# MishaLaskin/vqvae

Measured on AMD Instinct MI355X. Metric: images/sec VQ-VAE forward (32x32x3, K=512, D=64), higher is better.
Workload: dtype f32 (fp32 in/out/accumulate; conv products from two fp16 terms per operand, <= 2^-21 rel per product); 1 GPU; BASELINE config 3: full HIP path (Encoder+VQ+Decoder), 32x32x3, K=512, D=64; per_gpu_batch=4096, global_batch=4096, K=512, D=64, parallelism=batch-sharded replicas x1, no collective

## Files before the change

### vqvae_amd/csrc/common.h

```cpp
#pragma once

#include <hip/hip_runtime.h>
#include <stddef.h>
#include <stdint.h>

#include "../../include/vqvae_hip.h"

namespace vqvae {

typedef float f32x4 __attribute__((ext_vector_type(4)));
typedef float f32x16 __attribute__((ext_vector_type(16)));

__device__ __forceinline__ float sqsum8_f16(unsigned vx, unsigned vy, unsigned vz, unsigned vw, float s) {
    asm("v_dot2c_f32_f16 %0, %1, %1\n\tv_dot2c_f32_f16 %0, %2, %2\n\tv_dot2c_f32_f16 %0, %3, %3\n\tv_dot2c_f32_f16 %0, %4, %4"
        : "+v"(s) : "v"(vx), "v"(vy), "v"(vz), "v"(vw));
    return s;
}

constexpr int kWave = 64;
constexpr int kLdsBytes = 160 * 1024;

inline int num_cus() {
    static int n[64] = {0};
    int dev = 0;
    if (hipGetDevice(&dev) != hipSuccess || dev < 0 || dev >= 64) return 256;
    if (n[dev] == 0) {
        hipDeviceProp_t p;
        int c = 0;
        if (hipGetDeviceProperties(&p, dev) == hipSuccess) c = p.multiProcessorCount;
        n[dev] = c > 0 ? c : 256;
    }
    return n[dev];
}

void prof_begin(int id, hipStream_t st);
void prof_end(int id, hipStream_t st);
bool prof_dispatch(int id, hipEvent_t *start, hipEvent_t *stop);

inline size_t align_up(size_t x, size_t a) { return (x + a - 1) / a * a; }

inline unsigned grid_of(long long total, long long cap = 65536) {
    long long g = (total + 255) / 256;
    if (g > cap) g = cap;
    if (g < 1) g = 1;
    return (unsigned)g;
}

__device__ __forceinline__ void block_sum_f64(double *red, int tid, double v) {
    red[tid] = v;
    __syncthreads();
    for (int o = 128; o > 0; o >>= 1) {
        if (tid < o) red[tid] += red[tid + o];
        __syncthreads();
    }
}

struct VqPlan {
    int KC;
    int nchunks;
    int K_pad;
    size_t off_flags, off_ee, off_img, off_partials, off_img16, off_neh, off_imgh, off_seeds, off_imgf, off_chunk, total;
    size_t lds_bytes;
    int K32;
    size_t filter_lds_bytes;
};
constexpr int kVqCandCap = 8;
constexpr int kVqTilesPerWave = 2;
constexpr int kVqTicketBytes = 4096;
constexpr int kVqMaxGrid = 1024;
constexpr int kVqSlabRows = 1 << 18;
constexpr int kVqGroupSlabs = 16;

bool vq_track_ok(int K, int D);
bool vq_chunk_ok(int K, int D);
size_t vq_chunk_scratch_bytes(int D);

inline size_t vq_filter_lds_bytes(int K, int D) {
    const size_t K32 = ((size_t)K + 31) / 32 * 32;
    return K32 * D * 2 + K32 * 4 + (size_t)K * 4 + kVqTilesPerWave * (8 * 32 * 2 * kVqCandCap * 2 + 8 * 96 * 4) + 256 + 8;
}

enum class VqRoute { Track, TrackNchw, Chunk, Filter, Exact, AnyD, GenericVector, Unsupported };
VqRoute vq_route(int K, int D, int HW, int flags);

inline VqPlan vq_plan(int K, int D) {
    VqPlan p;
    const long budget = kLdsBytes - 256 - (long)K * 4;
    long kc = budget / ((long)D * 4 + 4);
    kc = kc / 32 * 32;
    const long kneed = ((long)K + 31) / 32 * 32;
    if (kc > kneed) kc = kneed;
    if (kc < 32) kc = 32;
    p.KC = (int)kc;
    p.nchunks = (K + p.KC - 1) / p.KC;
    p.K_pad = p.nchunks * p.KC;
    p.lds_bytes = (size_t)p.KC * D * 4 + (size_t)p.KC * 4 + (size_t)K * 4 + 256;
    p.off_flags = 0;
    p.off_ee = 256 + kVqTicketBytes;
    p.off_img = align_up(p.off_ee + (size_t)p.K_pad * 4, 256);
    p.off_partials = align_up(p.off_img + (size_t)p.K_pad * D * 4, 256);
    p.K32 = (K + 31) / 32 * 32;
    p.off_img16 = align_up(p.off_partials + sizeof(double) * kVqMaxGrid, 256);
    p.off_neh = align_up(p.off_img16 + (size_t)p.K32 * D * 2, 256);
    p.off_imgh = align_up(p.off_neh + (size_t)p.K32 * 4, 256);
    p.off_seeds = align_up(p.off_imgh + (size_t)(p.K32 + 512) * D * 2, 256);
    p.off_imgf = align_up(p.off_seeds + (size_t)p.K32 * 4 + 4096, 256);
    p.off_chunk = align_up(p.off_imgf + (size_t)(p.K32 + 512) * D * 2, 256);
    p.total = p.off_chunk + (vq_route(K, D, 0, VQVAE_VQ_ROWMAJOR) == VqRoute::Chunk ? vq_chunk_scratch_bytes(D) : 0);
    p.filter_lds_bytes = vq_filter_lds_bytes(K, D);
    return p;
}

int launch_vq_filter_d64(const float *z, const float *cb, long long N, int HW, int K, bool rowmajor,
                         float *zq, long long *idx, int *hist, char *ws, hipStream_t st, int *grid_out);

bool vq_track_nchw_ok(int K, int D, int HW);
inline int vq_form_of_flags(int flags) {
    const bool a = flags & VQVAE_VQ_UNITS64_8WAVES, b = flags & VQVAE_VQ_UNITS32_16WAVES;
    if (flags & VQVAE_VQ_UNITS32_8WAVES) return 32;
    return a && b ? 12 : (b ? 16 : (a ? 8 : 0));
}
struct VqTrackForm { int waves, unit_rows, grid, pool_pct; long long nunits; };
bool vq_track_form(long long N, int K, int HW, bool nchw, int form, int cus, VqTrackForm &f);
int launch_vq_track_d64(const float *z, const float *cb, long long N, int K, float *zq, long long *idx, int *hist,
                        char *ws, hipStream_t st, int *grid_out, int HW = 0, bool nchw = false, int form = 0);
void launch_vq_prepare16(const float *cb, int K, int D, char *ws, hipStream_t st);
int launch_vq_chunked(const float *z, const float *cb, long long N, int K, int D, float *zq, long long *idx, int *hist,
                      char *ws, hipStream_t st, int *grid_out, int *zq_amax = nullptr, int hw = 1);

int conv_forward_impl(int kind, const float *x, const float *packed, const float *bias, int64_t B, int H, int W, int Cin,
                      int Cout, int flags, float *y, hipStream_t stream, const int *in_amax, int *out_amax,
                      const float *ep_add = nullptr, const float *ep_mask = nullptr);
bool conv_reads_amax(int kind, int H, int W, int Cin, int Cout, int flags);
int res_layer_forward_impl(const float *x, const float *packed_w1, const float *packed_w2, int64_t B, int H, int W, int C,
                           int Rh, int flags, float *y, hipStream_t stream, const int *in_amax, int *out_amax,
                           float *hidden = nullptr, float *hid_scratch = nullptr);
bool res_layer_fused_ok(int C, int Rh);
bool res_pair_supported(int H, int W, int C, int Rh, int flags);
struct VqFuse {
    const uint4 *imgf; const float *seeds; const float *ee; const int *flags; const float *cb;
    int K, K32;
    float *zq; long long *idx; int *hist; double *partials;
};
struct ResPairPost { const float *packed; const float *bias; int Cout; float *out; int *zero = nullptr; int zero_n = 0;
                     const VqFuse *vq = nullptr; bool debug_ze = false; };
bool res_pair_post_supported(int C, int Cout);
int res_pair_forward_impl(const float *x, const float *packed_w1, const float *packed_w2, int64_t B, int H, int W, int C,
                          int Rh, int flags, float *y, hipStream_t stream, const int *in_amax, int *out_amax,
                          const ResPairPost *post = nullptr);
bool conv_res_pair_supported(int kind, int H, int W, int Cin, int C, int Rh);
int conv_res_pair_forward_impl(int kind, const float *x, const float *packed_front, const float *bias_front, int Cin,
                               const float *packed_w1, const float *packed_w2, int64_t B, int H, int W, int C, int Rh, int flags,
                               float *y, hipStream_t stream, const int *in_amax, int *out_amax, const ResPairPost *post = nullptr,
                               const int64_t *gather_idx = nullptr, int gather_K = 0);
int convt_out_forward_impl(const float *x, const float *packed, const float *bias, int64_t B, int H, int W, int Cin, int Cout,
                           int flags, float *y_nchw, hipStream_t stream, const int *in_amax);
void weight_spread_impl(const float *w, int Cout, int Cin, int taps, bool transposed, float *out, hipStream_t st);
void act_absmax_impl(const float *x, int64_t B, long long elems_per_image, int *amax, hipStream_t st);
constexpr int kVqGenericMaxD = 256;
constexpr int kRowSqnormMaxD = 1024;
bool vq_generic_ok(int K, int D);
size_t vq_generic_workspace_bytes(int K, int D);
int launch_vq_generic(const float *z, const float *cb, long long N, int HW, int K, int D, float beta, bool rowmajor, float *zq,
                      long long *idx, int *hist, float *loss, float *ppl, char *ws, hipStream_t st, bool hist_zeroed,
                      bool vector_units = false, bool prepared = false);
bool vq_fuse_ok(int K, int D, int flags);
int vq_prepare_impl(const float *codebook, int K, int D, int flags, void *workspace, size_t workspace_bytes, hipStream_t st);
VqFuse vq_fuse_args(const float *codebook, int K, void *workspace, float *z_q, int64_t *idx, int32_t *hist);
int vq_finalize_impl(const double *partials, int grid, int32_t *hist, int K, int64_t n_rows, int D, float beta, float *loss,
                     float *perplexity, hipStream_t st);
int vq_forward_impl(const float *z_e, const float *codebook, int64_t B, int D, int H, int W, int K, float beta, int flags,
                    float *z_q, int64_t *idx, int32_t *hist, float *loss, float *perplexity, void *workspace,
                    size_t workspace_bytes, vqvae_stream_t stream, bool hist_zeroed, int *zq_amax = nullptr,
                    bool *zq_amax_done = nullptr);
bool enc_front_supported(int H, int W, int Cin, int C1, int C2);
int enc_front_forward_impl(const float *x_nchw, const float *packed_in, const float *bias_in, const float *packed2,
                           const float *bias2, int64_t B, int H, int W, int Cin, int C1, int C2, float *y, hipStream_t st,
                           int *out_amax, int *zero_buf = nullptr, int zero_n = 0);
bool dec_tail_supported(int h4, int w4, int C, int C1, int Cout);
int dec_tail_forward_impl(const float *x, const float *packed2, const float *bias2, const float *packed4, const float *bias4,
                          int64_t B, int h4, int w4, int C, int C1, int Cout, float *y_nchw, hipStream_t st, const int *in_amax);
int conv_in_forward_impl(const float *x_nchw, const float *packed, const float *bias, int64_t B, int H, int W, int Cin,
                         int Cout, int flags, float *y, hipStream_t stream, int *out_amax, const float *ep_mask = nullptr);

}
```

### vqvae_amd/csrc/conv_fused.hip

```cpp
#include "conv_host.h"

namespace vqvae {
#ifndef CRP_NW
#define CRP_NW 4
#endif
#ifndef CRP_MINW
#define CRP_MINW 2
#endif
template <int NT3, bool VQ = false, bool GATHER = false, bool ZEOUT = false>
__global__ __launch_bounds__(CRP_NW * 64, CRP_MINW) void conv_res_pair8_h2_kernel(const float *__restrict__ in, FrontConv fc,
                                                                   const u32x4 *__restrict__ w1img, const u32x4 *__restrict__ w2img,
                                                                   float *__restrict__ out, int B, int flags,
                                                                   const int *__restrict__ hdr1, const int *__restrict__ hdr2,
                                                                   const int *__restrict__ in_amax, int *__restrict__ out_amax,
                                                                   const u32x4 *__restrict__ w3img, const int *__restrict__ hdr3,
                                                                   const float *__restrict__ bias3, float *__restrict__ out3,
                                                                   int *__restrict__ zero_buf, int zero_n, VqFuse vq) {
    static_assert(NT3 == 0 || NT3 == 1 || NT3 == 2 || NT3 == 4, "the 1x1 post conv streams through NT3 weight stages of 16 KiB");
    static_assert(!VQ || (NT3 == 2 && CRP_NW == 4), "the fused quantizer takes the 64-channel z_e of four images per workgroup");
    constexpr int NT2 = 4, C = 128, MT = 2, PX = 64, HP = PX + 1, PLANE = HP * 2;
    constexpr int TILE4 = 2 * 2 * PLANE;
    constexpr int RBUF = 4 * HP;
    __shared__ u32x4 As_all[CRP_NW * TILE4];
    constexpr int WBUF = 18 * 64;
    const int nvq = VQ ? (vq.K32 >> 7) : 0;
    const int NSTAGE = 18 + NT3 + nvq;
    __shared__ u32x4 Wb_all[2 * WBUF];
    __shared__ __attribute__((aligned(16))) unsigned char vq_tab_all[VQ ? CRP_NW * 1040 : 16];
    __shared__ int vq_hist_s[VQ ? 1024 : 1];
    __shared__ __attribute__((aligned(16))) float dw_s[288 + 32 * (NT3 > 0 ? NT3 : 1)];
    for (int i = threadIdx.x; i < 288 + 32 * NT3; i += CRP_NW * 64)
        dw_s[i] = i < 128 ? h2_dw(fc.hdr)[i] : (i < 160 ? h2_dw(hdr1)[i - 128] : (i < 288 ? h2_dw(hdr2)[i - 160] : h2_dw(hdr3)[i - 288]));
    __shared__ double vq_red_s[VQ ? CRP_NW : 1];
    if constexpr (VQ) {
        for (int i = threadIdx.x; i < vq.K; i += CRP_NW * 64) vq_hist_s[i] = 0;
    }
    const int tid = threadIdx.x, lane = tid & 63, wave = tid >> 6;
    const int l31 = lane & 31, h = lane >> 5;
    u32x4 *As = As_all + wave * TILE4;
    float *Hs = reinterpret_cast<float *>(As);
    const bool relu_out = flags & kFlagReluOut;
    constexpr int cpt = C >> 5;

    const long long img = (long long)blockIdx.x * CRP_NW + wave;
    const bool img_ok = img < B;
    if (zero_buf && blockIdx.x == 0)
        for (int i = tid; i < zero_n; i += CRP_NW * 64) zero_buf[i] = 0;

    int spx[MT];
    unsigned tapok[MT], tapok0[MT];
#pragma unroll
    for (int mt = 0; mt < MT; ++mt) {
        spx[mt] = 32 * mt + l31;
        const int y = spx[mt] >> 3, x = spx[mt] & 7;
        unsigned m = 0, m0 = 0;
#pragma unroll
        for (int t = 0; t < 9; ++t) {
            const int yy = y + t / 3 - 1, xx = x + t % 3 - 1;
            if (yy >= 0 && yy < 8 && xx >= 0 && xx < 8) m |= 1u << t;
            const int y0 = y + (int)((fc.dym >> (4 * t)) & 15) - 8, x0 = x + (int)((fc.dxm >> (4 * t)) & 15) - 8;
            if (y0 >= 0 && y0 < 8 && x0 >= 0 && x0 < 8) m0 |= 1u << t;
        }
        tapok[mt] = m;
        tapok0[mt] = m0;
    }

    f32x16 Y[MT][NT2];
    const int wave_u = __builtin_amdgcn_readfirstlane(wave);
    const unsigned dma_lane = (unsigned)lane * 16u;
    auto dma = [&](const u32x4 *src_uniform, u32x4 *dst_piece) {
        const unsigned lds = __builtin_amdgcn_readfirstlane((unsigned)(unsigned long long)(__attribute__((address_space(3))) char *)(char *)dst_piece);
        asm volatile("s_mov_b32 m0, %2\n\ts_nop 0\n\tglobal_load_lds_dwordx4 %0, %1" ::"v"(dma_lane), "s"(src_uniform), "s"(lds) : "memory");
    };
    auto dma_slice = [&](int sl, int buf) {
        const u32x4 *base = w1img + (size_t)(sl >> 1) * 256 + (sl & 1) * 64;
        for (int p = wave_u; p < 18; p += CRP_NW)
            dma(base + (size_t)(p >> 1) * cpt * 256 + (p & 1) * 128, Wb_all + buf * WBUF + p * 64);
    };
    auto dma_linear = [&](const u32x4 *src, int buf) {
#pragma unroll
        for (int j = 0; j < 16 / CRP_NW; ++j) dma(src + (wave_u * (16 / CRP_NW) + j) * 64, Wb_all + buf * WBUF + (wave_u * (16 / CRP_NW) + j) * 64);
    };
    auto dma_stage = [&](int k, int buf) {
        if (VQ && k >= 18 + NT3) {
            const int j = k - (18 + NT3);
            dma_linear(reinterpret_cast<const u32x4 *>(vq.imgf) + (size_t)j * 1024, buf);
            if (wave_u == 0) dma(reinterpret_cast<const u32x4 *>(vq.seeds) + (size_t)j * 32, Wb_all + buf * WBUF + 16 * 64);
        }
        else if (k >= 18) dma_linear(w3img + (size_t)(k - 18) * 1024, buf);
        else if (k % 9 == 8) dma_linear(w2img, buf);
        else dma_slice(k % 9, buf);
    };
    auto dma_wait_sync = [&]() {
        asm volatile("s_waitcnt vmcnt(0)" ::: "memory");
        __syncthreads();
    };
    float ymax = 0.0f;
    int wstage = 0;
    {
        const int cpt0 = fc.Cin >> 5;
        const float *src = in + ((size_t)(img_ok ? img : 0) * PX + lane) * fc.Cin;
        bool gbad = false;
        if constexpr (GATHER) {
            const long long k = vq.idx[(size_t)(img_ok ? img : 0) * PX + lane];
            gbad = k < 0 || k >= vq.K;
            src = in + (size_t)(gbad ? 0 : k) * fc.Cin;
        }
        const bool gany = GATHER && __builtin_amdgcn_ballot_w64(gbad) != 0;
        f32x4 raw[8];
        auto load_raw0 = [&](int cc) {
#pragma unroll
            for (int j = 0; j < 8; ++j) raw[j] = *reinterpret_cast<const f32x4 *>(src + 32 * cc + 4 * j);
            if (gany) {
                const float qn = __builtin_nanf("");
#pragma unroll
                for (int j = 0; j < 8; ++j) if (gbad) raw[j] = f32x4{qn, qn, qn, qn};
            }
        };
        float m = 0.0f;
        const int given = (in_amax && img_ok) ? in_amax[img] : -1;
        if (given >= 0) m = __int_as_float(given);
        else for (int cc = 0; cc < cpt0; ++cc) {
            load_raw0(cc);
#pragma unroll
            for (int j = 0; j < 8; ++j)
                m = fmaxf(m, fmaxf(fmaxf(__builtin_fabsf(raw[j].x), __builtin_fabsf(raw[j].y)), fmaxf(__builtin_fabsf(raw[j].z), __builtin_fabsf(raw[j].w))));
        }
        const int kx = wave_scale_exp(img_ok ? m : 0.0f);
        const float xs = __builtin_ldexpf(1.0f, kx), d0 = __builtin_ldexpf(1.0f, -kx);
#pragma unroll
        for (int mt = 0; mt < MT; ++mt)
#pragma unroll
            for (int nt = 0; nt < NT2; ++nt)
#pragma unroll
                for (int r = 0; r < 16; ++r) Y[mt][nt][r] = 0.0f;
        if (lane < 8) As[(lane >> 1) * PLANE + (lane & 1) * HP + PX] = u32x4{0, 0, 0, 0};
        auto dma_front = [&](int cc, int tap, int buf) {
            const u32x4 *base = fc.wimg + (size_t)(tap * cpt0 + cc) * (NT2 * 256);
#pragma unroll
            for (int j = 0; j < 16 / CRP_NW; ++j) {
                const int p = wave_u * (16 / CRP_NW) + j;
                dma(base + (p >> 2) * 256 + ((p >> 1) & 1) * 64 + (p & 1) * 128, Wb_all + buf * WBUF + p * 64);
            }
        };
        load_raw0(0);
        dma_front(0, 0, 0);
        for (int cc = 0; cc < cpt0; ++cc) {
            __builtin_amdgcn_wave_barrier();
            u32x4 *dst = As + lane;
#pragma unroll
            for (int t = 0; t < 2; ++t)
#pragma unroll
                for (int hh = 0; hh < 2; ++hh) {
                    u32x4 t1, t2;
                    split8_h(raw[4 * hh + 2 * t], raw[4 * hh + 2 * t + 1], xs, t1, t2);
                    dst[(t * 2 + 0) * PLANE + hh * HP] = t1;
                    dst[(t * 2 + 1) * PLANE + hh * HP] = t2;
                }
            lds_order_wave();
#pragma unroll 1
            for (int tap = 0; tap < 9; ++tap, ++wstage) {
                const int shift = ((int)((fc.dym >> (4 * tap)) & 15) - 8) * 8 + ((int)((fc.dxm >> (4 * tap)) & 15) - 8);
                u32x4 X[2][MT][2];
#pragma unroll
                for (int t = 0; t < 2; ++t)
#pragma unroll
                    for (int mt = 0; mt < MT; ++mt) {
                        const int p = ((tapok0[mt] >> tap) & 1u) ? spx[mt] + shift : PX;
                        const u32x4 *ap = As + (t * 2) * PLANE + h * HP + p;
                        X[t][mt][0] = ap[0];
                        X[t][mt][1] = ap[PLANE];
                    }
                if (tap == 1 && cc + 1 < cpt0) {
                    asm volatile("s_waitcnt vmcnt(8)" ::: "memory");
                    __syncthreads();
                } else dma_wait_sync();
                if (tap + 1 < 9) dma_front(cc, tap + 1, (wstage + 1) & 1);
                else if (cc + 1 < cpt0) dma_front(cc + 1, 0, (wstage + 1) & 1);
                else dma_stage(0, (wstage + 1) & 1);
                if (tap == 0 && cc + 1 < cpt0) load_raw0(cc + 1);
                const u32x4 *wt = Wb_all + (wstage & 1) * WBUF + lane;
                u32x4 Wc0 = wt[0], Wc1 = wt[64];
#pragma unroll
                for (int g = 0; g < 8; ++g) {
                    const int t = g >> 2, nt = g & 3;
                    u32x4 Wn0 = Wc0, Wn1 = Wc1;
                    if (g + 1 < 8) {
                        const u32x4 *bp = wt + (((g + 1) & 3) * 4 + ((g + 1) >> 2) * 2) * 64;
                        Wn0 = bp[0];
                        Wn1 = bp[64];
                    }
                    __builtin_amdgcn_sched_barrier(0);
                    prod3x2t(X[t][0][0], X[t][0][1], X[t][1][0], X[t][1][1], Wc0, Wc1, Y[0][nt], Y[1][nt]);
                    __builtin_amdgcn_sched_barrier(0);
                    Wc0 = Wn0;
                    Wc1 = Wn1;
                }
            }
        }
#pragma unroll
        for (int nt = 0; nt < NT2; ++nt)
#pragma unroll
            for (int g = 0; g < 4; ++g) {
                f32x4 bv = {0.0f, 0.0f, 0.0f, 0.0f};
                if (fc.bias) bv = *reinterpret_cast<const f32x4 *>(fc.bias + nt * 32 + 8 * g + 4 * h);
                const f32x4 dv = h2_dw4(dw_s, nt * 32, g, h, d0);
#pragma unroll
                for (int mt = 0; mt < MT; ++mt)
#pragma unroll
                    for (int q = 0; q < 4; q += 2)
                        SCALE2_BIAS_RELU2(Y[mt][nt][4 * g + q], Y[mt][nt][4 * g + q + 1], dv[q], dv[q + 1], bv[q], bv[q + 1], ymax);
            }
    }
    lds_order_wave();

    auto stage_sync = [&](int k) -> const u32x4 * {
        dma_wait_sync();
        if (k + 1 < NSTAGE) dma_stage(k + 1, (wstage + k + 1) & 1);
        return Wb_all + ((wstage + k) & 1) * WBUF + lane;
    };
    f32x16 acc1[MT];
    auto taps = [&](const u32x4 *wb, const u32x4 *pl) {
        u32x4 Xc[MT][2], Wc[2];
        auto ld = [&](int tap, u32x4(&X)[MT][2], u32x4(&W)[2]) {
            const int shift = (tap / 3 - 1) * 8 + (tap % 3 - 1);
#pragma unroll
            for (int mt = 0; mt < MT; ++mt) {
                const int p = ((tapok[mt] >> tap) & 1u) ? spx[mt] + shift : PX;
                X[mt][0] = pl[p];
                X[mt][1] = pl[p + HP * 2];
            }
            W[0] = wb[tap * 128];
            W[1] = wb[tap * 128 + 64];
        };
        ld(0, Xc, Wc);
#pragma unroll
        for (int tap = 0; tap < 9; ++tap) {
            u32x4 Xn[MT][2], Wn[2];
            if (tap + 1 < 9) ld(tap + 1, Xn, Wn);
            __builtin_amdgcn_sched_barrier(0);
            prod3x2t(Xc[0][0], Xc[0][1], Xc[1][0], Xc[1][1], Wc[0], Wc[1], acc1[0], acc1[1]);
            __builtin_amdgcn_sched_barrier(0);
            if (tap + 1 < 9) {
#pragma unroll
                for (int mt = 0; mt < MT; ++mt) { Xc[mt][0] = Xn[mt][0]; Xc[mt][1] = Xn[mt][1]; }
                Wc[0] = Wn[0]; Wc[1] = Wn[1];
            }
        }
    };
    auto put_planes = [&](int buf, const u32x4(&T1)[MT][2], const u32x4(&T2)[MT][2], int t) {
        u32x4 *pb = As + buf * RBUF + h * HP + l31;
#pragma unroll
        for (int mt = 0; mt < MT; ++mt) {
            pb[32 * mt] = T1[mt][t];
            pb[32 * mt + 2 * HP] = T2[mt][t];
        }
    };
    auto layer = [&](auto LT, bool relu_after) __attribute__((always_inline)) {
        constexpr int LI = decltype(LT)::value;
        const int kx = wave_scale_exp(img_ok ? ymax : 0.0f);
        const float xscale = __builtin_ldexpf(1.0f, kx), d1 = __builtin_ldexpf(1.0f, -kx);
#pragma unroll
        for (int mt = 0; mt < MT; ++mt)
#pragma unroll
            for (int r = 0; r < 16; ++r) acc1[mt][r] = 0.0f;
        u32x4 T1[MT][2], T2[MT][2];
#pragma unroll
        for (int mt = 0; mt < MT; ++mt) acc_to_ksteps(Y[mt][0], xscale, T1[mt], T2[mt]);
        __builtin_amdgcn_wave_barrier();
        put_planes(0, T1, T2, 0);
#pragma unroll
        for (int c = 0; c < NT2; ++c) {
            __builtin_amdgcn_wave_barrier();
            put_planes(1, T1, T2, 1);
            lds_order_wave();
            taps(stage_sync(9 * LI + 2 * c), As + h * HP);
            if (c + 1 < NT2) {
#pragma unroll
                for (int mt = 0; mt < MT; ++mt) acc_to_ksteps(Y[mt][c + 1], xscale, T1[mt], T2[mt]);
                __builtin_amdgcn_wave_barrier();
                put_planes(0, T1, T2, 0);
            }
            lds_order_wave();
            taps(stage_sync(9 * LI + 2 * c + 1), As + RBUF + h * HP);
        }
        float m = 0.0f;
#pragma unroll
        for (int g = 0; g < 4; ++g) {
            const f32x4 dv = h2_dw4(dw_s + 128, 0, g, h, d1);
#pragma unroll
            for (int mt = 0; mt < MT; ++mt)
#pragma unroll
                for (int q = 0; q < 4; q += 2)
                    SCALE2_BIAS_RELU2(acc1[mt][4 * g + q], acc1[mt][4 * g + q + 1], dv[q], dv[q + 1], 0.0f, 0.0f, m);
        }
        const int kh = wave_scale_exp(m);
        const float hscale = __builtin_ldexpf(1.0f, kh), d2 = __builtin_ldexpf(1.0f, -kh);
        u32x4 H1[MT][2], Hb[MT][2];
#pragma unroll
        for (int mt = 0; mt < MT; ++mt) acc_to_ksteps(acc1[mt], hscale, H1[mt], Hb[mt]);
        const u32x4 *wb = stage_sync(9 * LI + 8);
        float nmax = 0.0f;
#pragma unroll
        for (int nt = 0; nt < NT2; ++nt) {
            u32x4 Wc[2][2];
#pragma unroll
            for (int t = 0; t < 2; ++t) { Wc[t][0] = wb[nt * 256 + t * 64]; Wc[t][1] = wb[nt * 256 + t * 64 + 128]; }
            f32x16 acc2[MT];
#pragma unroll
            for (int mt = 0; mt < MT; ++mt)
#pragma unroll
                for (int r = 0; r < 16; ++r) acc2[mt][r] = 0.0f;
#pragma unroll
            for (int t = 0; t < 2; ++t)
                prod3x2t(H1[0][t], Hb[0][t], H1[1][t], Hb[1][t], Wc[t][0], Wc[t][1], acc2[0], acc2[1]);
            if (relu_after) {
#pragma unroll
                for (int g = 0; g < 4; ++g) {
                    const f32x4 dv = h2_dw4(dw_s + 160, nt * 32, g, h, d2);
#pragma unroll
                    for (int mt = 0; mt < MT; ++mt)
#pragma unroll
                        for (int q = 0; q < 4; q += 2) {
                            const int r = 4 * g + q;
                            const float y0 = relu1(__builtin_fmaf(acc2[mt][r], dv[q], Y[mt][nt][r]));
                            const float y1 = relu1(__builtin_fmaf(acc2[mt][r + 1], dv[q + 1], Y[mt][nt][r + 1]));
                            Y[mt][nt][r] = y0;
                            Y[mt][nt][r + 1] = y1;
                            vmax3(nmax, y0, y1);
                        }
                }
            } else {
#pragma unroll
                for (int g = 0; g < 4; ++g) {
                    const f32x4 dv = h2_dw4(dw_s + 160, nt * 32, g, h, d2);
#pragma unroll
                    for (int mt = 0; mt < MT; ++mt)
#pragma unroll
                        for (int q = 0; q < 4; q += 2) {
                            const int r = 4 * g + q;
                            const float y0 = __builtin_fmaf(acc2[mt][r], dv[q], Y[mt][nt][r]), y1 = __builtin_fmaf(acc2[mt][r + 1], dv[q + 1], Y[mt][nt][r + 1]);
                            Y[mt][nt][r] = y0;
                            Y[mt][nt][r + 1] = y1;
                            vmax3_abs(nmax, y0, y1);
                        }
                }
            }
        }
        ymax = nmax;
    };
    layer(std::integral_constant<int, 0>{}, true);
    layer(std::integral_constant<int, 1>{}, relu_out);
    if (out_amax && img_ok) publish_amax_exclusive(out_amax, img, ymax, lane);

    auto store_tile = [&](const float(&v)[16], float *dst, int ld) {
        __builtin_amdgcn_wave_barrier();
#pragma unroll
        for (int g = 0; g < 4; ++g)
            *reinterpret_cast<f32x4 *>(Hs + l31 * 36 + 8 * g + 4 * h) = f32x4{v[4 * g], v[4 * g + 1], v[4 * g + 2], v[4 * g + 3]};
        lds_order_wave();
#pragma unroll
        for (int k = 0; k < 4; ++k) {
            const int p = (lane >> 3) + 8 * k;
            *reinterpret_cast<f32x4 *>(dst + (size_t)p * ld + 4 * (lane & 7)) = *reinterpret_cast<const f32x4 *>(Hs + p * 36 + 4 * (lane & 7));
        }
    };
    const long long wbase = img * PX;
    if constexpr (NT3 > 0) {
        const int kx3 = wave_scale_exp(img_ok ? ymax : 0.0f);
        const float xs3 = __builtin_ldexpf(1.0f, kx3), d3 = __builtin_ldexpf(1.0f, -kx3);
        f32x16 acc3[MT][NT3];
#pragma unroll
        for (int mt = 0; mt < MT; ++mt)
#pragma unroll
            for (int n3 = 0; n3 < NT3; ++n3)
#pragma unroll
                for (int r = 0; r < 16; ++r) acc3[mt][n3][r] = 0.0f;
        const u32x4 *wb = nullptr;
#pragma unroll
        for (int c = 0; c < NT2; ++c) {
            u32x4 T1[MT][2], T2[MT][2];
#pragma unroll
            for (int mt = 0; mt < MT; ++mt) acc_to_ksteps(Y[mt][c], xs3, T1[mt], T2[mt]);
            constexpr int CPS = 4 / NT3;
            if (c % CPS == 0) wb = stage_sync(18 + c / CPS);
#pragma unroll
            for (int t = 0; t < 2; ++t)
#pragma unroll
                for (int n3 = 0; n3 < NT3; ++n3) {
                    const u32x4 *bp = wb + ((c % CPS) * NT3 + n3) * 256 + t * 64;
                    prod3x2t(T1[0][t], T2[0][t], T1[1][t], T2[1][t], bp[0], bp[128], acc3[0][n3], acc3[1][n3]);
                }
        }
        if constexpr (VQ) {
#pragma unroll
            for (int mt = 0; mt < MT; ++mt)
#pragma unroll
                for (int n3 = 0; n3 < NT3; ++n3)
#pragma unroll
                    for (int g = 0; g < 4; ++g) {
                        f32x4 bv = {0.0f, 0.0f, 0.0f, 0.0f};
                        if (bias3) bv = *reinterpret_cast<const f32x4 *>(bias3 + n3 * 32 + 8 * g + 4 * h);
                        const f32x4 dv = h2_dw4(dw_s + 288, n3 * 32, g, h, d3);
#pragma unroll
                        for (int q = 0; q < 4; ++q) acc3[mt][n3][4 * g + q] = acc3[mt][n3][4 * g + q] * dv[q] + bv[q];
                    }
            u32x4 zb[MT][4];
            float zn2[MT];
#pragma unroll
            for (int mt = 0; mt < MT; ++mt) {
                float sq = 0.0f;
#pragma unroll
                for (int n3 = 0; n3 < NT3; ++n3)
#pragma unroll
                    for (int t = 0; t < 2; ++t) {
                        float P[4], Q[4];
#pragma unroll
                        for (int q = 0; q < 4; ++q) {
                            P[q] = acc3[mt][n3][4 * t + q];
                            Q[q] = acc3[mt][n3][8 + 4 * t + q];
                            swap_halves(P[q], Q[q]);
                        }
                        u32x4 v;
                        v.x = __builtin_bit_cast(unsigned, __builtin_convertvector((f32x2v{P[0], P[1]}), f16x2));
                        v.y = __builtin_bit_cast(unsigned, __builtin_convertvector((f32x2v{P[2], P[3]}), f16x2));
                        v.z = __builtin_bit_cast(unsigned, __builtin_convertvector((f32x2v{Q[0], Q[1]}), f16x2));
                        v.w = __builtin_bit_cast(unsigned, __builtin_convertvector((f32x2v{Q[2], Q[3]}), f16x2));
                        zb[mt][2 * n3 + t] = v;
                        sq = sqsum8_f16(v.x, v.y, v.z, v.w, sq);
                    }
                const auto sw = __builtin_amdgcn_permlane32_swap(__float_as_uint(sq), __float_as_uint(sq), false, false);
                zn2[mt] = sq + __uint_as_float(h ? sw[0] : sw[1]);
            }
            const float inf = __builtin_inff();
            const float pinf = inf, ninf = -inf;
            unsigned keymask = trk::kKeyMask;
            asm volatile("" : "+v"(keymask));
            trk::Lane L[MT];
#pragma unroll
            for (int mt = 0; mt < MT; ++mt) trk::init(L[mt], ninf);
            auto sweep_stage = [&](const u32x4 *wb, const float *sd, int j, auto &&use) {
#pragma unroll
                for (int ctl = 0; ctl < 4; ++ctl) {
                    f32x16 seed;
#pragma unroll
                    for (int g = 0; g < 4; ++g) {
                        const f32x4 e4 = *reinterpret_cast<const f32x4 *>(sd + ctl * 32 + h * 16 + 4 * g);
                        seed[4 * g] = e4.x; seed[4 * g + 1] = e4.y; seed[4 * g + 2] = e4.z; seed[4 * g + 3] = e4.w;
                    }
                    u32x4 a[4];
#pragma unroll
                    for (int ks = 0; ks < 4; ++ks) a[ks] = wb[ctl * 256 + ks * 64];
                    use(4 * j + ctl, a, seed);
                }
            };
            for (int j = 0; j < nvq; ++j) {
                const u32x4 *wb = stage_sync(18 + NT3 + j);
                const float *sd = reinterpret_cast<const float *>(wb - lane + 16 * 64);
                sweep_stage(wb, sd, j, [&](int ct, const u32x4(&a)[4], const f32x16 &seed) {
                    f32x16 acc[MT];
#pragma unroll
                    for (int mt = 0; mt < MT; ++mt) {
                        acc[mt] = __builtin_amdgcn_mfma_f32_32x32x16_f16(__builtin_bit_cast(f16x8, a[0]), __builtin_bit_cast(f16x8, zb[mt][0]), seed, 0, 0, 0);
#pragma unroll
                        for (int ks = 1; ks < 4; ++ks)
                            acc[mt] = __builtin_amdgcn_mfma_f32_32x32x16_f16(__builtin_bit_cast(f16x8, a[ks]), __builtin_bit_cast(f16x8, zb[mt][ks]), acc[mt], 0, 0, 0);
                    }
                    unsigned cell0 = (unsigned)(2 * ct), cell1 = cell0 + 1u;
                    asm volatile("" : "+s"(cell0), "+s"(cell1));
#pragma unroll
                    for (int mt = 0; mt < MT; ++mt) trk::tile(L[mt], acc[mt], cell0, cell1, keymask, ninf, pinf);
                });
            }
            vqu::Tables tb = vqu::tables(vq_tab_all + wave_u * 1040);
            const vqu::BoundP bound = vqu::load_boundp(vq.flags);
            vqu::RowsSp<MT> R;
            vqu::classify_sp<MT>(L, zn2, bound, vq.K, lane, img_ok ? PX : 0, ninf, tb.task_s, R);
            vqu::Flagged FL = vqu::exact_begin_sp<MT>(R, lane, tb);
            int ntasks = FL.ndirect;
            const bool rescan_me = FL.hmask && FL.ndirect <= 64;
            int nres = 0;
            if (__syncthreads_or(rescan_me ? 1 : 0)) {
                dma_stage(18 + NT3, 0);
                for (int j = 0; j < nvq; ++j) {
                    dma_wait_sync();
                    if (j + 1 < nvq) dma_stage(18 + NT3 + j + 1, (j + 1) & 1);
                    if (rescan_me && FL.ndirect + nres <= 64) {
                        const u32x4 *wb = Wb_all + (j & 1) * WBUF + lane;
                        const float *sd = reinterpret_cast<const float *>(Wb_all + (j & 1) * WBUF + 16 * 64);
#pragma unroll
                        for (int mt = 0; mt < MT; ++mt)
                            if ((unsigned)(FL.hmask >> (32 * mt))) {
                                const float thr_t = (((unsigned)(FL.hmask >> (32 * mt)) >> l31) & 1u) ? R.thr[mt] : inf;
                                sweep_stage(wb, sd, j, [&](int ct, const u32x4(&a)[4], const f32x16 &seed) {
                                    f32x16 acc = __builtin_amdgcn_mfma_f32_32x32x16_f16(__builtin_bit_cast(f16x8, a[0]), __builtin_bit_cast(f16x8, zb[mt][0]), seed, 0, 0, 0);
#pragma unroll
                                    for (int ks = 1; ks < 4; ++ks)
                                        acc = __builtin_amdgcn_mfma_f32_32x32x16_f16(__builtin_bit_cast(f16x8, a[ks]), __builtin_bit_cast(f16x8, zb[mt][ks]), acc, 0, 0, 0);
                                    vqu::rescan_tile(acc, thr_t, ct, mt, lane, vq.K, FL.ndirect, ninf, tb, nres);
                                });
                            }
                    }
                }
                if (rescan_me) {
                    lds_order_wave();
                    ntasks = FL.ndirect + nres;
                }
            }
            __syncthreads();
            unsigned char *zlo = reinterpret_cast<unsigned char *>(As);
            unsigned char *zhi = reinterpret_cast<unsigned char *>(Wb_all) + (size_t)wave_u * 9216;
            auto zchunk = [&](int row, int c16) -> f32x4 * {
                unsigned char *b = row < 32 ? zlo + row * 256 : zhi + (row - 32) * 256;
                return reinterpret_cast<f32x4 *>(b + (((unsigned)c16 ^ ((unsigned)row & 15u)) << 4));
            };
            __builtin_amdgcn_wave_barrier();
#pragma unroll
            for (int mt = 0; mt < MT; ++mt)
#pragma unroll
                for (int n3 = 0; n3 < NT3; ++n3)
#pragma unroll
                    for (int g = 0; g < 4; ++g)
                        *zchunk(32 * mt + l31, 8 * n3 + 2 * g + h) = f32x4{acc3[mt][n3][4 * g], acc3[mt][n3][4 * g + 1], acc3[mt][n3][4 * g + 2], acc3[mt][n3][4 * g + 3]};
            lds_order_wave();
            if constexpr (ZEOUT) {
                if (img_ok)
#pragma unroll
                    for (int c16 = 0; c16 < 16; ++c16)
                        *reinterpret_cast<f32x4 *>(out3 + ((size_t)img * PX + lane) * 64 + 4 * c16) = *zchunk(lane, c16);
            }
            vqu::exact_end_sp<MT>(R, FL, ntasks, lane, tb, vq.cb, vq.ee, vq.K,
                           [&](int rr, int jc) { return *zchunk(rr, jc); },
                           [&](int rr, int c) { return reinterpret_cast<const float *>(zchunk(rr, c >> 2))[c & 3]; });
            const int j16 = lane & 15, g4 = lane >> 4;
            const float sacc = vqu::epilogue_sp<false, MT>(R, lane, vq.cb, vq.K, [&](int t, int i) { return *zchunk(32 * t + 4 * i + g4, j16); },
                                             (img_ok && vq.zq) ? vq.zq + (size_t)img * PX * 64 : nullptr, img_ok ? PX : 0,
                                             vq.idx + (size_t)(img_ok ? img : 0) * PX, vq_hist_s);
            double dacc = img_ok ? (double)sacc : 0.0;
#pragma unroll
            for (int o = 32; o > 0; o >>= 1) dacc += __shfl_xor(dacc, o);
            if (lane == 0) vq_red_s[wave_u] = dacc;
            __syncthreads();
            if (tid == 0) {
                double sum = 0.0;
                for (int w = 0; w < CRP_NW; ++w) sum += vq_red_s[w];
                vq.partials[blockIdx.x] = sum;
            }
            for (int k = tid; k < vq.K; k += CRP_NW * 64) {
                const int c = vq_hist_s[k];
                if (c) atomicAdd(&vq.hist[k], c);
            }
        } else
        if (img_ok) {
#pragma unroll
            for (int mt = 0; mt < MT; ++mt)
#pragma unroll
                for (int n3 = 0; n3 < NT3; ++n3) {
                    float v[16];
#pragma unroll
                    for (int g = 0; g < 4; ++g) {
                        f32x4 bv = {0.0f, 0.0f, 0.0f, 0.0f};
                        if (bias3) bv = *reinterpret_cast<const f32x4 *>(bias3 + n3 * 32 + 8 * g + 4 * h);
                        const f32x4 dv = h2_dw4(dw_s + 288, n3 * 32, g, h, d3);
#pragma unroll
                        for (int q = 0; q < 4; ++q) v[4 * g + q] = acc3[mt][n3][4 * g + q] * dv[q] + bv[q];
                    }
                    store_tile(v, out3 + (wbase + mt * 32) * (32 * NT3) + n3 * 32, 32 * NT3);
                }
        }
    } else if (img_ok) {
#pragma unroll
        for (int mt = 0; mt < MT; ++mt)
#pragma unroll
            for (int nt = 0; nt < NT2; ++nt) {
                float v[16];
#pragma unroll
                for (int r = 0; r < 16; ++r) v[r] = Y[mt][nt][r];
                store_tile(v, out + (wbase + mt * 32) * C + nt * 32, C);
            }
    }
}

#ifndef EF_MINW
#define EF_MINW 2
#endif
template <int CIN>
__global__ __launch_bounds__(256, EF_MINW) void enc_front8_h2_kernel(const float *__restrict__ x, const u32x4 *__restrict__ w0img,
                                                               const int *__restrict__ hdr0, const float *__restrict__ bias0,
                                                               const u32x4 *__restrict__ w2img, const int *__restrict__ hdr2,
                                                               const float *__restrict__ bias2, float *__restrict__ out, int B,
                                                               int *__restrict__ out_amax, int *__restrict__ zero_buf, int zero_n) {
    constexpr int NT = 4, MT = 2, PX = 64, HP = PX + 1, PLANE = HP * 2, C0 = 64, C = 128;
    if (zero_buf && blockIdx.x == 0)
        for (int i = threadIdx.x; i < zero_n; i += 256) zero_buf[i] = 0;
    constexpr int TILE4 = 2 * 2 * PLANE;
    constexpr int WBUF = 16 * 64, NSTAGE = 32;
    __shared__ u32x4 As_all[4 * TILE4];
    __shared__ u32x4 Wb_all[2 * WBUF];
    __shared__ u32x4 W0s[2 * CIN * 2 * 64];
    __shared__ __attribute__((aligned(16))) float dw_s[64 + 128];
    const int tid = threadIdx.x, lane = tid & 63, wave = tid >> 6;
    const int l31 = lane & 31, h = lane >> 5;
    u32x4 *As = As_all + wave * TILE4;
    float *Hs = reinterpret_cast<float *>(As);
    const int wave_u = __builtin_amdgcn_readfirstlane(wave);
    const long long img = (long long)blockIdx.x * 4 + wave;
    const bool img_ok = img < B;

    const unsigned dma_lane = (unsigned)lane * 16u;
    auto dma = [&](const u32x4 *src_uniform, u32x4 *dst_piece) {
        const unsigned lds = __builtin_amdgcn_readfirstlane((unsigned)(unsigned long long)(__attribute__((address_space(3))) char *)(char *)dst_piece);
        asm volatile("s_mov_b32 m0, %2\n\ts_nop 0\n\tglobal_load_lds_dwordx4 %0, %1" ::"v"(dma_lane), "s"(src_uniform), "s"(lds) : "memory");
    };
    auto dma_stage = [&](int k, int buf) {
        const u32x4 *src = w2img + (size_t)k * 1024;
#pragma unroll
        for (int j = 0; j < 4; ++j) dma(src + (wave_u * 4 + j) * 64, Wb_all + buf * WBUF + (wave_u * 4 + j) * 64);
    };
    auto dma_wait_sync = [&]() {
        asm volatile("s_waitcnt vmcnt(0)" ::: "memory");
        __syncthreads();
    };
    dma_stage(0, 0);
    for (int i = tid; i < 2 * CIN * 2 * 64; i += 256) W0s[i] = w0img[i];
    if (tid < C0 + C) dw_s[tid] = tid < C0 ? h2_dw(hdr0)[tid] : h2_dw(hdr2)[tid - C0];
    if (lane < 8) As[(lane >> 1) * PLANE + (lane & 1) * HP + PX] = u32x4{0, 0, 0, 0};

    int spx[MT];
    unsigned tapok[MT];
#pragma unroll
    for (int mt = 0; mt < MT; ++mt) {
        spx[mt] = 32 * mt + l31;
        const int y = spx[mt] >> 3, xx0 = spx[mt] & 7;
        unsigned m = 0;
        for (int q = 0; q < 16; ++q) {
            const int yy = y + ((q >> 1) & 1) - (q >> 3), xx = xx0 + (q & 1) - ((q >> 2) & 1);
            if (yy >= 0 && yy < 8 && xx >= 0 && xx < 8) m |= 1u << q;
        }
        tapok[mt] = m;
    }

    const float *ximg = x + (size_t)(img_ok ? img : 0) * (CIN * 1024);
    float xm = 0.0f;
#pragma unroll
    for (int j = 0; j < CIN * 4; ++j) {
        const f32x4 v = *reinterpret_cast<const f32x4 *>(ximg + 4 * lane + 256 * j);
        xm = fmaxf(xm, fmaxf(fmaxf(__builtin_fabsf(v.x), __builtin_fabsf(v.y)), fmaxf(__builtin_fabsf(v.z), __builtin_fabsf(v.w))));
    }
#pragma unroll
    for (int o = 32; o > 0; o >>= 1) xm = fmaxf(xm, __shfl_xor(xm, o));
    const int kx0 = wave_scale_exp(img_ok ? xm : 0.0f);
    const float xs0 = __builtin_ldexpf(1.0f, kx0), d0 = __builtin_ldexpf(1.0f, -kx0);
    float bm = bias0 ? __builtin_fabsf(bias0[lane]) : 0.0f;
    const float bound = (__int_as_float(hdr0[1]) * xm + bm) * 1.0001f;
    const int k1 = wave_scale_exp(img_ok ? bound : 0.0f);
    const float xs1 = __builtin_ldexpf(1.0f, k1), d2 = __builtin_ldexpf(1.0f, -k1);

    f32x16 Y[MT][NT];
#pragma unroll
    for (int mt = 0; mt < MT; ++mt)
#pragma unroll
        for (int nt = 0; nt < NT; ++nt)
#pragma unroll
            for (int r = 0; r < 16; ++r) Y[mt][nt][r] = 0.0f;
    const long long img_u = (long long)blockIdx.x * 4 + wave_u;
    const auto xrs = __builtin_amdgcn_make_buffer_rsrc(const_cast<float *>(x + (size_t)(img_u < B ? img_u : 0) * (CIN * 1024)), 0,
                                                       (unsigned)(CIN * 4096), 0x00020000);
    __syncthreads();

    auto taps = [&](int cc) {
        const int sub = cc >> 1;
#pragma unroll 1
        for (int tap = 0; tap < 4; ++tap) {
            const int k = cc * 4 + tap;
            const int shift = ((tap >> 1) - (sub >> 1)) * 8 + ((tap & 1) - (sub & 1)), okbit = sub * 4 + tap;
            u32x4 X[2][MT][2];
#pragma unroll
            for (int t = 0; t < 2; ++t)
#pragma unroll
                for (int mt = 0; mt < MT; ++mt) {
                    const int p = ((tapok[mt] >> okbit) & 1u) ? spx[mt] + shift : PX;
                    const u32x4 *ap = As + (t * 2) * PLANE + h * HP + p;
                    X[t][mt][0] = ap[0];
                    X[t][mt][1] = ap[PLANE];
                }
            dma_wait_sync();
            if (k + 1 < NSTAGE) dma_stage(k + 1, (k + 1) & 1);
            const u32x4 *wt = Wb_all + (k & 1) * WBUF + lane;
            u32x4 Wc0 = wt[0], Wc1 = wt[128];
#pragma unroll
            for (int g = 0; g < 8; ++g) {
                const int t = g >> 2, nt = g & 3;
                u32x4 Wn0 = Wc0, Wn1 = Wc1;
                if (g + 1 < 8) {
                    const u32x4 *bp = wt + ((g + 1) & 3) * 256 + ((g + 1) >> 2) * 64;
                    Wn0 = bp[0];
                    Wn1 = bp[128];
                }
                __builtin_amdgcn_sched_barrier(0);
                prod3x2t(X[t][0][0], X[t][0][1], X[t][1][0], X[t][1][1], Wc0, Wc1, Y[0][nt], Y[1][nt]);
                __builtin_amdgcn_sched_barrier(0);
                Wc0 = Wn0;
                Wc1 = Wn1;
            }
        }
    };
    auto put_planes = [&](const u32x4(&T1)[MT][2], const u32x4(&T2)[MT][2]) {
        __builtin_amdgcn_wave_barrier();
#pragma unroll
        for (int t = 0; t < 2; ++t)
#pragma unroll
            for (int mt = 0; mt < MT; ++mt) {
                As[(t * 2 + 0) * PLANE + h * HP + 32 * mt + l31] = T1[mt][t];
                As[(t * 2 + 1) * PLANE + h * HP + 32 * mt + l31] = T2[mt][t];
            }
        lds_order_wave();
    };
    auto first_layer = [&](int sl, const u32x4(&XB)[MT][CIN][2], u32x4(&T1)[MT][2], u32x4(&T2)[MT][2]) {
        f32x16 acc0[MT];
#pragma unroll
        for (int mt = 0; mt < MT; ++mt)
#pragma unroll
            for (int r = 0; r < 16; ++r) acc0[mt][r] = 0.0f;
        const u32x4 *wp = W0s + (sl * CIN) * 128 + lane;
#pragma unroll
        for (int ci = 0; ci < CIN; ++ci)
            prod3x2t(XB[0][ci][0], XB[0][ci][1], XB[1][ci][0], XB[1][ci][1], wp[ci * 128], wp[ci * 128 + 64], acc0[0], acc0[1]);
#pragma unroll
        for (int g = 0; g < 4; ++g) {
            f32x4 bv = {0.0f, 0.0f, 0.0f, 0.0f};
            if (bias0) bv = *reinterpret_cast<const f32x4 *>(bias0 + sl * 32 + 8 * g + 4 * h);
            const f32x4 dv = h2_dw4(dw_s, sl * 32, g, h, d0);
#pragma unroll
            for (int mt = 0; mt < MT; ++mt)
#pragma unroll
                for (int q = 0; q < 4; q += 2) {
                    float unused = 0.0f;
                    SCALE2_BIAS_RELU2(acc0[mt][4 * g + q], acc0[mt][4 * g + q + 1], dv[q], dv[q + 1], bv[q], bv[q + 1], unused);
                }
        }
#pragma unroll
        for (int mt = 0; mt < MT; ++mt) acc_to_ksteps(acc0[mt], xs1, T1[mt], T2[mt]);
    };

#pragma unroll 1
    for (int s = 0; s < 4; ++s) {
        const int sy = s >> 1, sx = s & 1;
        u32x4 XB[MT][CIN][2];
#pragma unroll
        for (int mt = 0; mt < MT; ++mt) {
            const int by = spx[mt] >> 3, bx = spx[mt] & 7;
            const int col0 = 4 * bx + 2 * sx - 1;
            const int adj = col0 < 0 ? 1 : (col0 + 3 > 31 ? -1 : 0);
            f32x4 pv[CIN][2];
#pragma unroll
            for (int ci = 0; ci < CIN; ++ci)
#pragma unroll
                for (int rr = 0; rr < 2; ++rr) {
                    const int row = 4 * by + 2 * sy - 1 + 2 * h + rr;
                    const unsigned off = (row >= 0 && row < 32) ? (unsigned)(((ci * 32 + row) * 32 + col0 + adj) * 4) : kOobOffset;
                    pv[ci][rr] = __builtin_bit_cast(f32x4, __builtin_amdgcn_raw_buffer_load_b128(xrs, off, 0, 0));
                }
#pragma unroll
            for (int ci = 0; ci < CIN; ++ci) {
#pragma unroll
                for (int rr = 0; rr < 2; ++rr) {
                    const f32x4 v = pv[ci][rr];
                    f32x4 o;
                    o.x = adj > 0 ? 0.0f : (adj < 0 ? v.y : v.x);
                    o.y = adj > 0 ? v.x : (adj < 0 ? v.z : v.y);
                    o.z = adj > 0 ? v.y : (adj < 0 ? v.w : v.z);
                    o.w = adj > 0 ? v.z : (adj < 0 ? 0.0f : v.w);
                    pv[ci][rr] = o;
                }
                split8_h(pv[ci][0], pv[ci][1], xs0, XB[mt][ci][0], XB[mt][ci][1]);
            }
        }
        u32x4 T1[MT][2], T2[MT][2], U1[MT][2], U2[MT][2];
        first_layer(0, XB, T1, T2);
        put_planes(T1, T2);
        first_layer(1, XB, U1, U2);
        taps(2 * s);
        put_planes(U1, U2);
        taps(2 * s + 1);
    }

    float ymax = 0.0f;
    const long long wbase = img * PX;
#pragma unroll
    for (int mt = 0; mt < MT; ++mt)
#pragma unroll
        for (int nt = 0; nt < NT; ++nt) {
            float v[16];
#pragma unroll
            for (int g = 0; g < 4; ++g) {
                f32x4 bv = {0.0f, 0.0f, 0.0f, 0.0f};
                if (bias2) bv = *reinterpret_cast<const f32x4 *>(bias2 + nt * 32 + 8 * g + 4 * h);
                const f32x4 dv = h2_dw4(dw_s + C0, nt * 32, g, h, d2);
#pragma unroll
                for (int q = 0; q < 4; q += 2) {
                    v[4 * g + q] = Y[mt][nt][4 * g + q];
                    v[4 * g + q + 1] = Y[mt][nt][4 * g + q + 1];
                    SCALE2_BIAS_RELU2(v[4 * g + q], v[4 * g + q + 1], dv[q], dv[q + 1], bv[q], bv[q + 1], ymax);
                }
            }
            if (img_ok) {
                float *dst = out + (wbase + mt * 32) * C + nt * 32;
                __builtin_amdgcn_wave_barrier();
#pragma unroll
                for (int g = 0; g < 4; ++g)
                    *reinterpret_cast<f32x4 *>(Hs + l31 * 36 + 8 * g + 4 * h) = f32x4{v[4 * g], v[4 * g + 1], v[4 * g + 2], v[4 * g + 3]};
                lds_order_wave();
#pragma unroll
                for (int k = 0; k < 4; ++k) {
                    const int p = (lane >> 3) + 8 * k;
                    *reinterpret_cast<f32x4 *>(dst + (size_t)p * C + 4 * (lane & 7)) = *reinterpret_cast<const f32x4 *>(Hs + p * 36 + 4 * (lane & 7));
                }
            }
        }
    if (out_amax && img_ok) publish_amax_exclusive(out_amax, img, ymax, lane);
    (void)C0;
}

struct TailGeom {
    unsigned long long dym[4], dxm[4];
};

#ifndef DT_MINW
#define DT_MINW 2
#endif
__global__ __launch_bounds__(256, DT_MINW) void dec_tail8_h2_kernel(const float *__restrict__ in, const u32x4 *__restrict__ w2img,
                                                              const int *__restrict__ hdr2, const float *__restrict__ bias2,
                                                              TailGeom tg, const u32x4 *__restrict__ w4img,
                                                              const int *__restrict__ hdr4, const float *__restrict__ bias4,
                                                              float *__restrict__ out, int B, const int *__restrict__ in_amax) {
    constexpr int NT = 2, MT = 2, PX = 64, HP = PX + 1, PLANE = HP * 2, CIN = 128, CPT = CIN / 32, CO = 3;
    constexpr int TILE4 = 2 * 2 * PLANE;
    constexpr int WBUF = 16 * 64, NSTAGE = 34;
    __shared__ u32x4 As_all[4 * TILE4];
    __shared__ u32x4 Wb_all[2 * WBUF];
    __shared__ __attribute__((aligned(16))) float dw_s[64];
    if (threadIdx.x < 64) dw_s[threadIdx.x] = h2_dw(hdr2)[threadIdx.x];
    const int tid = threadIdx.x, lane = tid & 63, wave = tid >> 6;
    const int l31 = lane & 31, h = lane >> 5;
    u32x4 *As = As_all + wave * TILE4;
    const int wave_u = __builtin_amdgcn_readfirstlane(wave);
    const long long img = (long long)blockIdx.x * 4 + wave;
    const bool img_ok = img < B;

    const unsigned dma_lane = (unsigned)lane * 16u;
    auto dma = [&](const u32x4 *src_uniform, u32x4 *dst_piece) {
        const unsigned lds = __builtin_amdgcn_readfirstlane((unsigned)(unsigned long long)(__attribute__((address_space(3))) char *)(char *)dst_piece);
        asm volatile("s_mov_b32 m0, %2\n\ts_nop 0\n\tglobal_load_lds_dwordx4 %0, %1" ::"v"(dma_lane), "s"(src_uniform), "s"(lds) : "memory");
    };
    auto dma_stage = [&](int k, int buf) {
        const int py = k / 17, i = k - 17 * py;
#pragma unroll
        for (int j = 0; j < 4; ++j) {
            const int p = wave_u * 4 + j, half = p >> 3;
            const int ty = (i >> 1) & 1, kind = i & 1, tap = ty * 2 + (half ? 1 - kind : kind);
            const u32x4 *src = i == 16 ? w4img + p * 64
                                       : w2img + (size_t)((2 * py + half) * 16 + tap * CPT + (i >> 2)) * 512 + (p & 7) * 64;
            dma(src, Wb_all + buf * WBUF + p * 64);
        }
    };
    auto dma_wait_sync = [&]() {
        asm volatile("s_waitcnt vmcnt(0)" ::: "memory");
        __syncthreads();
    };
    dma_stage(0, 0);
    if (lane < 8) As[(lane >> 1) * PLANE + (lane & 1) * HP + PX] = u32x4{0, 0, 0, 0};

    const long long img_u = (long long)blockIdx.x * 4 + wave_u;
    const auto ors = __builtin_amdgcn_make_buffer_rsrc(out + (size_t)(img_u < B ? img_u : 0) * (CO * 1024), 0, img_u < B ? (unsigned)(CO * 4096) : 0u, 0x00020000);
    int spx[MT];
#pragma unroll
    for (int mt = 0; mt < MT; ++mt) spx[mt] = 32 * mt + l31;
    const float *src = in + ((size_t)(img_ok ? img : 0) * PX + lane) * CIN;
    f32x4 raw[8];
    auto load_raw = [&](int cc) {
#pragma unroll
        for (int j = 0; j < 8; ++j) raw[j] = *reinterpret_cast<const f32x4 *>(src + 32 * cc + 4 * j);
    };
    float m = 0.0f;
    const int given = (in_amax && img_ok) ? in_amax[img] : -1;
    if (given >= 0) m = __int_as_float(given);
    else for (int cc = 0; cc < CPT; ++cc) {
        load_raw(cc);
#pragma unroll
        for (int j = 0; j < 8; ++j)
            m = fmaxf(m, fmaxf(fmaxf(__builtin_fabsf(raw[j].x), __builtin_fabsf(raw[j].y)), fmaxf(__builtin_fabsf(raw[j].z), __builtin_fabsf(raw[j].w))));
    }
    const int kx = wave_scale_exp(img_ok ? m : 0.0f);
    const float xs = __builtin_ldexpf(1.0f, kx), d1 = __builtin_ldexpf(1.0f, -kx);
    load_raw(0);

#pragma unroll 1
    for (int py = 0; py < 2; ++py) {
        unsigned long long dym[2], dxm[2];
        unsigned tapok[2][MT];
#pragma unroll
        for (int px = 0; px < 2; ++px) {
            dym[px] = tg.dym[2 * py + px];
            dxm[px] = tg.dxm[2 * py + px];
#pragma unroll
            for (int mt = 0; mt < MT; ++mt) {
                const int y = spx[mt] >> 3, x = spx[mt] & 7;
                unsigned mk = 0;
#pragma unroll
                for (int t = 0; t < 4; ++t) {
                    const int yy = y + (int)((dym[px] >> (4 * t)) & 15) - 8, xx = x + (int)((dxm[px] >> (4 * t)) & 15) - 8;
                    if (yy >= 0 && yy < 8 && xx >= 0 && xx < 8) mk |= 1u << t;
                }
                tapok[px][mt] = mk;
            }
        }
        f32x16 acc[2][MT][NT];
#pragma unroll
        for (int px = 0; px < 2; ++px)
#pragma unroll
            for (int mt = 0; mt < MT; ++mt)
#pragma unroll
                for (int nt = 0; nt < NT; ++nt)
#pragma unroll
                    for (int r = 0; r < 16; ++r) acc[px][mt][nt][r] = 0.0f;
#pragma unroll 1
        for (int cc = 0; cc < CPT; ++cc) {
            __builtin_amdgcn_wave_barrier();
            u32x4 *dst = As + lane;
#pragma unroll
            for (int t = 0; t < 2; ++t)
#pragma unroll
                for (int hh = 0; hh < 2; ++hh) {
                    u32x4 t1, t2;
                    split8_h(raw[4 * hh + 2 * t], raw[4 * hh + 2 * t + 1], xs, t1, t2);
                    dst[(t * 2 + 0) * PLANE + hh * HP] = t1;
                    dst[(t * 2 + 1) * PLANE + hh * HP] = t2;
                }
            lds_order_wave();
#pragma unroll 1
            for (int i = 0; i < 4; ++i) {
                const int k = py * 17 + cc * 4 + i;
                const int ty = i >> 1, kind = i & 1;
                const int tapA = ty * 2 + kind, tapB = ty * 2 + 1 - kind;
                u32x4 X[2][MT][2];
                auto ldX = [&](int t, int px, int tap) {
                    const int shift = ((int)((dym[px] >> (4 * tap)) & 15) - 8) * 8 + ((int)((dxm[px] >> (4 * tap)) & 15) - 8);
#pragma unroll
                    for (int mt = 0; mt < MT; ++mt) {
                        const int p = ((tapok[px][mt] >> tap) & 1u) ? spx[mt] + shift : PX;
                        const u32x4 *ap = As + (t * 2) * PLANE + h * HP + p;
                        X[t][mt][0] = ap[0];
                        X[t][mt][1] = ap[PLANE];
                    }
                };
                ldX(0, 0, tapA);
                ldX(1, 0, tapA);
                if (i == 1) {
                    asm volatile("s_waitcnt vmcnt(8)" ::: "memory");
                    __syncthreads();
                } else dma_wait_sync();
                dma_stage(k + 1, (k + 1) & 1);
                if (i == 0) load_raw(cc + 1 < CPT ? cc + 1 : 0);
                const u32x4 *wt = Wb_all + (k & 1) * WBUF + lane;
                u32x4 Wc0 = wt[0], Wc1 = wt[128];
#pragma unroll
                for (int g = 0; g < 8; ++g) {
                    const int px = g >> 2, t = (g >> 1) & 1, nt = g & 1;
                    u32x4 Wn0 = Wc0, Wn1 = Wc1;
                    if (g + 1 < 8) {
                        const int g1 = g + 1;
                        const u32x4 *bp = wt + (g1 >> 2) * 512 + (g1 & 1) * 256 + ((g1 >> 1) & 1) * 64;
                        Wn0 = bp[0];
                        Wn1 = bp[128];
                    }
                    if (g == 2) ldX(0, 1, tapB);
                    if (g == 4) ldX(1, 1, tapB);
                    __builtin_amdgcn_sched_barrier(0);
                    prod3x2t(X[t][0][0], X[t][0][1], X[t][1][0], X[t][1][1], Wc0, Wc1, acc[px][0][nt], acc[px][1][nt]);
                    __builtin_amdgcn_sched_barrier(0);
                    Wc0 = Wn0;
                    Wc1 = Wn1;
                }
            }
        }
        f32x16 T[2][2][MT];
        float d4[2];
        const u32x4 *wt4 = nullptr;
#pragma unroll
        for (int px = 0; px < 2; ++px) {
            float um = 0.0f;
#pragma unroll
            for (int nt = 0; nt < NT; ++nt)
#pragma unroll
                for (int g = 0; g < 4; ++g) {
                    f32x4 bv = {0.0f, 0.0f, 0.0f, 0.0f};
                    if (bias2) bv = *reinterpret_cast<const f32x4 *>(bias2 + nt * 32 + 8 * g + 4 * h);
                    const f32x4 dv = h2_dw4(dw_s, nt * 32, g, h, d1);
#pragma unroll
                    for (int mt = 0; mt < MT; ++mt)
#pragma unroll
                        for (int q = 0; q < 4; q += 2)
                            SCALE2_BIAS_RELU2(acc[px][mt][nt][4 * g + q], acc[px][mt][nt][4 * g + q + 1], dv[q], dv[q + 1], bv[q], bv[q + 1], um);
                }
            const int ku = wave_scale_exp(img_ok ? um : 0.0f);
            const float us = __builtin_ldexpf(1.0f, ku);
            d4[px] = __builtin_ldexpf(1.0f, -ku);
            u32x4 U1[MT][NT][2], U2[MT][NT][2];
#pragma unroll
            for (int mt = 0; mt < MT; ++mt)
#pragma unroll
                for (int nt = 0; nt < NT; ++nt) acc_to_ksteps(acc[px][mt][nt], us, U1[mt][nt], U2[mt][nt]);
#pragma unroll
            for (int m2 = 0; m2 < 2; ++m2)
#pragma unroll
                for (int mt = 0; mt < MT; ++mt)
#pragma unroll
                    for (int r = 0; r < 16; ++r) T[px][m2][mt][r] = 0.0f;
            if (px == 0) {
                const int k = py * 17 + 16;
                dma_wait_sync();
                if (k + 1 < NSTAGE) dma_stage(k + 1, (k + 1) & 1);
                wt4 = Wb_all + (k & 1) * WBUF + lane;
            }
#pragma unroll
            for (int kk = 0; kk < 4; ++kk)
#pragma unroll
                for (int m2 = 0; m2 < 2; ++m2) {
                    const u32x4 *bp = wt4 + (m2 * 4 + kk) * 128;
                    prod3x2t(U1[0][kk >> 1][kk & 1], U2[0][kk >> 1][kk & 1], U1[1][kk >> 1][kk & 1], U2[1][kk >> 1][kk & 1], bp[0], bp[64],
                             T[px][m2][0], T[px][m2][1]);
                }
        }
        const bool xl = (lane & 7) != 0, xr = (lane & 7) != 7;
        unsigned roff[MT][2];
        bool only1[MT][2];
#pragma unroll
        for (int mt = 0; mt < MT; ++mt)
#pragma unroll
            for (int g = 0; g < 2; ++g) {
                const int row = 4 * (spx[mt] >> 3) + 2 * py - 1 + h + 2 * g;
                roff[mt][g] = (row >= 0 && row < 32) ? (unsigned)((row * 32 + 4 * (lane & 7)) * 4) : kOobOffset;
                only1[mt][g] = row == 31;
            }
        f32x4 ov[2][MT][2];
        auto ov_load = [&](int co, f32x4(&o)[MT][2]) {
#pragma unroll
            for (int mt = 0; mt < MT; ++mt)
#pragma unroll
                for (int g = 0; g < 2; ++g)
                    o[mt][g] = __builtin_bit_cast(f32x4, __builtin_amdgcn_raw_buffer_load_b128(ors, roff[mt][g], (unsigned)co * 4096u, 0));
        };
        if (py > 0) ov_load(0, ov[0]);
#pragma unroll
        for (int co = 0; co < CO; ++co) {
            if (py > 0 && co + 1 < CO) ov_load(co + 1, ov[(co + 1) & 1]);
            const float bv = bias4 ? bias4[co] : 0.0f;
            const float w4d = h2_dw(hdr4)[co];
            const float d40 = d4[0] * w4d, d41 = d4[1] * w4d;
#pragma unroll
            for (int mt = 0; mt < MT; ++mt)
#pragma unroll
                for (int g = 0; g < 2; ++g) {
                    const f32x16 &T0 = T[0][co >> 1][mt], &T1 = T[1][co >> 1][mt];
                    const int r0 = 8 * (co & 1) + 4 * g;
                    const float a0 = T0[r0] * d40, b0 = T1[r0] * d41, b1 = T1[r0 + 1] * d41, b2 = T1[r0 + 2] * d41, b3 = T1[r0 + 3] * d41;
                    float lb3 = __builtin_bit_cast(float, __builtin_amdgcn_update_dpp(0, __builtin_bit_cast(int, b3), 0x111, 0xf, 0xf, true));
                    float ra0 = __builtin_bit_cast(float, __builtin_amdgcn_update_dpp(0, __builtin_bit_cast(int, a0), 0x101, 0xf, 0xf, true));
                    lb3 = xl ? lb3 : 0.0f;
                    ra0 = xr ? ra0 : 0.0f;
                    f32x4 e;
                    e.x = __builtin_fmaf(T0[r0 + 1], d40, lb3);
                    e.y = __builtin_fmaf(T0[r0 + 2], d40, b0);
                    e.z = __builtin_fmaf(T0[r0 + 3], d40, b1);
                    e.w = ra0 + b2;
                    f32x4 base = {bv, bv, bv, bv};
                    if (py > 0 && !only1[mt][g]) base = ov[co & 1][mt][g];
                    const f32x4 v = base + e;
                    __builtin_amdgcn_raw_buffer_store_b128(__builtin_bit_cast(u32x4, v), ors, roff[mt][g] == kOobOffset ? kOobOffset : roff[mt][g] + (unsigned)co * 4096u, 0, 0);
                }
        }
        __builtin_amdgcn_wave_barrier();
        if (lane < 8) As[(lane >> 1) * PLANE + (lane & 1) * HP + PX] = u32x4{0, 0, 0, 0};
    }
}

}

using namespace vqvae;

bool vqvae::conv_res_pair_supported(int kind, int H, int W, int Cin, int C, int Rh) {
    return (kind == VQVAE_CONV_3x3_S1 || kind == VQVAE_CONVT_3x3_S1) && H == 8 && W == 8 && C == 128 && Cin >= 32 && Cin % 32 == 0 &&
           Cin <= 256 && Rh >= 1 && Rh <= 32;
}

int vqvae::conv_res_pair_forward_impl(int kind, const float *x, const float *packed_front, const float *bias_front, int Cin,
                                      const float *packed_w1, const float *packed_w2, int64_t B, int H, int W, int C, int Rh,
                                      int flags, float *y, hipStream_t st, const int *in_amax, int *out_amax,
                                      const ResPairPost *post, const int64_t *gather_idx, int gather_K) {
    if (gather_idx && (post || gather_K < 1)) return VQVAE_ERR_UNSUPPORTED;
    if (!x || !packed_front || !packed_w1 || !packed_w2 || (!y && !post)) return VQVAE_ERR_NULL;
    if (B < 1 || !conv_res_pair_supported(kind, H, W, Cin, C, Rh)) return VQVAE_ERR_UNSUPPORTED;
    if ((reinterpret_cast<uintptr_t>(x) | reinterpret_cast<uintptr_t>(y) | reinterpret_cast<uintptr_t>(post ? post->out : nullptr)) & 15)
        return VQVAE_ERR_UNSUPPORTED;
    ConvGeom g;
    if (make_geom(kind, B, H, W, Cin, C, 0, g) != VQVAE_OK || g.nphase != 1 || g.ntaps != 9) return VQVAE_ERR_UNSUPPORTED;
    const char *hf = reinterpret_cast<const char *>(packed_front) + packed_h2_offset(g, kind);
    FrontConv fc;
    fc.wimg = reinterpret_cast<const u32x4 *>(hf + h2_header_bytes(g.ntile));
    fc.hdr = reinterpret_cast<const int *>(hf);
    fc.bias = bias_front;
    fc.dym = g.dymask[0];
    fc.dxm = g.dxmask[0];
    fc.Cin = Cin;
    const int cpt = C / 32;
    const char *h1 = reinterpret_cast<const char *>(packed_w1) + (size_t)9 * cpt * (1024 * sizeof(float) + 3072 * sizeof(unsigned short));
    const char *h2 = reinterpret_cast<const char *>(packed_w2) + (size_t)cpt * (1024 * sizeof(float) + 3072 * sizeof(unsigned short));
    const u32x4 *w1h = reinterpret_cast<const u32x4 *>(h1 + h2_header_bytes(1)), *w2h = reinterpret_cast<const u32x4 *>(h2 + h2_header_bytes((C + 31) / 32));
    const int *hd1 = reinterpret_cast<const int *>(h1), *hd2 = reinterpret_cast<const int *>(h2);
    const unsigned gtc = (unsigned)((B + CRP_NW - 1) / CRP_NW);
    ConvGeom g3;
    if (post && (!post->packed || !post->out || !res_pair_post_supported(C, post->Cout) ||
                 make_geom(VQVAE_CONV_1x1, 1, 8, 8, C, post->Cout, 0, g3) != VQVAE_OK)) return VQVAE_ERR_UNSUPPORTED;
    if (post && post->vq && (post->Cout != 64 || CRP_NW != 4 || post->vq->K32 % 128 || post->vq->K32 > 1024 || !post->vq->partials))
        return VQVAE_ERR_UNSUPPORTED;
    prof_begin(VQVAE_PROF_RES_LAYER, st);
    if (post) {
        const char *h3 = reinterpret_cast<const char *>(post->packed) + packed_h2_offset(g3, VQVAE_CONV_1x1);
        const u32x4 *w3h = reinterpret_cast<const u32x4 *>(h3 + h2_header_bytes(g3.ntile));
        const int *hd3 = reinterpret_cast<const int *>(h3);
#define CRP_POST(NT3_)                                                                                                          \
    hipLaunchKernelGGL((conv_res_pair8_h2_kernel<NT3_>), dim3(gtc), dim3(CRP_NW * 64), 0, st, x, fc, w1h, w2h, y, (int)B, flags, hd1, hd2, \
                       in_amax, out_amax, w3h, hd3, post->bias, post->out, post->zero, post->zero_n, VqFuse{})
        if (post->vq && post->debug_ze) {
            hipLaunchKernelGGL((conv_res_pair8_h2_kernel<2, true, false, true>), dim3(gtc), dim3(CRP_NW * 64), 0, st, x, fc, w1h, w2h, y, (int)B, flags,
                               hd1, hd2, in_amax, out_amax, w3h, hd3, post->bias, post->out, post->zero, post->zero_n, *post->vq);
        } else if (post->vq) {
            hipLaunchKernelGGL((conv_res_pair8_h2_kernel<2, true>), dim3(gtc), dim3(CRP_NW * 64), 0, st, x, fc, w1h, w2h, y, (int)B, flags,
                               hd1, hd2, in_amax, out_amax, w3h, hd3, post->bias, post->out, post->zero, post->zero_n, *post->vq);
        } else
        switch (post->Cout / 32) {
            case 1: CRP_POST(1); break;
            case 2: CRP_POST(2); break;
            case 4: CRP_POST(4); break;
        }
#undef CRP_POST
    } else {
        if (gather_idx) {
            VqFuse gf{};
            gf.idx = reinterpret_cast<long long *>(const_cast<int64_t *>(gather_idx));
            gf.K = gather_K;
            hipLaunchKernelGGL((conv_res_pair8_h2_kernel<0, false, true>), dim3(gtc), dim3(CRP_NW * 64), 0, st, x, fc, w1h, w2h, y, (int)B, flags,
                               hd1, hd2, in_amax, out_amax, nullptr, nullptr, nullptr, nullptr, nullptr, 0, gf);
        } else
        hipLaunchKernelGGL((conv_res_pair8_h2_kernel<0>), dim3(gtc), dim3(CRP_NW * 64), 0, st, x, fc, w1h, w2h, y, (int)B, flags, hd1, hd2,
                           in_amax, out_amax, nullptr, nullptr, nullptr, nullptr, nullptr, 0, VqFuse{});
    }
    prof_end(VQVAE_PROF_RES_LAYER, st);
    return (int)hipGetLastError();
}

bool vqvae::enc_front_supported(int H, int W, int Cin, int C1, int C2) { return H == 32 && W == 32 && Cin == 3 && C1 == 64 && C2 == 128; }

int vqvae::enc_front_forward_impl(const float *x_nchw, const float *packed_in, const float *bias_in, const float *packed2,
                                  const float *bias2, int64_t B, int H, int W, int Cin, int C1, int C2, float *y, hipStream_t st,
                                  int *out_amax, int *zero_buf, int zero_n) {
    if (!x_nchw || !packed_in || !packed2 || !y) return VQVAE_ERR_NULL;
    if (B < 1 || !enc_front_supported(H, W, Cin, C1, C2)) return VQVAE_ERR_UNSUPPORTED;
    if ((reinterpret_cast<uintptr_t>(x_nchw) | reinterpret_cast<uintptr_t>(y)) & 15) return VQVAE_ERR_UNSUPPORTED;
    const int ntile0 = (C1 + 31) / 32;
    const char *h0 = reinterpret_cast<const char *>(packed_in) +
                     (size_t)ntile0 * ((size_t)((Cin * 8 + 3) / 4) * 256 + (size_t)Cin * 768) * sizeof(float);
    ConvGeom g;
    if (make_geom(VQVAE_CONV_4x4_S2, B, H / 2, W / 2, C1, C2, 0, g) != VQVAE_OK) return VQVAE_ERR_UNSUPPORTED;
    const char *h2 = reinterpret_cast<const char *>(packed2) + packed_h2_offset(g, VQVAE_CONV_4x4_S2);
    const u32x4 *w2s2d = reinterpret_cast<const u32x4 *>(h2 + h2_header_bytes(g.ntile) + packed_h2_bytes(g));
    prof_begin(VQVAE_PROF_CONV_IGEMM, st);
    hipLaunchKernelGGL((enc_front8_h2_kernel<3>), dim3((unsigned)((B + 3) / 4)), dim3(256), 0, st, x_nchw,
                       reinterpret_cast<const u32x4 *>(h0 + h2_header_bytes(ntile0)), reinterpret_cast<const int *>(h0), bias_in, w2s2d,
                       reinterpret_cast<const int *>(h2), bias2, y, (int)B, out_amax, zero_buf, zero_n);
    prof_end(VQVAE_PROF_CONV_IGEMM, st);
    return (int)hipGetLastError();
}

bool vqvae::dec_tail_supported(int h4, int w4, int C, int C1, int Cout) { return h4 == 8 && w4 == 8 && C == 128 && C1 == 64 && Cout == 3; }

int vqvae::dec_tail_forward_impl(const float *x, const float *packed2, const float *bias2, const float *packed4, const float *bias4,
                                 int64_t B, int h4, int w4, int C, int C1, int Cout, float *y_nchw, hipStream_t st, const int *in_amax) {
    if (!x || !packed2 || !packed4 || !y_nchw) return VQVAE_ERR_NULL;
    if (B < 1 || !dec_tail_supported(h4, w4, C, C1, Cout)) return VQVAE_ERR_UNSUPPORTED;
    if ((reinterpret_cast<uintptr_t>(x) | reinterpret_cast<uintptr_t>(y_nchw)) & 15) return VQVAE_ERR_UNSUPPORTED;
    ConvGeom g;
    if (make_geom(VQVAE_CONVT_4x4_S2, B, h4, w4, C, C1, 0, g) != VQVAE_OK) return VQVAE_ERR_UNSUPPORTED;
    const char *h2 = reinterpret_cast<const char *>(packed2) + packed_h2_offset(g, VQVAE_CONVT_4x4_S2);
    TailGeom tg;
    for (int ph = 0; ph < 4; ++ph) { tg.dym[ph] = g.dymask[ph]; tg.dxm[ph] = g.dxmask[ph]; }
    const int ntile4 = (16 * Cout + 31) / 32, cpt4 = (C1 + 31) / 32;
    const size_t cells = (size_t)cpt4 * ntile4;
    const char *h4p = reinterpret_cast<const char *>(packed4) + cells * (1024 * sizeof(float) + 3072 * sizeof(unsigned short));
    prof_begin(VQVAE_PROF_CONV_OUT, st);
    hipLaunchKernelGGL(dec_tail8_h2_kernel, dim3((unsigned)((B + 3) / 4)), dim3(256), 0, st, x,
                       reinterpret_cast<const u32x4 *>(h2 + h2_header_bytes(g.ntile)), reinterpret_cast<const int *>(h2), bias2, tg,
                       reinterpret_cast<const u32x4 *>(h4p + h2_header_bytes(1) + cells * 2048 * sizeof(unsigned short)),
                       reinterpret_cast<const int *>(h4p), bias4, y_nchw, (int)B, in_amax);
    prof_end(VQVAE_PROF_CONV_OUT, st);
    return (int)hipGetLastError();
}
```

### vqvae_amd/csrc/model.hip

```cpp
#include "common.h"
#include <map>
#include <mutex>
#include <utility>
#include <vector>

namespace vqvae {
namespace {

struct PartsRecord {
    int64_t B;
    int H, W, flags;
    const void *vqws;
    std::vector<std::pair<int64_t, int64_t>> claimed;
};
std::mutex g_parts_mu;
std::map<const void *, PartsRecord> g_parts;

constexpr int kVqFormFlags = VQVAE_VQ_UNITS64_8WAVES | VQVAE_VQ_UNITS32_16WAVES | VQVAE_VQ_UNITS32_8WAVES;

struct Carve {
    char *p;
    size_t left;
    bool ok = true;
    float *f32(size_t n) { return reinterpret_cast<float *>(raw(n * sizeof(float))); }
    void *raw(size_t bytes) {
        bytes = align_up(bytes, 256);
        if (bytes > left) { ok = false; return nullptr; }
        void *r = p;
        p += bytes;
        left -= bytes;
        return r;
    }
};

bool dims_ok(const VqvaeDims *d) {
    return d && d->h_dim >= 8 && d->h_dim % 8 == 0 && d->res_h_dim >= 1 && d->n_res_layers >= 0 && d->n_embeddings >= 1 &&
           d->embedding_dim >= 1 && (d->in_ch == 1 || d->in_ch == 3 || d->in_ch == 4);
}

size_t act_elems(const VqvaeDims *d, int64_t B, int H, int W) {
    const size_t half = (size_t)B * (H / 2) * (W / 2) * (d->h_dim / 2);
    const size_t quarter = (size_t)B * (H / 4) * (W / 4) * d->h_dim;
    return half > quarter ? half : quarter;
}

int res_stack(const float *w1, const float *w2, const float *x, int64_t B, int H, int W, int C, int Rh, int n_layers,
              bool first_relu_in, bool final_relu, float *y, float *tmp, hipStream_t st, const float **out, int *amax = nullptr,
              const ResPairPost *post = nullptr, bool *post_done = nullptr, int conv_flags = 0, float *hid_scratch = nullptr) {
    const float *cur = x;
    *out = x;
    const bool generic = !res_layer_fused_ok(C, Rh);
    if (generic && !hid_scratch) return VQVAE_ERR_UNSUPPORTED;
    if (generic) amax = nullptr;
    const bool pairs = !generic && n_layers >= 2 && res_pair_supported(H, W, C, Rh, conv_flags);
    const int nsteps = pairs ? n_layers / 2 + (n_layers & 1) : n_layers;
    int i = 0;
    for (int j = 0; j < nsteps; ++j) {
        const bool pair = pairs && i + 1 < n_layers;
        const int last = pair ? i + 1 : i;
        int flags = ((i == 0 && first_relu_in) ? VQVAE_CONV_RELU_IN : 0) | conv_flags;
        if (last < n_layers - 1 || final_relu) flags |= VQVAE_CONV_RELU_OUT;
        float *dst = ((nsteps - 1 - j) % 2 == 0) ? y : tmp;
        const int *ain = amax ? amax + (size_t)i * B : nullptr;
        int *aout = amax ? amax + (size_t)(last + 1) * B : nullptr;
#ifdef VQVAE_NO_PAIR_POST
        const bool with_post = false;
#else
        const bool with_post = pair && post && j == nsteps - 1 && res_pair_post_supported(C, post->Cout);
#endif
        const int rc = pair ? res_pair_forward_impl(cur, w1, w2, B, H, W, C, Rh, flags, dst, st, ain, aout, with_post ? post : nullptr)
                            : res_layer_forward_impl(cur, w1, w2, B, H, W, C, Rh, flags, dst, st, ain, aout, nullptr, hid_scratch);
        if (with_post && post_done) *post_done = true;
        if (rc != 0) return rc;
        cur = dst;
        i = last + 1;
    }
    *out = cur;
    return 0;
}

size_t res_hidden_bytes(const VqvaeDims *d, int64_t B, int H, int W) {
    if (d->n_res_layers < 1 || res_layer_fused_ok(d->h_dim, d->res_h_dim)) return 0;
    return align_up((size_t)B * (H / 4) * (W / 4) * d->res_h_dim * sizeof(float), 256);
}

size_t amax_bytes(const VqvaeDims *d, int64_t B) { return align_up((size_t)(4 + d->n_res_layers) * B * sizeof(int), 256); }

int conv_scheme(int flags) {
    const int sel = flags & (VQVAE_FWD_CONV_BF16_SPLIT | VQVAE_FWD_CONV_EXACT_FP32);
    if (sel == (VQVAE_FWD_CONV_BF16_SPLIT | VQVAE_FWD_CONV_EXACT_FP32)) return -1;
    return sel == VQVAE_FWD_CONV_BF16_SPLIT ? VQVAE_CONV_BF16_SPLIT : (sel == VQVAE_FWD_CONV_EXACT_FP32 ? VQVAE_CONV_EXACT_FP32 : 0);
}

struct FwdPlan {
    int cf;
    bool enc_front;
    bool enc_pair_post;
    bool dec_front;
    bool dec_tail;
    bool fused;
    bool vq_fuse;
    bool zq_amax;
};
FwdPlan fwd_plan(const VqvaeDims *d, int H, int W, int flags) {
    FwdPlan p{};
    p.cf = conv_scheme(flags);
    if (!dims_ok(d)) return p;
    const int h = d->h_dim, h4 = H / 4, w4 = W / 4;
    p.zq_amax = conv_reads_amax(VQVAE_CONVT_3x3_S1, h4, w4, d->embedding_dim, h, 0);
    if (p.cf != 0) return p;
#ifndef VQVAE_NO_ENC_FRONT_FUSION
    p.enc_front = enc_front_supported(H, W, d->in_ch, h / 2, h);
#endif
#ifndef VQVAE_NO_FRONT_FUSION
    p.enc_pair_post = d->n_res_layers == 2 && conv_res_pair_supported(VQVAE_CONV_3x3_S1, h4, w4, h, h, d->res_h_dim) &&
                      res_pair_post_supported(h, d->embedding_dim);
    p.dec_front = d->n_res_layers == 2 && conv_res_pair_supported(VQVAE_CONVT_3x3_S1, h4, w4, d->embedding_dim, h, d->res_h_dim);
#endif
#ifndef VQVAE_NO_DEC_TAIL_FUSION
    p.dec_tail = dec_tail_supported(h4, w4, h, h / 2, d->in_ch);
#endif
    p.fused = p.enc_front && p.enc_pair_post && p.dec_front && p.dec_tail;
    p.vq_fuse = p.fused && vq_fuse_ok(d->n_embeddings, d->embedding_dim, flags);
    return p;
}

__global__ __launch_bounds__(256) void decode_gather_kernel(const long long *__restrict__ idx, const float *__restrict__ codebook,
                                                            long long rows, int D, int K, float *__restrict__ z_q) {
    const long long total = rows * D;
    for (long long e = (long long)blockIdx.x * 256 + threadIdx.x; e < total; e += (long long)gridDim.x * 256) {
        const long long i = e / D;
        const int c = (int)(e - i * D);
        const long long k = idx[i];
        z_q[e] = (k >= 0 && k < K) ? codebook[(size_t)k * D + c] : __builtin_nanf("");
    }
}

}
}

using namespace vqvae;

extern "C" {

size_t vqvae_weights_packed_bytes(const VqvaeDims *d) {
    if (!dims_ok(d)) return 0;
    const int h = d->h_dim, D = d->embedding_dim, Rh = d->res_h_dim;
    size_t n = 0;
    const size_t parts[] = {
        vqvae_conv_in_packed_bytes(d->in_ch, h / 2), vqvae_conv_packed_bytes(VQVAE_CONV_4x4_S2, h / 2, h),
        vqvae_conv_packed_bytes(VQVAE_CONV_3x3_S1, h, h), vqvae_conv_packed_bytes(VQVAE_CONV_3x3_S1, h, Rh),
        vqvae_conv_packed_bytes(VQVAE_CONV_1x1, Rh, h), vqvae_conv_packed_bytes(VQVAE_CONV_1x1, h, D),
        vqvae_conv_packed_bytes(VQVAE_CONVT_3x3_S1, D, h), vqvae_conv_packed_bytes(VQVAE_CONV_3x3_S1, h, Rh),
        vqvae_conv_packed_bytes(VQVAE_CONV_1x1, Rh, h), vqvae_conv_packed_bytes(VQVAE_CONVT_4x4_S2, h, h / 2),
        vqvae_convt_out_packed_bytes(h / 2, d->in_ch)};
    for (size_t b : parts) {
        if (b == 0) return 0;
        n += align_up(b, 256);
    }
    return n;
}

int vqvae_weights_pack_f32(const VqvaeDims *d, const VqvaeRawWeights *raw, void *packed, size_t packed_bytes,
                           VqvaeWeights *out, vqvae_stream_t stream) {
    if (!d || !raw || !packed || !out) return VQVAE_ERR_NULL;
    const size_t need = vqvae_weights_packed_bytes(d);
    if (need == 0) return VQVAE_ERR_UNSUPPORTED;
    if (packed_bytes < need) return VQVAE_ERR_WORKSPACE;
    const float *req[] = {raw->enc0_w, raw->enc0_b, raw->enc2_w, raw->enc2_b, raw->enc4_w, raw->enc4_b, raw->enc_res_w1,
                          raw->enc_res_w2, raw->pre_w, raw->pre_b, raw->codebook, raw->dec0_w, raw->dec0_b, raw->dec_res_w1,
                          raw->dec_res_w2, raw->dec2_w, raw->dec2_b, raw->dec4_w, raw->dec4_b};
    for (const float *q : req)
        if (!q) return VQVAE_ERR_NULL;
    const int h = d->h_dim, D = d->embedding_dim, Rh = d->res_h_dim;
    Carve c{static_cast<char *>(packed), packed_bytes};
    int rc;
#define PACK_CONV(dst, kind, w, Cin, Cout)                                                          \
    do {                                                                                            \
        float *buf = static_cast<float *>(c.raw(vqvae_conv_packed_bytes(kind, Cin, Cout)));         \
        if (!c.ok) return VQVAE_ERR_WORKSPACE;                                                      \
        if ((rc = vqvae_conv_pack_f32(kind, w, Cin, Cout, buf, stream)) != 0) return rc;            \
        out->dst = buf;                                                                             \
    } while (0)
    {
        float *buf = static_cast<float *>(c.raw(vqvae_conv_in_packed_bytes(d->in_ch, h / 2)));
        if (!c.ok) return VQVAE_ERR_WORKSPACE;
        if ((rc = vqvae_conv_in_pack_f32(raw->enc0_w, d->in_ch, h / 2, buf, stream)) != 0) return rc;
        out->enc0 = buf;
    }
    PACK_CONV(enc2, VQVAE_CONV_4x4_S2, raw->enc2_w, h / 2, h);
    PACK_CONV(enc4, VQVAE_CONV_3x3_S1, raw->enc4_w, h, h);
    PACK_CONV(enc_res_w1, VQVAE_CONV_3x3_S1, raw->enc_res_w1, h, Rh);
    PACK_CONV(enc_res_w2, VQVAE_CONV_1x1, raw->enc_res_w2, Rh, h);
    PACK_CONV(pre, VQVAE_CONV_1x1, raw->pre_w, h, D);
    PACK_CONV(dec0, VQVAE_CONVT_3x3_S1, raw->dec0_w, D, h);
    PACK_CONV(dec_res_w1, VQVAE_CONV_3x3_S1, raw->dec_res_w1, h, Rh);
    PACK_CONV(dec_res_w2, VQVAE_CONV_1x1, raw->dec_res_w2, Rh, h);
    PACK_CONV(dec2, VQVAE_CONVT_4x4_S2, raw->dec2_w, h, h / 2);
#undef PACK_CONV
    {
        float *buf = static_cast<float *>(c.raw(vqvae_convt_out_packed_bytes(h / 2, d->in_ch)));
        if (!c.ok) return VQVAE_ERR_WORKSPACE;
        if ((rc = vqvae_convt_out_pack_f32(raw->dec4_w, h / 2, d->in_ch, buf, stream)) != 0) return rc;
        out->dec4 = buf;
    }
    out->dims = *d;
    out->enc0_b = raw->enc0_b; out->enc2_b = raw->enc2_b; out->enc4_b = raw->enc4_b; out->pre_b = raw->pre_b;
    out->dec0_b = raw->dec0_b; out->dec2_b = raw->dec2_b; out->dec4_b = raw->dec4_b;
    out->codebook = raw->codebook;
    return VQVAE_OK;
}

int vqvae_weights_range_check_f32(const VqvaeDims *d, const VqvaeRawWeights *raw, float *spread_log2_host, int *recommended_flags,
                                  void *scratch_device, size_t scratch_bytes, vqvae_stream_t stream) {
    if (!d || !raw || !recommended_flags || !scratch_device) return VQVAE_ERR_NULL;
    if (!dims_ok(d)) return VQVAE_ERR_UNSUPPORTED;
    if (scratch_bytes < 16 * sizeof(float)) return VQVAE_ERR_WORKSPACE;
    const int h = d->h_dim, D = d->embedding_dim, Rh = d->res_h_dim;
    struct Lay { const float *w; int Cout, Cin, taps; bool transposed; };
    const Lay lay[11] = {{raw->enc0_w, h / 2, d->in_ch, 16, false}, {raw->enc2_w, h, h / 2, 16, false}, {raw->enc4_w, h, h, 9, false},
                         {raw->enc_res_w1, Rh, h, 9, false},         {raw->enc_res_w2, h, Rh, 1, false},  {raw->pre_w, D, h, 1, false},
                         {raw->dec0_w, h, D, 9, true},               {raw->dec_res_w1, Rh, h, 9, false},  {raw->dec_res_w2, h, Rh, 1, false},
                         {raw->dec2_w, h / 2, h, 16, true},          {raw->dec4_w, d->in_ch, h / 2, 16, true}};
    hipStream_t st = static_cast<hipStream_t>(stream);
    float *out = static_cast<float *>(scratch_device);
    for (int i = 0; i < 11; ++i) {
        if (!lay[i].w) return VQVAE_ERR_NULL;
        if (d->n_res_layers == 0 && (i == 3 || i == 4 || i == 7 || i == 8)) { weight_spread_impl(nullptr, 0, 0, 0, false, out + i, st); continue; }
        if (lay[i].Cout > 1024 || lay[i].Cin > 1024) return VQVAE_ERR_UNSUPPORTED;
        weight_spread_impl(lay[i].w, lay[i].Cout, lay[i].Cin, lay[i].taps, lay[i].transposed, out + i, st);
    }
    float host[11];
    hipError_t e = hipMemcpyAsync(host, out, sizeof(host), hipMemcpyDeviceToHost, st);
    if (e == hipSuccess) e = hipStreamSynchronize(st);
    if (e != hipSuccess) return (int)e;
    float worst = 0.0f;
    for (int i = 1; i < 11; ++i) worst = host[i] > worst ? host[i] : worst;
    if (spread_log2_host) for (int i = 0; i < 11; ++i) spread_log2_host[i] = host[i];
    *recommended_flags = worst > VQVAE_RANGE_SPREAD_LIMIT_LOG2 ? VQVAE_FWD_CONV_BF16_SPLIT : 0;
    return VQVAE_OK;
}

size_t vqvae_workspace_ze_offset(const VqvaeDims *d, int64_t B, int H, int W) {
    if (vqvae_workspace_bytes(d, B, H, W) == 0) return 0;
    return 2 * align_up(act_elems(d, B, H, W) * sizeof(float), 256) + 2 * amax_bytes(d, B);
}

size_t vqvae_workspace_bytes(const VqvaeDims *d, int64_t B, int H, int W) {
    if (!dims_ok(d) || B < 1 || H < 4 || W < 4 || H % 4 || W % 4) return 0;
    const size_t vq = vqvae_vq_workspace_bytes(B * (int64_t)(H / 4) * (W / 4), d->n_embeddings, d->embedding_dim);
    if (vq == 0) return 0;
    const size_t act = align_up(act_elems(d, B, H, W) * sizeof(float), 256);
    const size_t lat = align_up((size_t)B * (H / 4) * (W / 4) * d->embedding_dim * sizeof(float), 256);
    const size_t rows = (size_t)B * (H / 4) * (W / 4);
    return 2 * act + 2 * amax_bytes(d, B) + 2 * lat + align_up(rows * sizeof(int64_t), 256) +
           align_up((size_t)d->n_embeddings * sizeof(int32_t), 256) + align_up(vq, 256) + 256 + res_hidden_bytes(d, B, H, W);
}

int vqvae_resstack_f32(const float *packed_w1, const float *packed_w2, const float *x, int64_t B, int H, int W, int C,
                       int Rh, int n_layers, int flags, float *y, float *tmp, vqvae_stream_t stream) {
    if (!packed_w1 || !packed_w2 || !x || !y) return VQVAE_ERR_NULL;
    if (n_layers > 1 && !tmp) return VQVAE_ERR_NULL;
    if (n_layers < 1) return VQVAE_ERR_SHAPE;
    const float *res = nullptr;
    return res_stack(packed_w1, packed_w2, x, B, H, W, C, Rh, n_layers, flags & VQVAE_CONV_RELU_IN, flags & VQVAE_CONV_RELU_OUT,
                     y, tmp, static_cast<hipStream_t>(stream), &res);
}

static int encoder_run(const VqvaeWeights *w, const float *x, int64_t B, int H, int W, float *z_e, void *workspace,
                       size_t workspace_bytes, hipStream_t st, const FwdPlan &p, int *am_given, int *zero_buf = nullptr, int zero_n = 0,
                       bool *zeroed = nullptr, const VqFuse *vq = nullptr, float *hid_given = nullptr, bool debug_ze = false) {
    if (!w || !x || !z_e || !workspace) return VQVAE_ERR_NULL;
    const VqvaeDims *d = &w->dims;
    if (!dims_ok(d) || B < 1 || H < 4 || W < 4 || H % 4 || W % 4) return VQVAE_ERR_SHAPE;
    Carve c{static_cast<char *>(workspace), workspace_bytes};
    const size_t act = act_elems(d, B, H, W);
    float *a = c.f32(act), *b = c.f32(act);
    if (!c.ok) return VQVAE_ERR_WORKSPACE;
    float *hid = hid_given;
    if (!hid && res_hidden_bytes(d, B, H, W)) {
        hid = static_cast<float *>(c.raw(res_hidden_bytes(d, B, H, W)));
        if (!c.ok) return VQVAE_ERR_WORKSPACE;
    }
    int *am = am_given;
    if (!am) {
        am = static_cast<int *>(c.raw(amax_bytes(d, B)));
        if (am && !p.fused && hipMemsetAsync(am, 0xFF, amax_bytes(d, B), st) != hipSuccess) am = nullptr;
    }
    int *am0 = am, *am1 = am ? am + B : nullptr, *am2 = am ? am + 2 * B : nullptr;
    const int h = d->h_dim, cf = p.cf;
    int rc;
    if (p.enc_front) {
        if ((rc = enc_front_forward_impl(x, w->enc0, w->enc0_b, w->enc2, w->enc2_b, B, H, W, d->in_ch, h / 2, h, b, st, am1,
                                         vq ? zero_buf : nullptr, vq ? zero_n : 0)) != 0) return rc;
    } else {
        if ((rc = conv_in_forward_impl(x, w->enc0, w->enc0_b, B, H, W, d->in_ch, h / 2, VQVAE_CONV_RELU_OUT | cf, a, st, am0)) != 0) return rc;
        if ((rc = conv_forward_impl(VQVAE_CONV_4x4_S2, a, w->enc2, w->enc2_b, B, H / 2, W / 2, h / 2, h, VQVAE_CONV_RELU_OUT | cf, b, st, am0, am1)) != 0) return rc;
    }
    if (p.enc_pair_post) {
        const ResPairPost post{w->pre, w->pre_b, d->embedding_dim, z_e, vq ? nullptr : zero_buf, vq ? 0 : zero_n, vq, vq && debug_ze};
        if (zeroed) *zeroed = zero_buf != nullptr;
        return conv_res_pair_forward_impl(VQVAE_CONV_3x3_S1, b, w->enc4, w->enc4_b, h, w->enc_res_w1, w->enc_res_w2, B, H / 4, W / 4, h,
                                          d->res_h_dim, VQVAE_CONV_RELU_OUT, nullptr, st, am1, nullptr, &post);
    }
    if ((rc = conv_forward_impl(VQVAE_CONV_3x3_S1, b, w->enc4, w->enc4_b, B, H / 4, W / 4, h, h, VQVAE_CONV_RELU_OUT | cf, a, st, am1, am2)) != 0) return rc;
    const float *t = a;
    const int *amt = am2;
    if (d->n_res_layers > 0) {
        float *y = (d->n_res_layers & 1) ? b : a, *tmp = (d->n_res_layers & 1) ? a : b;
        const ResPairPost post{w->pre, w->pre_b, d->embedding_dim, z_e};
        bool post_done = false;
        if ((rc = res_stack(w->enc_res_w1, w->enc_res_w2, a, B, H / 4, W / 4, h, d->res_h_dim, d->n_res_layers, false, true, y, tmp, st, &t, am2,
                            &post, &post_done, cf, hid)) != 0)
            return rc;
        if (post_done) return 0;
        if (am2) amt = am2 + (size_t)d->n_res_layers * B;
        if (!res_layer_fused_ok(h, d->res_h_dim)) amt = nullptr;
    }
    return conv_forward_impl(VQVAE_CONV_1x1, t, w->pre, w->pre_b, B, H / 4, W / 4, h, d->embedding_dim, cf, z_e, st, amt, nullptr);
}

int vqvae_encoder_ex_f32(const VqvaeWeights *w, const float *x, int64_t B, int H, int W, int flags, float *z_e, void *workspace,
                         size_t workspace_bytes, vqvae_stream_t stream) {
    const FwdPlan p = fwd_plan(w ? &w->dims : nullptr, H, W, flags);
    if (p.cf < 0 || (flags & ~(VQVAE_FWD_CONV_BF16_SPLIT | VQVAE_FWD_CONV_EXACT_FP32))) return VQVAE_ERR_UNSUPPORTED;
    return encoder_run(w, x, B, H, W, z_e, workspace, workspace_bytes, static_cast<hipStream_t>(stream), p, nullptr);
}

int vqvae_encoder_f32(const VqvaeWeights *w, const float *x, int64_t B, int H, int W, float *z_e, void *workspace,
                      size_t workspace_bytes, vqvae_stream_t stream) {
    return vqvae_encoder_ex_f32(w, x, B, H, W, 0, z_e, workspace, workspace_bytes, stream);
}

static int *zq_amax_slot(const VqvaeDims *d, int64_t B, int *am) { return am + (size_t)(2 + d->n_res_layers) * B; }
static int decoder_run(const VqvaeWeights *w, const float *z_q, int64_t B, int h4, int w4, float *x_hat, void *workspace,
                       size_t workspace_bytes, hipStream_t st, const FwdPlan &p, int *am_given, bool zq_amax_given = false,
                       float *hid_given = nullptr, const int64_t *gather_idx = nullptr) {
    if (!w || !z_q || !x_hat || !workspace) return VQVAE_ERR_NULL;
    const VqvaeDims *d = &w->dims;
    if (!dims_ok(d) || B < 1 || h4 < 1 || w4 < 1) return VQVAE_ERR_SHAPE;
    Carve c{static_cast<char *>(workspace), workspace_bytes};
    const size_t act = act_elems(d, B, 4 * h4, 4 * w4);
    float *a = c.f32(act), *b = c.f32(act);
    if (!c.ok) return VQVAE_ERR_WORKSPACE;
    float *hid = hid_given;
    if (!hid && res_hidden_bytes(d, B, 4 * h4, 4 * w4)) {
        hid = static_cast<float *>(c.raw(res_hidden_bytes(d, B, 4 * h4, 4 * w4)));
        if (!c.ok) return VQVAE_ERR_WORKSPACE;
    }
    int *am = am_given;
    if (!am) {
        am = static_cast<int *>(c.raw(amax_bytes(d, B)));
        if (am && !p.fused && hipMemsetAsync(am, 0xFF, amax_bytes(d, B), st) != hipSuccess) am = nullptr;
    }
    const int h = d->h_dim, cf = p.cf;
    int rc;
    if (gather_idx && !p.dec_front) return VQVAE_ERR_UNSUPPORTED;
    int *amz = nullptr;
    if (am && !gather_idx && p.zq_amax) {
        amz = zq_amax_slot(d, B, am);
        if (!zq_amax_given) act_absmax_impl(z_q, B, (long long)h4 * w4 * d->embedding_dim, amz, st);
    }
    const float *t = a;
    const int *amt = am;
    if (p.dec_front) {
        int *aout = am ? am + (size_t)2 * B : nullptr;
        if ((rc = conv_res_pair_forward_impl(VQVAE_CONVT_3x3_S1, z_q, w->dec0, w->dec0_b, d->embedding_dim, w->dec_res_w1, w->dec_res_w2, B, h4,
                                             w4, h, d->res_h_dim, VQVAE_CONV_RELU_OUT, a, st, amz, aout, nullptr, gather_idx,
                                             d->n_embeddings)) != 0) return rc;
        amt = aout;
    } else if ((rc = conv_forward_impl(VQVAE_CONVT_3x3_S1, z_q, w->dec0, w->dec0_b, B, h4, w4, d->embedding_dim, h, VQVAE_CONV_RELU_OUT | cf, a, st, amz, am)) != 0) return rc;
    if (!p.dec_front && d->n_res_layers > 0) {
        float *y = (d->n_res_layers & 1) ? b : a, *tmp = (d->n_res_layers & 1) ? a : b;
        if ((rc = res_stack(w->dec_res_w1, w->dec_res_w2, a, B, h4, w4, h, d->res_h_dim, d->n_res_layers, false, true, y, tmp, st, &t, am,
                            nullptr, nullptr, cf, hid)) != 0) return rc;
        if (am) amt = am + (size_t)d->n_res_layers * B;
        if (!res_layer_fused_ok(h, d->res_h_dim)) amt = nullptr;
    }
    if (p.dec_tail)
        return dec_tail_forward_impl(t, w->dec2, w->dec2_b, w->dec4, w->dec4_b, B, h4, w4, h, h / 2, d->in_ch, x_hat, st, amt);
    float *u = (t == a) ? b : a;
    int *am_u = am ? am + (size_t)(3 + d->n_res_layers) * B : nullptr;
    if ((rc = conv_forward_impl(VQVAE_CONVT_4x4_S2, t, w->dec2, w->dec2_b, B, h4, w4, h, h / 2, VQVAE_CONV_RELU_OUT | cf, u, st, amt, am_u)) != 0) return rc;
    return convt_out_forward_impl(u, w->dec4, w->dec4_b, B, 2 * h4, 2 * w4, h / 2, d->in_ch, cf, x_hat, st, am_u);
}

int vqvae_decoder_ex_f32(const VqvaeWeights *w, const float *z_q, int64_t B, int h4, int w4, int flags, float *x_hat, void *workspace,
                         size_t workspace_bytes, vqvae_stream_t stream) {
    const FwdPlan p = fwd_plan(w ? &w->dims : nullptr, 4 * h4, 4 * w4, flags);
    if (p.cf < 0 || (flags & ~(VQVAE_FWD_CONV_BF16_SPLIT | VQVAE_FWD_CONV_EXACT_FP32))) return VQVAE_ERR_UNSUPPORTED;
    return decoder_run(w, z_q, B, h4, w4, x_hat, workspace, workspace_bytes, static_cast<hipStream_t>(stream), p, nullptr);
}

int vqvae_decoder_f32(const VqvaeWeights *w, const float *z_q, int64_t B, int h4, int w4, float *x_hat, void *workspace,
                      size_t workspace_bytes, vqvae_stream_t stream) {
    return vqvae_decoder_ex_f32(w, z_q, B, h4, w4, 0, x_hat, workspace, workspace_bytes, stream);
}

}

namespace {
struct FwdWs {
    void *acts; size_t act, rows; int *am2; float *z_e, *z_q; int64_t *idx_ws; int32_t *hist; void *vqws; size_t vqws_bytes;
    float *hid;
};
int carve_forward(const VqvaeDims *d, int64_t B, int H, int W, void *workspace, size_t workspace_bytes, void *vq_workspace,
                  size_t vq_workspace_bytes, int &vq_flags, FwdWs &f, bool with_vq = true) {
    const size_t need = vqvae_workspace_bytes(d, B, H, W);
    if (need == 0) return VQVAE_ERR_UNSUPPORTED;
    if (workspace_bytes < need) return VQVAE_ERR_WORKSPACE;
    Carve c{static_cast<char *>(workspace), workspace_bytes};
    f.act = act_elems(d, B, H, W);
    f.rows = (size_t)B * (H / 4) * (W / 4);
    f.acts = c.raw(2 * align_up(f.act * sizeof(float), 256));
    f.am2 = static_cast<int *>(c.raw(2 * amax_bytes(d, B)));
    f.z_e = c.f32(f.rows * d->embedding_dim);
    f.z_q = c.f32(f.rows * d->embedding_dim);
    f.idx_ws = static_cast<int64_t *>(c.raw(f.rows * sizeof(int64_t)));
    f.hist = static_cast<int32_t *>(c.raw((size_t)d->n_embeddings * sizeof(int32_t)));
    const size_t vqb = vqvae_vq_workspace_bytes((int64_t)f.rows, d->n_embeddings, d->embedding_dim);
    f.vqws = vq_workspace;
    f.vqws_bytes = vq_workspace_bytes;
    if (!f.vqws && with_vq) {
        f.vqws = c.raw(vqb);
        f.vqws_bytes = vqb;
        vq_flags &= ~VQVAE_VQ_CODEBOOK_PREPARED;
    }
    f.hid = res_hidden_bytes(d, B, H, W) ? static_cast<float *>(c.raw(res_hidden_bytes(d, B, H, W))) : nullptr;
    return c.ok ? VQVAE_OK : VQVAE_ERR_WORKSPACE;
}
}

extern "C" {

int vqvae_forward_f32(const VqvaeWeights *w, const float *x, int64_t B, int H, int W, int vq_flags, float *x_hat,
                      float *loss, float *perplexity, int64_t *idx, void *workspace, size_t workspace_bytes,
                      void *vq_workspace, size_t vq_workspace_bytes, vqvae_stream_t stream) {
    if (!w || !x || !x_hat || !loss || !perplexity || !workspace) return VQVAE_ERR_NULL;
    const VqvaeDims *d = &w->dims;
    FwdWs f;
    {
        const int crc = carve_forward(d, B, H, W, workspace, workspace_bytes, vq_workspace, vq_workspace_bytes, vq_flags, f);
        if (crc != VQVAE_OK) return crc;
    }
    const size_t act = f.act, rows = f.rows;
    void *acts = f.acts;
    int *am2 = f.am2;
    float *z_e = f.z_e, *z_q = f.z_q;
    int64_t *idx_ws = f.idx_ws;
    int32_t *hist = f.hist;
    void *vqws = f.vqws;
    const size_t vqws_bytes = f.vqws_bytes;
    const size_t acts_bytes = 2 * align_up(act * sizeof(float), 256);
    hipStream_t st = static_cast<hipStream_t>(stream);
    const FwdPlan p = fwd_plan(d, H, W, vq_flags);
    if (p.cf < 0) return VQVAE_ERR_UNSUPPORTED;
    if (!p.fused && hipMemsetAsync(am2, 0xFF, 2 * amax_bytes(d, B), st) != hipSuccess) return VQVAE_ERR_WORKSPACE;
    int *am_dec = reinterpret_cast<int *>(reinterpret_cast<char *>(am2) + amax_bytes(d, B));
    int rc;
    bool hist_zeroed = false;
    if (p.vq_fuse && !(vq_flags & kVqFormFlags)) {
        if ((rc = vq_prepare_impl(w->codebook, d->n_embeddings, d->embedding_dim, vq_flags, vqws, vqws_bytes, st)) != 0) return rc;
        VqFuse vf = vq_fuse_args(w->codebook, d->n_embeddings, vqws, z_q, idx ? idx : idx_ws, hist);
        vf.partials = reinterpret_cast<double *>(z_e);
        const bool debug_ze = vq_flags & VQVAE_FWD_DEBUG_ZE;
        if (debug_ze && !idx) return VQVAE_ERR_NULL;
        if (debug_ze) vf.partials = reinterpret_cast<double *>(idx_ws);
        if ((rc = encoder_run(w, x, B, H, W, z_e, acts, acts_bytes, st, p, am2, hist, d->n_embeddings, &hist_zeroed, &vf, nullptr,
                              debug_ze)) != 0) return rc;
        if ((rc = vq_finalize_impl(vf.partials, (int)((B + 3) / 4), hist, d->n_embeddings, (int64_t)rows, d->embedding_dim, d->beta, loss,
                                   perplexity, st)) != 0) return rc;
        return decoder_run(w, z_q, B, H / 4, W / 4, x_hat, acts, acts_bytes, st, p, am_dec);
    }
    bool zq_amax_done = false;
    if ((rc = encoder_run(w, x, B, H, W, z_e, acts, acts_bytes, st, p, am2, p.fused ? hist : nullptr, d->n_embeddings, &hist_zeroed,
                          nullptr, f.hid)) != 0)
        return rc;
    if ((rc = vq_forward_impl(z_e, w->codebook, B, d->embedding_dim, H / 4, W / 4, d->n_embeddings, d->beta,
                              (vq_flags & (VQVAE_VQ_CODEBOOK_PREPARED | VQVAE_VQ_EXACT_SWEEP | VQVAE_VQ_BF16_FILTER |
                                           VQVAE_VQ_REMOVED_FLAGS | kVqFormFlags)) | VQVAE_VQ_ROWMAJOR,
                              z_q, idx ? idx : idx_ws, hist, loss, perplexity, vqws, vqws_bytes, stream, hist_zeroed,
                              p.zq_amax ? zq_amax_slot(d, B, am_dec) : nullptr, &zq_amax_done)) != 0) return rc;
    return decoder_run(w, z_q, B, H / 4, W / 4, x_hat, acts, acts_bytes, st, p, am_dec, zq_amax_done, f.hid);
}


int vqvae_encode_f32(const VqvaeWeights *w, const float *x, int64_t B, int H, int W, int vq_flags, int64_t *idx, void *workspace,
                     size_t workspace_bytes, void *vq_workspace, size_t vq_workspace_bytes, vqvae_stream_t stream) {
    if (!w || !x || !idx || !workspace) return VQVAE_ERR_NULL;
    const VqvaeDims *d = &w->dims;
    FwdWs f;
    {
        const int crc = carve_forward(d, B, H, W, workspace, workspace_bytes, vq_workspace, vq_workspace_bytes, vq_flags, f);
        if (crc != VQVAE_OK) return crc;
    }
    hipStream_t st = static_cast<hipStream_t>(stream);
    const FwdPlan p = fwd_plan(d, H, W, vq_flags);
    if (p.cf < 0) return VQVAE_ERR_UNSUPPORTED;
    const size_t acts_bytes = 2 * align_up(f.act * sizeof(float), 256);
    if (!p.fused && hipMemsetAsync(f.am2, 0xFF, 2 * amax_bytes(d, B), st) != hipSuccess) return VQVAE_ERR_WORKSPACE;
    int rc;
    bool hist_zeroed = false;
    if (p.vq_fuse && !(vq_flags & kVqFormFlags)) {
        if ((rc = vq_prepare_impl(w->codebook, d->n_embeddings, d->embedding_dim, vq_flags, f.vqws, f.vqws_bytes, st)) != 0) return rc;
        VqFuse vf = vq_fuse_args(w->codebook, d->n_embeddings, f.vqws, nullptr, idx, f.hist);
        vf.partials = reinterpret_cast<double *>(f.z_e);
        return encoder_run(w, x, B, H, W, f.z_e, f.acts, acts_bytes, st, p, f.am2, f.hist, d->n_embeddings, &hist_zeroed, &vf);
    }
    if ((rc = encoder_run(w, x, B, H, W, f.z_e, f.acts, acts_bytes, st, p, f.am2, p.fused ? f.hist : nullptr, d->n_embeddings, &hist_zeroed,
                          nullptr, f.hid)) != 0) return rc;
    float *scal = reinterpret_cast<float *>(f.idx_ws);
    return vq_forward_impl(f.z_e, w->codebook, B, d->embedding_dim, H / 4, W / 4, d->n_embeddings, d->beta,
                           (vq_flags & (VQVAE_VQ_CODEBOOK_PREPARED | VQVAE_VQ_EXACT_SWEEP | VQVAE_VQ_BF16_FILTER | VQVAE_VQ_REMOVED_FLAGS |
                                        kVqFormFlags)) | VQVAE_VQ_ROWMAJOR,
                           f.z_q, idx, f.hist, scal, scal + 1, f.vqws, f.vqws_bytes, stream, hist_zeroed, nullptr, nullptr);
}

int vqvae_decode_f32(const VqvaeWeights *w, const int64_t *idx, int64_t B, int h4, int w4, int flags, float *x_hat, void *workspace,
                     size_t workspace_bytes, vqvae_stream_t stream) {
    if (!w || !idx || !x_hat || !workspace) return VQVAE_ERR_NULL;
    const VqvaeDims *d = &w->dims;
    const FwdPlan p = fwd_plan(d, 4 * h4, 4 * w4, flags);
    if (p.cf < 0 || (flags & ~(VQVAE_FWD_CONV_BF16_SPLIT | VQVAE_FWD_CONV_EXACT_FP32))) return VQVAE_ERR_UNSUPPORTED;
    if (!dims_ok(d) || B < 1 || h4 < 1 || w4 < 1) return VQVAE_ERR_SHAPE;
    FwdWs f;
    int vq_flags = VQVAE_VQ_CODEBOOK_PREPARED;
    {
        const int crc = carve_forward(d, B, 4 * h4, 4 * w4, workspace, workspace_bytes, workspace, 0, vq_flags, f, false);
        if (crc != VQVAE_OK) return crc;
    }
    hipStream_t st = static_cast<hipStream_t>(stream);
    const size_t acts_bytes = 2 * align_up(f.act * sizeof(float), 256);
    int *am_dec = reinterpret_cast<int *>(reinterpret_cast<char *>(f.am2) + amax_bytes(d, B));
    if (!p.fused && hipMemsetAsync(am_dec, 0xFF, amax_bytes(d, B), st) != hipSuccess) return VQVAE_ERR_WORKSPACE;
    if (p.dec_front)
        return decoder_run(w, w->codebook, B, h4, w4, x_hat, f.acts, acts_bytes, st, p, am_dec, false, f.hid, idx);
    {
        const long long total = (long long)f.rows * d->embedding_dim;
        const long long blocks = (total + 255) / 256;
        hipLaunchKernelGGL(decode_gather_kernel, dim3((unsigned)(blocks < 65536 ? blocks : 65536)), dim3(256), 0, st,
                           reinterpret_cast<const long long *>(idx), w->codebook, (long long)f.rows, d->embedding_dim, d->n_embeddings,
                           f.z_q);
        const int lrc = (int)hipGetLastError();
        if (lrc != 0) return lrc;
    }
    return decoder_run(w, f.z_q, B, h4, w4, x_hat, f.acts, acts_bytes, st, p, am_dec, false, f.hid);
}

int vqvae_forward_begin_f32(const VqvaeWeights *w, int64_t B, int H, int W, int vq_flags, void *workspace, size_t workspace_bytes,
                            void *vq_workspace, size_t vq_workspace_bytes, vqvae_stream_t stream) {
    if (!w || !workspace) return VQVAE_ERR_NULL;
    const VqvaeDims *d = &w->dims;
    FwdWs f;
    int rc = carve_forward(d, B, H, W, workspace, workspace_bytes, vq_workspace, vq_workspace_bytes, vq_flags, f);
    if (rc != VQVAE_OK) return rc;
    if (!fwd_plan(d, H, W, vq_flags).vq_fuse) return VQVAE_ERR_UNSUPPORTED;
    hipStream_t st = static_cast<hipStream_t>(stream);
    if ((rc = vq_prepare_impl(w->codebook, d->n_embeddings, d->embedding_dim, vq_flags, f.vqws, f.vqws_bytes, st)) != 0) return rc;
    if (hipMemsetAsync(f.hist, 0, (size_t)d->n_embeddings * sizeof(int32_t), st) != hipSuccess) return VQVAE_ERR_WORKSPACE;
    {
        std::lock_guard<std::mutex> lk(g_parts_mu);
        g_parts[workspace] = PartsRecord{B, H, W, vq_flags, vq_workspace, {}};
    }
    return VQVAE_OK;
}

int vqvae_forward_part_f32(const VqvaeWeights *w, const float *x, int64_t B, int64_t b0, int64_t Bc, int H, int W, int vq_flags,
                           float *x_hat, int64_t *idx, void *workspace, size_t workspace_bytes, void *vq_workspace,
                           size_t vq_workspace_bytes, vqvae_stream_t stream) {
    if (!w || !x || !x_hat || !workspace) return VQVAE_ERR_NULL;
    const VqvaeDims *d = &w->dims;
    if (B < 1 || b0 < 0 || Bc < 1 || b0 + Bc > B || b0 % 64 || (b0 + Bc < B && Bc % 64)) return VQVAE_ERR_SHAPE;
    FwdWs f;
    int rc = carve_forward(d, B, H, W, workspace, workspace_bytes, vq_workspace, vq_workspace_bytes, vq_flags, f);
    if (rc != VQVAE_OK) return rc;
    const FwdPlan p = fwd_plan(d, H, W, vq_flags);
    if (!p.vq_fuse) return VQVAE_ERR_UNSUPPORTED;
    {
        std::lock_guard<std::mutex> lk(g_parts_mu);
        auto it = g_parts.find(workspace);
        if (it == g_parts.end()) return VQVAE_ERR_SHAPE;
        PartsRecord &r = it->second;
        if (r.B != B || r.H != H || r.W != W || r.flags != vq_flags || r.vqws != vq_workspace) return VQVAE_ERR_SHAPE;
        for (const auto &c : r.claimed)
            if (b0 < c.second && c.first < b0 + Bc) return VQVAE_ERR_SHAPE;
        r.claimed.emplace_back(b0, b0 + Bc);
    }
    hipStream_t st = static_cast<hipStream_t>(stream);
    const size_t per_img = f.act / (size_t)B, lat = (size_t)(H / 4) * (W / 4);
    char *acts_p = static_cast<char *>(f.acts) + 2 * (size_t)b0 * per_img * sizeof(float);
    const size_t acts_p_bytes = 2 * align_up((size_t)Bc * per_img * sizeof(float), 256);
    const size_t am_ints = (size_t)(4 + d->n_res_layers);
    int *am_p = f.am2 + 2 * am_ints * (size_t)b0;
    int *am_dec_p = reinterpret_cast<int *>(reinterpret_cast<char *>(am_p) + amax_bytes(d, Bc));
    float *z_q_p = f.z_q + (size_t)b0 * lat * d->embedding_dim;
    int64_t *idx_p = (idx ? idx : f.idx_ws) + (size_t)b0 * lat;
    VqFuse vf = vq_fuse_args(w->codebook, d->n_embeddings, f.vqws, z_q_p, idx_p, f.hist);
    vf.partials = reinterpret_cast<double *>(f.z_e) + b0 / 4;
    const float *x_p = x + (size_t)b0 * d->in_ch * H * W;
    rc = encoder_run(w, x_p, Bc, H, W, f.z_e, acts_p, acts_p_bytes, st, p, am_p, nullptr, 0, nullptr, &vf);
    if (rc == 0) rc = decoder_run(w, z_q_p, Bc, H / 4, W / 4, x_hat + (size_t)b0 * d->in_ch * H * W, acts_p, acts_p_bytes, st, p, am_dec_p);
    if (rc != 0) {
        std::lock_guard<std::mutex> lk(g_parts_mu);
        auto it = g_parts.find(workspace);
        if (it != g_parts.end()) {
            auto &cl = it->second.claimed;
            for (size_t i = 0; i < cl.size(); ++i)
                if (cl[i].first == b0 && cl[i].second == b0 + Bc) { cl.erase(cl.begin() + (long)i); break; }
        }
    }
    return rc;
}

int vqvae_forward_abort_f32(void *workspace) {
    std::lock_guard<std::mutex> lk(g_parts_mu);
    g_parts.erase(workspace);
    return VQVAE_OK;
}

int vqvae_forward_end_f32(const VqvaeWeights *w, int64_t B, int H, int W, float *loss, float *perplexity, void *workspace,
                          size_t workspace_bytes, vqvae_stream_t stream) {
    if (!w || !loss || !perplexity || !workspace) return VQVAE_ERR_NULL;
    const VqvaeDims *d = &w->dims;
    FwdWs f;
    int flags = 0;
    int rc = carve_forward(d, B, H, W, workspace, workspace_bytes, nullptr, 0, flags, f, false);
    if (rc != VQVAE_OK) return rc;
    {
        std::lock_guard<std::mutex> lk(g_parts_mu);
        auto it = g_parts.find(workspace);
        if (it == g_parts.end() || it->second.B != B || it->second.H != H || it->second.W != W) return VQVAE_ERR_SHAPE;
        int64_t covered = 0;
        for (const auto &c : it->second.claimed) covered += c.second - c.first;
        if (covered != B) return VQVAE_ERR_SHAPE;
        g_parts.erase(it);
    }
    return vq_finalize_impl(reinterpret_cast<const double *>(f.z_e), (int)((B + 3) / 4), f.hist, d->n_embeddings, (int64_t)f.rows,
                            d->embedding_dim, d->beta, loss, perplexity, static_cast<hipStream_t>(stream));
}

}
```

### vqvae_amd/csrc/vq_exact.hip

```cpp
#include "common.h"
#include "vq_device.h"

namespace vqvae {

template <int D>
__global__ __launch_bounds__(64) void vq_prepare_kernel(const float *__restrict__ cb, int K, int KC,
                                                        int K_pad, float *__restrict__ ee,
                                                        float *__restrict__ img,
                                                        int *__restrict__ flags, int K32,
                                                        unsigned short *__restrict__ img16,
                                                        float *__restrict__ neh) {
    const int k = blockIdx.x * 64 + threadIdx.x;
    if (k >= K_pad && k >= K32) return;
    if (k >= K_pad) {
        for (int c = 0; c < D; ++c) img16[(((c % (D / 2)) / 8 * 2 + c / (D / 2)) * (size_t)K32 + k) * 8 + (c & 7)] = 0;
        neh[k] = -__builtin_inff();
        return;
    }
    const int ch = k / KC, kl = k - ch * KC;
    float *dst = img + (size_t)ch * KC * D;
    float e[D];
    if (k < K) {
#pragma unroll
        for (int c = 0; c < D; c += 4) {
            const f32x4 v = *reinterpret_cast<const f32x4 *>(cb + (size_t)k * D + c);
            e[c] = v.x; e[c + 1] = v.y; e[c + 2] = v.z; e[c + 3] = v.w;
        }
    } else {
#pragma unroll
        for (int c = 0; c < D; ++c) e[c] = 0.0f;
    }
#pragma unroll
    for (int c = 0; c < D; ++c) {
        const int j = c >> 3, i = (c & 7) >> 1, h = c & 1;
        dst[((size_t)(j * 2 + h) * KC + kl) * 4 + i] = e[c];
    }
    float n2 = __builtin_inff();
    if (k < K) {
        float sq[D];
#pragma unroll
        for (int c = 0; c < D; ++c) sq[c] = e[c] * e[c];
        n2 = aten_sqsum_full<D>(sq);
        if (!(n2 < 1.0e38f)) atomicOr(flags, 1);
        atomicMax(flags + 1, __float_as_int(n2));
        float am = 0.0f;
#pragma unroll
        for (int c = 0; c < D; ++c) am = fmaxf(am, __builtin_fabsf(e[c]));
        atomicMax(flags + 2, __float_as_int(am));
    }
    ee[k] = n2;
    if (k < K32) {
#pragma unroll
        for (int c = 0; c < D; ++c) {
            const unsigned u = __float_as_uint(e[c]);
            const unsigned r = (u + 0x7FFFu + ((u >> 16) & 1u)) >> 16;
            const unsigned short bf = (e[c] != e[c]) ? 0x7FC0 : (unsigned short)r;
            img16[(((c % (D / 2)) / 8 * 2 + c / (D / 2)) * (size_t)K32 + k) * 8 + (c & 7)] = bf;
        }
        neh[k] = k < K ? -0.5f * n2 : -__builtin_inff();
    }
}

template <int D, int RT, bool DO_MFMA, bool DO_ARG>
__device__ __forceinline__ void vq_tile_step(const float *__restrict__ ap, size_t jstride,
                                             const float (&zr)[RT][D / 2], f32x16 (&accM)[RT],
                                             const float *__restrict__ ee_t, int code0,
                                             const f32x16 (&accA)[RT], const float (&zz)[RT],
                                             float (&bd)[RT], int (&bk)[RT]) {
    constexpr int NJ = D / 8;
    if (DO_MFMA) {
#pragma unroll
        for (int t = 0; t < RT; ++t)
#pragma unroll
            for (int r = 0; r < 16; ++r) accM[t][r] = 0.0f;
    }
    f32x4 e4 = {0.0f, 0.0f, 0.0f, 0.0f};
#pragma unroll
    for (int j = 0; j < NJ; ++j) {
        if (DO_MFMA) {
            const f32x4 a = *reinterpret_cast<const f32x4 *>(ap + (size_t)j * jstride);
#pragma unroll
            for (int i = 0; i < 4; ++i)
#pragma unroll
                for (int t = 0; t < RT; ++t)
                    accM[t] = __builtin_amdgcn_mfma_f32_32x32x2f32(a[i], zr[t][4 * j + i], accM[t], 0, 0, 0);
        }
        if (DO_ARG) {
            const int r0 = (16 * j) / NJ, r1 = (16 * (j + 1)) / NJ;
#pragma unroll
            for (int r = r0; r < r1; ++r) {
                if ((r & 3) == 0) e4 = *reinterpret_cast<const f32x4 *>(ee_t + 8 * (r >> 2));
                const int code = code0 + 8 * (r >> 2) + (r & 3);
#pragma unroll
                for (int t = 0; t < RT; ++t) {
                    const float tt = zz[t] + e4[r & 3];
                    const float d = __builtin_fmaf(-2.0f, accA[t][r], tt);
                    const bool lt = d < bd[t];
                    bd[t] = lt ? d : bd[t];
                    bk[t] = lt ? code : bk[t];
                }
            }
        }
    }
}

template <int D, int RT, bool ROWMAJOR>
__global__ __launch_bounds__(512, 2) void vq_exact_kernel(
    const float *__restrict__ z, const float *__restrict__ cb, const float *__restrict__ img,
    const float *__restrict__ ee_g, const int *__restrict__ flags, long long N, int HW, int K,
    int KC, int nchunks, long long nblocks, float *__restrict__ zq, long long *__restrict__ idx,
    int *__restrict__ hist, double *__restrict__ partials) {
    constexpr int S = D / 2;
    constexpr int ROWS_WG = 8 * 32 * RT;
    extern __shared__ __attribute__((aligned(16))) float smem[];
    float *Es = smem;
    float *ee_s = Es + (size_t)KC * D;
    int *hist_s = reinterpret_cast<int *>(ee_s + KC);
    double *red = reinterpret_cast<double *>(hist_s + ((K + 1) & ~1));

    const int tid = threadIdx.x;
    const int lane = tid & 63, wave = tid >> 6;
    const int l31 = lane & 31, h = lane >> 5;
    const int wave_u = __builtin_amdgcn_readfirstlane(wave);
    const int cb_bad = flags[0];
    for (int k = tid; k < K; k += 512) hist_s[k] = 0;

    auto stage = [&](int ch) {
        const f32x4 *src = reinterpret_cast<const f32x4 *>(img + (size_t)ch * KC * D);
        f32x4 *dst = reinterpret_cast<f32x4 *>(Es);
        const int n4 = KC * D / 4;
        for (int i = tid; i < n4; i += 512) dst[i] = src[i];
        for (int i = tid; i < KC; i += 512) ee_s[i] = ee_g[ch * KC + i];
    };
    if (nchunks == 1) stage(0);
    __syncthreads();

    double dacc = 0.0;

    for (long long rb = blockIdx.x; rb < nblocks; rb += gridDim.x) {
        float zr[RT][S];
        float zz[RT];
        long long row[RT];
        size_t zbase[RT];
        size_t img0[RT];
        unsigned voff[RT];
        bool valid[RT];
#pragma unroll
        for (int t = 0; t < RT; ++t) {
            row[t] = rb * ROWS_WG + wave * (32 * RT) + t * 32 + l31;
            valid[t] = row[t] < N;
            const long long rc = valid[t] ? row[t] : N - 1;
            if (ROWMAJOR) {
                zbase[t] = (size_t)rc * D;
#pragma unroll
                for (int q = 0; q < D / 4; ++q) {
                    const f32x4 v = *reinterpret_cast<const f32x4 *>(z + zbase[t] + 4 * q);
                    zr[t][2 * q] = h ? v.y : v.x;
                    zr[t][2 * q + 1] = h ? v.w : v.z;
                }
            } else {
                const long long r0 = rb * ROWS_WG + wave_u * (32 * RT) + t * 32;
                const long long b0 = (r0 < N ? r0 : N - 1) / HW;
                const long long b = rc / HW;
                const int hw = (int)(rc - b * HW);
                zbase[t] = (size_t)b * D * HW + hw;
                img0[t] = (size_t)b0 * D * HW;
                voff[t] = (unsigned)((((b - b0) * D + h) * HW + hw) * 4);
                const auto rs = make_rsrc(z + img0[t]);
#pragma unroll
                for (int s = 0; s < S; ++s)
                    zr[t][s] = __builtin_bit_cast(
                        float, __builtin_amdgcn_raw_buffer_load_b32(rs, voff[t], (unsigned)(2 * s) * HW * 4u, 0));
            }
        }
#pragma unroll
        for (int t = 0; t < RT; ++t) {
            constexpr int NV = D / 8, NI = NV / 4;
            float A[4];
#pragma unroll
            for (int u = 0; u < 4; ++u) {
                float P[4] = {0.0f, 0.0f, 0.0f, 0.0f};
#pragma unroll
                for (int i = 0; i < NI; ++i)
#pragma unroll
                    for (int q = 0; q < 4; ++q) {
                        const float x = zr[t][4 * (4 * i + q) + u];
                        P[q] = P[q] + x * x;
                    }
#pragma unroll
                for (int v = NI * 4; v < NV; ++v) {
                    const float x = zr[t][4 * v + u];
                    P[0] = P[0] + x * x;
                }
                A[u] = ((P[0] + P[1]) + P[2]) + P[3];
            }
            float fin = 0.0f;
#pragma unroll
            for (int u = 0; u < 4; ++u) {
                const float other = __shfl_xor(A[u], 32);
                const float ev = h ? other : A[u];
                const float od = h ? A[u] : other;
                fin = fin + ev;
                fin = fin + od;
            }
            zz[t] = fin;
        }

        float bd[RT];
        int bk[RT];
#pragma unroll
        for (int t = 0; t < RT; ++t) { bd[t] = __builtin_inff(); bk[t] = 0; }

        for (int ch = 0; ch < nchunks; ++ch) {
            if (nchunks > 1) {
                __syncthreads();
                stage(ch);
                __syncthreads();
            }
            const int ncode = min(KC, K - ch * KC);
            const int ntile = (ncode + 31) >> 5;
            const size_t jstride = (size_t)2 * KC * 4;
            const float *ap0 = Es + ((size_t)h * KC + l31) * 4;
            const float *ee0 = ee_s + 4 * h;
            const int cbase = ch * KC + 4 * h;
            f32x16 accA[RT], accB[RT];
            vq_tile_step<D, RT, true, false>(ap0, jstride, zr, accA, ee0, cbase, accB, zz, bd, bk);
            int ct = 1;
            for (; ct + 1 < ntile; ct += 2) {
                vq_tile_step<D, RT, true, true>(ap0 + ct * 128, jstride, zr, accB, ee0 + (ct - 1) * 32,
                                                cbase + (ct - 1) * 32, accA, zz, bd, bk);
                vq_tile_step<D, RT, true, true>(ap0 + (ct + 1) * 128, jstride, zr, accA, ee0 + ct * 32,
                                                cbase + ct * 32, accB, zz, bd, bk);
            }
            if (ct < ntile) {
                vq_tile_step<D, RT, true, true>(ap0 + ct * 128, jstride, zr, accB, ee0 + (ct - 1) * 32,
                                                cbase + (ct - 1) * 32, accA, zz, bd, bk);
                vq_tile_step<D, RT, false, true>(ap0, jstride, zr, accA, ee0 + ct * 32, cbase + ct * 32, accB, zz,
                                                 bd, bk);
            } else {
                vq_tile_step<D, RT, false, true>(ap0, jstride, zr, accB, ee0 + (ct - 1) * 32,
                                                 cbase + (ct - 1) * 32, accA, zz, bd, bk);
            }
        }

#pragma unroll
        for (int t = 0; t < RT; ++t) {
            const float pd = __shfl_xor(bd[t], 32);
            const int pk = __shfl_xor(bk[t], 32);
            const bool take = (pd < bd[t]) || (pd == bd[t] && pk < bk[t]);
            int k = take ? pk : bk[t];

            const bool bad = valid[t] && (cb_bad || !(zz[t] < 1.0e38f));
            if (__any(bad)) {
                int ks = 0;
                if (bad && h == 0)
                    ks = vq_slow_argmin<D, ROWMAJOR>(z, zbase[t], ROWMAJOR ? 1 : (size_t)HW, cb, ee_g,
                                                     K, zz[t]);
                ks = __shfl(ks, l31);
                if (bad) k = ks;
            }

            float sq = 0.0f;
            const float *e = cb + (size_t)k * D;
#pragma unroll
            for (int s = 0; s < S; ++s) {
                const float ev = e[2 * s + h];
                const float diff = ev - zr[t][s];
                sq = sq + diff * diff;
                zr[t][s] = zr[t][s] + diff;
            }
            if (valid[t]) {
                dacc += (double)sq;
                if (zq) {
                    if (ROWMAJOR) {
#pragma unroll
                        for (int q = 0; q < D / 4; ++q) {
                            const float o0 = __shfl_xor(zr[t][2 * q], 32);
                            const float o1 = __shfl_xor(zr[t][2 * q + 1], 32);
                            if ((q & 1) == h) {
                                f32x4 v;
                                v.x = h ? o0 : zr[t][2 * q];
                                v.y = h ? zr[t][2 * q] : o0;
                                v.z = h ? o1 : zr[t][2 * q + 1];
                                v.w = h ? zr[t][2 * q + 1] : o1;
                                *reinterpret_cast<f32x4 *>(zq + zbase[t] + 4 * q) = v;
                            }
                        }
                    }
                }
                if (h == 0) {
                    idx[row[t]] = k;
                    atomicAdd(&hist_s[k], 1);
                }
            }
            if (!ROWMAJOR && zq && valid[t]) {
                const auto rs = make_rsrc(zq + img0[t]);
#pragma unroll
                for (int s = 0; s < S; ++s)
                    __builtin_amdgcn_raw_buffer_store_b32(__builtin_bit_cast(unsigned, zr[t][s]), rs,
                                                          voff[t], (unsigned)(2 * s) * HW * 4u, 0);
            }
        }
    }

#pragma unroll
    for (int o = 32; o > 0; o >>= 1) dacc += __shfl_xor(dacc, o);
    __syncthreads();
    if (lane == 0) red[wave] = dacc;
    __syncthreads();
    if (tid == 0) {
        double s = 0.0;
        for (int w = 0; w < 8; ++w) s += red[w];
        partials[blockIdx.x] = s;
    }
    for (int k = tid; k < K; k += 512) {
        const int c = hist_s[k];
        if (c) atomicAdd(&hist[k], c);
    }
}

__global__ __launch_bounds__(256) void vq_finalize_kernel(const double *__restrict__ partials, int nparts,
                                                          const int *__restrict__ hist, int K,
                                                          long long N, int D, float beta,
                                                          float *__restrict__ loss,
                                                          float *__restrict__ perplexity) {
    __shared__ double red[256];
    const int tid = threadIdx.x;
    double s = 0.0;
    const float fn = (float)N;
    for (int k = tid; k < K; k += 256) {
        const float p = (float)hist[k] / fn;
        const float lg = (float)log((double)(p + 1e-10f));
        s += (double)(p * lg);
    }
    red[tid] = s;
    __syncthreads();
    for (int o = 128; o > 0; o >>= 1) {
        if (tid < o) red[tid] += red[tid + o];
        __syncthreads();
    }
    const double ent = red[0];
    __syncthreads();
    double q = 0.0;
    for (int i = tid; i < nparts; i += 256) q += partials[i];
    red[tid] = q;
    __syncthreads();
    for (int o = 128; o > 0; o >>= 1) {
        if (tid < o) red[tid] += red[tid + o];
        __syncthreads();
    }
    if (tid == 0) {
        *perplexity = (float)exp(-(double)(float)ent);
        const float m = (float)(red[0] / ((double)N * (double)D));
        const float bm = beta * m;
        *loss = m + bm;
    }
}

__global__ __launch_bounds__(256) void vq_onehot_kernel(const long long *__restrict__ idx, long long N,
                                                        int K, float *__restrict__ onehot) {
    const long long total = N * (long long)K;
    for (long long i = (long long)blockIdx.x * 256 + threadIdx.x; i < total;
         i += (long long)gridDim.x * 256) {
        const long long n = i / K;
        const int k = (int)(i - n * K);
        onehot[i] = idx[n] == k ? 1.0f : 0.0f;
    }
}

__global__ __launch_bounds__(256) void vq_decode_indices_kernel(const long long *__restrict__ idx,
                                                                const float *__restrict__ cb,
                                                                long long total, int D, int HW, int K,
                                                                float *__restrict__ zq) {
    for (long long i = (long long)blockIdx.x * 256 + threadIdx.x; i < total;
         i += (long long)gridDim.x * 256) {
        const int hw = (int)(i % HW);
        const long long bc = i / HW;
        const int c = (int)(bc % D);
        const long long b = bc / D;
        const long long k = idx[b * HW + hw];
        zq[i] = (k >= 0 && k < K) ? cb[(size_t)k * D + c] : __builtin_nanf("");
    }
}

template <int D>
static int launch_vq_prepare(const float *cb, int K, char *ws, hipStream_t st) {
    const VqPlan p = vq_plan(K, D);
    int *wflags = reinterpret_cast<int *>(ws + p.off_flags);
    hipError_t e;
    if ((e = hipMemsetAsync(wflags, 0, 256 + kVqTicketBytes, st)) != hipSuccess) return (int)e;
    const int kmax = p.K_pad > p.K32 ? p.K_pad : p.K32;
    hipLaunchKernelGGL(vq_prepare_kernel<D>, dim3((kmax + 63) / 64), dim3(64), 0, st, cb, K, p.KC, p.K_pad,
                       reinterpret_cast<float *>(ws + p.off_ee), reinterpret_cast<float *>(ws + p.off_img), wflags, p.K32,
                       reinterpret_cast<unsigned short *>(ws + p.off_img16), reinterpret_cast<float *>(ws + p.off_neh));
    const VqRoute r = vq_route(K, D, 0, VQVAE_VQ_ROWMAJOR);
    if (r == VqRoute::Track || r == VqRoute::Chunk) launch_vq_prepare16(cb, K, D, ws, st);
    return (int)hipGetLastError();
}

template <int D>
static int launch_vq(VqRoute route, const float *z, const float *cb, long long N, int HW, int K, float beta,
                     int flags, float *zq, long long *idx, int *hist, float *loss, float *ppl,
                     char *ws, hipStream_t st, bool hist_zeroed, int *zq_amax, bool *zq_amax_done) {
    const VqPlan p = vq_plan(K, D);
    int *wflags = reinterpret_cast<int *>(ws + p.off_flags);
    float *ee = reinterpret_cast<float *>(ws + p.off_ee);
    float *img = reinterpret_cast<float *>(ws + p.off_img);
    double *partials = reinterpret_cast<double *>(ws + p.off_partials);

    hipError_t e;
    if (!hist_zeroed && (e = hipMemsetAsync(hist, 0, sizeof(int) * (size_t)K, st)) != hipSuccess) return (int)e;
    if (!(flags & VQVAE_VQ_CODEBOOK_PREPARED)) {
        const int rc = launch_vq_prepare<D>(cb, K, ws, st);
        if (rc != 0) return rc;
    }
    const bool rowmajor = flags & VQVAE_VQ_ROWMAJOR;
    const bool timed = route != VqRoute::Track && route != VqRoute::TrackNchw;
    if (timed) prof_begin(VQVAE_PROF_VQ_MAIN, st);
    int fgrid = 0, rc = 0;
    switch (route) {
        case VqRoute::Track:
        case VqRoute::TrackNchw:
            rc = launch_vq_track_d64(z, cb, N, K, zq, idx, hist, ws, st, &fgrid, HW, route == VqRoute::TrackNchw, vq_form_of_flags(flags));
            break;
        case VqRoute::Chunk:
            rc = launch_vq_chunked(z, cb, N, K, D, zq, idx, hist, ws, st, &fgrid, zq_amax, HW);
            if (zq_amax_done) *zq_amax_done = zq_amax != nullptr && zq != nullptr;
            break;
        case VqRoute::Filter:
            rc = launch_vq_filter_d64(z, cb, N, HW, K, rowmajor, zq, idx, hist, ws, st, &fgrid);
            break;
        default: {
            const int cus = num_cus();
            int rt = (D <= 64 && (N + 511) / 512 >= 2LL * cus) ? 2 : 1;
            const long long rows_wg = 256LL * rt;
            const long long nblocks = (N + rows_wg - 1) / rows_wg;
            long long grid = nblocks < cus ? nblocks : cus;
            if (grid > kVqMaxGrid) grid = kVqMaxGrid;
            fgrid = (int)grid;
#define VQ_LAUNCH(RT_, RM_)                                                                        \
    do {                                                                                           \
        auto kfn = vq_exact_kernel<D, RT_, RM_>;                                                   \
                           \
            (void)hipFuncSetAttribute(reinterpret_cast<const void *>(kfn),                             \
                                hipFuncAttributeMaxDynamicSharedMemorySize, kLdsBytes);            \
        hipLaunchKernelGGL(kfn, dim3((unsigned)grid), dim3(512), p.lds_bytes, st, z, cb, img, ee,  \
                           wflags, N, HW, K, p.KC, p.nchunks, nblocks, zq, idx, hist, partials);   \
    } while (0)
            if (rt == 2) {
                if constexpr (D <= 64) {
                    if (rowmajor) VQ_LAUNCH(2, true); else VQ_LAUNCH(2, false);
                }
            } else {
                if (rowmajor) VQ_LAUNCH(1, true); else VQ_LAUNCH(1, false);
            }
#undef VQ_LAUNCH
        }
    }
    if (timed) prof_end(VQVAE_PROF_VQ_MAIN, st);
    if (rc != 0) return rc;
    hipLaunchKernelGGL(vq_finalize_kernel, dim3(1), dim3(256), 0, st, partials, fgrid, hist, K, N, D, beta, loss, ppl);
    return (int)hipGetLastError();
}

static bool vq_mfma_dim(int D) { return D == 32 || D == 64 || D == 128 || D == 256; }

VqRoute vq_route(int K, int D, int HW, int flags) {
    if (K < 1 || K > 16384 || (flags & VQVAE_VQ_REMOVED_FLAGS)) return VqRoute::Unsupported;
    if (!vq_mfma_dim(D)) return !vq_generic_ok(K, D) ? VqRoute::Unsupported
                                                      : ((flags & VQVAE_VQ_BF16_FILTER) ? VqRoute::GenericVector : VqRoute::AnyD);
    const bool rowmajor = flags & VQVAE_VQ_ROWMAJOR;
    const bool screen = !(flags & (VQVAE_VQ_EXACT_SWEEP | VQVAE_VQ_BF16_FILTER));
    if (screen && rowmajor && vq_track_ok(K, D)) return VqRoute::Track;
    if (screen && !rowmajor && vq_track_nchw_ok(K, D, HW)) return VqRoute::TrackNchw;
    if (screen && rowmajor && vq_chunk_ok(K, D)) return VqRoute::Chunk;
    if (D == 64 && !(flags & VQVAE_VQ_EXACT_SWEEP) && vq_filter_lds_bytes(K, D) <= (size_t)kLdsBytes) return VqRoute::Filter;
    return VqRoute::Exact;
}

}

using namespace vqvae;

extern "C" {

const char *vqvae_vq_kernel_name(int K, int D, int flags) {
    static const char *const names[] = {"vq_track_kernel_d64", "vq_track_kernel_d64", "vq_stream_sweep_kernel", "vq_filter_kernel_d64",
                                        "vq_exact_kernel", "vq_anyd_kernel", "vq_generic_kernel", "unsupported"};
    return names[(int)vq_route(K, D, 64, flags)];
}

int vqvae_vq_launch_form(int64_t n_rows, int K, int D, int HW, int flags, int *waves, int *unit_rows, int *pool_pct) {
    if (n_rows < 1 || K < 1 || HW < 1) return VQVAE_ERR_SHAPE;
    const VqRoute r = vq_route(K, D, HW, flags);
    VqTrackForm f;
    if ((r != VqRoute::Track && r != VqRoute::TrackNchw) ||
        !vq_track_form(n_rows, K, HW, r == VqRoute::TrackNchw, vq_form_of_flags(flags), num_cus(), f))
        return VQVAE_ERR_UNSUPPORTED;
    if (waves) *waves = f.waves;
    if (unit_rows) *unit_rows = f.unit_rows;
    if (pool_pct) *pool_pct = f.pool_pct;
    return VQVAE_OK;
}

int vqvae_vq_screen_sweeps(int K, int D, int flags) {
    const VqRoute r = vq_route(K, D, 64, flags);
    return (r == VqRoute::Track || r == VqRoute::TrackNchw || r == VqRoute::Chunk) ? 1 : (r == VqRoute::Filter ? 2 : 0);
}

size_t vqvae_vq_workspace_bytes(int64_t n_rows, int K, int D) {
    (void)n_rows;
    const VqRoute r = vq_route(K, D, 0, VQVAE_VQ_ROWMAJOR);
    return r == VqRoute::Unsupported ? 0 : (r == VqRoute::AnyD ? vq_generic_workspace_bytes(K, D) : vq_plan(K, D).total);
}

int vqvae_vq_forward_f32(const float *z_e, const float *codebook, int64_t B, int D, int H, int W,
                         int K, float beta, int flags, float *z_q, int64_t *idx, int32_t *hist,
                         float *loss, float *perplexity, void *workspace, size_t workspace_bytes,
                         vqvae_stream_t stream) {
    return vqvae::vq_forward_impl(z_e, codebook, B, D, H, W, K, beta, flags, z_q, idx, hist, loss, perplexity, workspace,
                                  workspace_bytes, stream, false);
}
}

bool vqvae::vq_fuse_ok(int K, int D, int flags) {
    return vq_route(K, D, 0, (flags & ~VQVAE_VQ_REMOVED_FLAGS) | VQVAE_VQ_ROWMAJOR) == VqRoute::Track && (K + 31) / 32 % 4 == 0 &&
           !(flags & VQVAE_VQ_UNFUSED);
}

int vqvae::vq_prepare_impl(const float *codebook, int K, int D, int flags, void *workspace, size_t workspace_bytes, hipStream_t st) {
    if (!codebook || !workspace) return VQVAE_ERR_NULL;
    if (D != 64 || K < 1 || K > 16384) return VQVAE_ERR_UNSUPPORTED;
    if (workspace_bytes < vqvae_vq_workspace_bytes(0, K, D)) return VQVAE_ERR_WORKSPACE;
    if (flags & VQVAE_VQ_CODEBOOK_PREPARED) return VQVAE_OK;
    return launch_vq_prepare<64>(codebook, K, static_cast<char *>(workspace), st);
}

vqvae::VqFuse vqvae::vq_fuse_args(const float *codebook, int K, void *workspace, float *z_q, int64_t *idx, int32_t *hist) {
    const VqPlan p = vq_plan(K, 64);
    char *ws = static_cast<char *>(workspace);
    VqFuse f;
    f.imgf = reinterpret_cast<const uint4 *>(ws + p.off_imgf);
    f.seeds = reinterpret_cast<const float *>(ws + p.off_seeds);
    f.ee = reinterpret_cast<const float *>(ws + p.off_ee);
    f.flags = reinterpret_cast<const int *>(ws + p.off_flags);
    f.cb = codebook;
    f.K = K;
    f.K32 = p.K32;
    f.zq = z_q;
    f.idx = reinterpret_cast<long long *>(idx);
    f.hist = hist;
    f.partials = reinterpret_cast<double *>(ws + p.off_partials);
    return f;
}

int vqvae::vq_finalize_impl(const double *partials, int grid, int32_t *hist, int K, int64_t n_rows, int D, float beta, float *loss,
                            float *perplexity, hipStream_t st) {
    hipLaunchKernelGGL(vq_finalize_kernel, dim3(1), dim3(256), 0, st, partials, grid, hist, K, (long long)n_rows, D, beta, loss, perplexity);
    return (int)hipGetLastError();
}

int vqvae::vq_forward_impl(const float *z_e, const float *codebook, int64_t B, int D, int H, int W,
                           int K, float beta, int flags, float *z_q, int64_t *idx, int32_t *hist,
                           float *loss, float *perplexity, void *workspace, size_t workspace_bytes,
                           vqvae_stream_t stream, bool hist_zeroed, int *zq_amax, bool *zq_amax_done) {
    if (zq_amax_done) *zq_amax_done = false;
    if (!z_e || !codebook || !idx || !hist || !loss || !perplexity) return VQVAE_ERR_NULL;
    if (B < 1 || D < 1 || H < 1 || W < 1 || K < 1) return VQVAE_ERR_SHAPE;
    if (vq_route(K, D, 0, flags & ~VQVAE_VQ_REMOVED_FLAGS) == VqRoute::Unsupported) return VQVAE_ERR_UNSUPPORTED;
    if ((int64_t)H * W > (int64_t)1 << 30) return VQVAE_ERR_OVERFLOW;
    const int64_t N = B * (int64_t)H * W;
    if (N / ((int64_t)H * W) != B || N > ((int64_t)1 << 40)) return VQVAE_ERR_OVERFLOW;
    const int HW = H * W;
    const VqRoute route = vq_route(K, D, HW, flags);
    if (route == VqRoute::Unsupported) return VQVAE_ERR_UNSUPPORTED;
    const size_t need = vqvae_vq_workspace_bytes(N, K, D);
    if (!workspace || workspace_bytes < need) return VQVAE_ERR_WORKSPACE;
    hipStream_t st = static_cast<hipStream_t>(stream);
    char *ws = static_cast<char *>(workspace);
    long long *idx_ll = reinterpret_cast<long long *>(idx);
    if (route == VqRoute::AnyD || route == VqRoute::GenericVector)
        return launch_vq_generic(z_e, codebook, N, HW, K, D, beta, (flags & VQVAE_VQ_ROWMAJOR) != 0, z_q, idx_ll, hist, loss, perplexity, ws, st,
                                 hist_zeroed, route == VqRoute::GenericVector, (flags & VQVAE_VQ_CODEBOOK_PREPARED) != 0);
    switch (D) {
        case 32:  return launch_vq<32>(route, z_e, codebook, N, HW, K, beta, flags, z_q, idx_ll, hist, loss, perplexity, ws, st, hist_zeroed, zq_amax, zq_amax_done);
        case 64:  return launch_vq<64>(route, z_e, codebook, N, HW, K, beta, flags, z_q, idx_ll, hist, loss, perplexity, ws, st, hist_zeroed, zq_amax, zq_amax_done);
        case 128: return launch_vq<128>(route, z_e, codebook, N, HW, K, beta, flags, z_q, idx_ll, hist, loss, perplexity, ws, st, hist_zeroed, zq_amax, zq_amax_done);
        case 256: return launch_vq<256>(route, z_e, codebook, N, HW, K, beta, flags, z_q, idx_ll, hist, loss, perplexity, ws, st, hist_zeroed, zq_amax, zq_amax_done);
    }
    return VQVAE_ERR_UNSUPPORTED;
}

extern "C" {

int vqvae_vq_onehot_f32(const int64_t *idx, int64_t N, int K, float *onehot, vqvae_stream_t stream) {
    if (!idx || !onehot) return VQVAE_ERR_NULL;
    if (N < 1 || K < 1) return VQVAE_ERR_SHAPE;
    if (N > INT64_MAX / K) return VQVAE_ERR_OVERFLOW;
    const long long total = N * (long long)K;
    long long grid = (total + 255) / 256;
    if (grid > 256 * 16) grid = 256 * 16;
    hipLaunchKernelGGL(vq_onehot_kernel, dim3((unsigned)grid), dim3(256), 0,
                       static_cast<hipStream_t>(stream), reinterpret_cast<const long long *>(idx), N, K,
                       onehot);
    return (int)hipGetLastError();
}

int vqvae_vq_decode_indices_f32(const int64_t *idx, const float *codebook, int64_t B, int D, int H,
                                int W, int K, float *z_q, vqvae_stream_t stream) {
    if (!idx || !codebook || !z_q) return VQVAE_ERR_NULL;
    if (B < 1 || D < 1 || H < 1 || W < 1 || K < 1) return VQVAE_ERR_SHAPE;
    const long long total = B * (long long)D * H * W;
    long long grid = (total + 255) / 256;
    if (grid > 256 * 16) grid = 256 * 16;
    hipLaunchKernelGGL(vq_decode_indices_kernel, dim3((unsigned)grid), dim3(256), 0,
                       static_cast<hipStream_t>(stream), reinterpret_cast<const long long *>(idx),
                       codebook, total, D, H * W, K, z_q);
    return (int)hipGetLastError();
}

}
```

### vqvae_amd/csrc/vq_unit.h

```cpp
#pragma once
#include "common.h"
#include "vq_track.h"

#ifndef VQ_ZQ_STORE_AUX
#define VQ_ZQ_STORE_AUX 0
#endif

namespace vqvae {
namespace vqu {

typedef unsigned u32x4v __attribute__((ext_vector_type(4)));

__device__ __forceinline__ void lds_order_wave() { asm volatile("" ::: "memory"); __builtin_amdgcn_wave_barrier(); }

struct Bound {
    int cb_bad;
    float A, Ehat, dE, EmaxS, EEh, EEa;
};

__device__ __forceinline__ Bound load_bound(const int *__restrict__ flags) {
    Bound b;
    b.cb_bad = flags[0];
    b.A = __builtin_ldexpf(1.0f, flags[5]);
    const float EEmax = __int_as_float(flags[1]) * 1.0001f;
    b.Ehat = __builtin_sqrtf(__int_as_float(flags[3])) * 1.0001f;
    b.dE = __builtin_sqrtf(__int_as_float(flags[4])) * 1.0001f;
    b.EmaxS = __builtin_sqrtf(EEmax) * b.A * 1.0001f;
    b.EEh = 0.5f * EEmax * b.A;
    b.EEa = EEmax * b.A;
    return b;
}

constexpr int kTabBytes = 1552;
struct Tables {
    unsigned *task_s;
    unsigned long long *best_s;
    float *zz_s;
    int *cnt_s;
};
__device__ __forceinline__ Tables tables(unsigned char *tab_s) {
    return Tables{reinterpret_cast<unsigned *>(tab_s), reinterpret_cast<unsigned long long *>(tab_s + 256),
                  reinterpret_cast<float *>(tab_s + 768), reinterpret_cast<int *>(tab_s + 1024)};
}

struct Flagged {
    bool o_open, o_hard, o_bad;
    unsigned long long fm, hmask;
    int ndirect;
};

__device__ __forceinline__ void rescan_tile(const f32x16 &acc, float thr_t, int ct, int t, int lane, int K, int ndirect, float ninf,
                                            const Tables &tb, int &nres) {
    const int l31 = lane & 31, h = lane >> 5;
    const float x0 = trk::max3(trk::max3(acc[0], acc[1], acc[2]), trk::max3(acc[3], acc[4], acc[5]), trk::max3(acc[6], acc[7], acc[8]));
    const float x1 = trk::max3(trk::max3(acc[9], acc[10], acc[11]), trk::max3(acc[12], acc[13], acc[14]), acc[15]);
    const float mx = trk::max3(x0, x1, ninf);
    if (__builtin_amdgcn_ballot_w64(mx >= thr_t)) {
#pragma unroll
        for (int r = 0; r < 16; ++r) {
            const int code = ct * 32 + (r & 3) + 8 * (r >> 2) + 4 * h;
            const bool hit = acc[r] >= thr_t && code < K;
            const unsigned long long b = __builtin_amdgcn_ballot_w64(hit);
            if (b) {
                const int sl = ndirect + nres + (int)__builtin_amdgcn_mbcnt_hi((unsigned)(b >> 32), __builtin_amdgcn_mbcnt_lo((unsigned)b, 0));
                if (hit && sl < 64) tb.task_s[sl] = (unsigned)(32 * t + l31) | ((unsigned)code << 6) | ((unsigned)code << 19);
                nres += __builtin_popcountll(b);
            }
        }
    }
}


struct BoundP {
    int cb_bad;
    float D2, D1, D0, T1, T0;
};

__device__ __forceinline__ BoundP load_boundp(const int *__restrict__ flags) {
    const Bound b = load_bound(flags);
    const float c1 = 4.89e-4f, c0 = 2.5e-7f, s = 1.00016f, q = (1.0f + c1) * s, up = 1.0002f;
    BoundP p;
    p.cb_bad = b.cb_bad;
    p.D2 = up * 2.002f * (1.2e-7f * b.A * q * q);
    p.D1 = up * 2.002f * (b.Ehat * (c1 * s) + b.dE * ((1.0f + 2.0f * c1) * s) + 7.76e-6f * b.Ehat * q + 3.86e-6f * b.EmaxS * q + 1.2e-7f * b.A * (2.0f * q * c0));
    p.D0 = up * 2.002f * (b.Ehat * c0 + 2.0f * b.dE * c0 + 7.76e-6f * (b.Ehat * c0 + b.EEh) + 3.86e-6f * b.EmaxS * c0 + 1.2e-7f * (b.A * c0 * c0 + b.EEa));
    p.T1 = 1.01f * 8.0e-6f * b.Ehat * q;
    p.T0 = 1.01f * 8.0e-6f * (b.Ehat * c0 + b.EEh);
    p.cb_bad = __builtin_amdgcn_readfirstlane(p.cb_bad);
    int d2, d1, d0, t1, t0;
    asm volatile("v_readfirstlane_b32 %0, %5\n\tv_readfirstlane_b32 %1, %6\n\tv_readfirstlane_b32 %2, %7\n\t"
                 "v_readfirstlane_b32 %3, %8\n\tv_readfirstlane_b32 %4, %9"
                 : "=s"(d2), "=s"(d1), "=s"(d0), "=s"(t1), "=s"(t0) : "v"(p.D2), "v"(p.D1), "v"(p.D0), "v"(p.T1), "v"(p.T0));
    p.D2 = __int_as_float(d2); p.D1 = __int_as_float(d1); p.D0 = __int_as_float(d0); p.T1 = __int_as_float(t1); p.T0 = __int_as_float(t0);
    return p;
}

template <int T>
struct RowsSp {
    int kbest;
    bool valid, bad, open, hard;
    unsigned long long openm, hardm;
    float thr[T];
    int ncls;
};

template <int T>
__device__ __forceinline__ void classify_sp(const trk::Lane (&L)[T], const float (&zn2)[T], const BoundP &B, int K, int lane, int nleft,
                                            float ninf, unsigned *task_s, RowsSp<T> &R) {
    const int l31 = lane & 31, h = lane >> 5;
    const unsigned gemask = trk::kGeBits | (((unsigned)lane & 32u) << 9);
    float v1[T];
    if constexpr (T == 1) {
        const float a = trk::lane_max(L[0], ninf);
        const auto sv = __builtin_amdgcn_permlane32_swap(__float_as_uint(a), __float_as_uint(a), false, false);
        v1[0] = trk::max2(__uint_as_float(sv[0]), __uint_as_float(sv[1]));
    } else {
        const float a0 = trk::lane_max(L[0], ninf), a1 = trk::lane_max(L[1], ninf);
        const auto sv = __builtin_amdgcn_permlane32_swap(__float_as_uint(a0), __float_as_uint(a1), false, false);
        const float m = trk::max2(__uint_as_float(sv[0]), __uint_as_float(sv[1]));
        const auto sw = __builtin_amdgcn_permlane32_swap(__float_as_uint(m), __float_as_uint(m), false, false);
        v1[0] = __uint_as_float(sw[0]);
        v1[1] = __uint_as_float(sw[1]);
    }
    unsigned ge[T], w[T];
    bool badl[T];
#pragma unroll
    for (int t = 0; t < T; ++t) {
        const float Z = __builtin_amdgcn_sqrtf(zn2[t]);
        const float delta = __builtin_fmaf(Z * B.D2 + B.D1, Z, B.D0);
        const float th = v1[t] - delta;
        const float thB = __builtin_fmaf(Z, -B.T1, th - B.T0);
        R.thr[t] = th;
        const float av = __builtin_fabsf(v1[t]);
        badl[t] = !(av < 1.0e37f) || !(delta < 1.0e37f) || av < 1.0e-30f;
        ge[t] = ~trk::lt_of(L[t], th, thB, ninf) & gemask;
        w[t] = trk::word_of(L[t], ge[t]);
    }
    unsigned Wlo, Whi;
    bool bad_sp;
    if constexpr (T == 1) {
        unsigned junk;
        asm volatile("" : "=v"(junk));
        const auto sv = __builtin_amdgcn_permlane32_swap(w[0], junk, false, false);
        Wlo = sv[0]; Whi = sv[1];
        bad_sp = badl[0];
    } else {
        const auto sv = __builtin_amdgcn_permlane32_swap(w[0], w[1], false, false);
        Wlo = sv[0]; Whi = sv[1];
        bad_sp = h ? badl[T - 1] : badl[0];
    }
    const trk::Spoken V = trk::spoken_of(Wlo, Whi);
    const bool closed = trk::spoken_closed(V, K);
    R.kbest = V.kbest;
    R.valid = lane < nleft;
    R.bad = R.valid && (bad_sp || B.cb_bad);
    R.open = false; R.hard = false; R.openm = 0ull; R.hardm = 0ull; R.ncls = 0;
    const bool nonclosed = R.valid && !R.bad && !closed;
    if (__builtin_amdgcn_ballot_w64(nonclosed)) {
        R.hard = nonclosed && trk::spoken_hard(V, K);
        R.open = nonclosed && !R.hard;
        R.openm = __builtin_amdgcn_ballot_w64(R.open);
        R.hardm = __builtin_amdgcn_ballot_w64(R.hard);
#pragma unroll
        for (int t = 0; t < T; ++t) {
            const unsigned om = (unsigned)(R.openm >> (32 * t));
            if (om) {
                const trk::Cands C = trk::cands2_of(L[t], ge[t], h, K);
                const int nt = ((om >> l31) & 1u) ? C.ntask : 0;
                const unsigned long long b1 = __builtin_amdgcn_ballot_w64(nt >= 1), b2 = __builtin_amdgcn_ballot_w64(nt >= 2);
                const int below = __builtin_amdgcn_mbcnt_hi((unsigned)(b1 >> 32), __builtin_amdgcn_mbcnt_lo((unsigned)b1, 0)) +
                                  __builtin_amdgcn_mbcnt_hi((unsigned)(b2 >> 32), __builtin_amdgcn_mbcnt_lo((unsigned)b2, 0));
                const int slot = R.ncls + below;
                const unsigned rowu = (unsigned)(32 * t + l31);
                if (nt >= 1 && slot < 64) task_s[slot] = rowu | ((unsigned)C.ta[0] << 6) | ((unsigned)C.tb[0] << 19);
                if (nt >= 2 && slot + 1 < 64) task_s[slot + 1] = rowu | ((unsigned)C.ta[1] << 6) | ((unsigned)C.tb[1] << 19);
                R.ncls += __builtin_popcountll(b1) + __builtin_popcountll(b2);
            }
        }
    }
}

template <int T>
__device__ __forceinline__ Flagged exact_begin_sp(const RowsSp<T> &R, int lane, const Tables &tb) {
    Flagged F;
    F.o_open = R.open; F.o_hard = R.hard; F.o_bad = R.bad;
    F.fm = __builtin_amdgcn_ballot_w64(R.open || R.hard || R.bad);
    F.hmask = 0ull;
    F.ndirect = R.ncls;
    if (F.fm) {
        const unsigned long long lowmask = (1ull << lane) - 1ull;
        unsigned ones;
        asm volatile("v_mov_b32 %0, -1" : "=v"(ones));
        reinterpret_cast<unsigned *>(tb.best_s)[2 * lane] = ones;
        reinterpret_cast<unsigned *>(tb.best_s)[2 * lane + 1] = ones;
        const unsigned long long tmb = __builtin_amdgcn_ballot_w64(F.o_bad);
        if (F.o_bad && R.ncls + __builtin_popcountll(tmb & lowmask) < 64) tb.task_s[R.ncls + __builtin_popcountll(tmb & lowmask)] = (unsigned)lane;
        F.ndirect = R.ncls + __builtin_popcountll(tmb);
        F.hmask = R.hardm;
        if (F.hmask && lane == 0) tb.cnt_s[0] = 0;
        lds_order_wave();
    }
    return F;
}

template <int T, class ZRow, class ZScalar>
__device__ __forceinline__ void exact_end_sp(RowsSp<T> &R, Flagged &F, int ntasks, int lane, const Tables &tb, const float *__restrict__ cb,
                                             const float *__restrict__ ee_g, int K, ZRow &&zrow, ZScalar &&zscalar) {
    constexpr int D = 64;
    if (!F.fm) return;
    const int j8 = lane & 7, g8 = lane >> 3;
    bool o_wide = F.o_bad;
    if (ntasks > 64) {
        const unsigned long long lowmask = (1ull << lane) - 1ull;
        const int nh = __builtin_popcountll(F.hmask);
        __builtin_amdgcn_wave_barrier();
        if (F.hmask && F.ndirect + nh <= 64) {
            if (F.o_hard) tb.task_s[F.ndirect + __builtin_popcountll(F.hmask & lowmask)] = (unsigned)lane;
            o_wide = o_wide || F.o_hard;
            ntasks = F.ndirect + nh;
        } else {
            o_wide = o_wide || F.o_open || F.o_hard;
            if (o_wide) tb.task_s[__builtin_popcountll(F.fm & lowmask)] = (unsigned)lane;
            ntasks = __builtin_popcountll(F.fm);
        }
    }
    lds_order_wave();
    const auto cb_rs = __builtin_amdgcn_make_buffer_rsrc(const_cast<float *>(cb), 0, (unsigned)K * (D * 4), 0x00020000);
    for (int base = 0; base < ntasks; base += 4) {
        const int jj = base + (g8 >> 1);
        const unsigned task = tb.task_s[jj < ntasks ? jj : 0];
        const int rr = (int)(task & 63u), ka = (int)((task >> 6) & 8191u), kb2 = (int)(task >> 19);
        const int kc = (g8 & 1) ? kb2 : ka;
        const f32x4 z0 = zrow(rr, 2 * j8), z1 = zrow(rr, 2 * j8 + 1);
        const f32x4 e0 = __builtin_bit_cast(f32x4, __builtin_amdgcn_raw_buffer_load_b128(cb_rs, (unsigned)kc * 256u + (unsigned)j8 * 32u, 0, 0));
        const f32x4 e1 = __builtin_bit_cast(f32x4, __builtin_amdgcn_raw_buffer_load_b128(cb_rs, (unsigned)kc * 256u + (unsigned)j8 * 32u + 16u, 0, 0));
        const float eek = ee_g[kc];
        const float sq[8] = {z0.x * z0.x, z0.y * z0.y, z0.z * z0.z, z0.w * z0.w, z1.x * z1.x, z1.y * z1.y, z1.z * z1.z, z1.w * z1.w};
        float P[8], A[8];
#pragma unroll
        for (int t = 0; t < 8; ++t) P[t] = sq[t] + __int_as_float(__builtin_amdgcn_update_dpp(0, __float_as_int(sq[t]), 0x104, 0xf, 0xf, true));
#pragma unroll
        for (int t = 0; t < 8; ++t) A[t] = P[t] + __int_as_float(__builtin_amdgcn_update_dpp(0, __float_as_int(P[t]), 0x101, 0xf, 0xf, true));
#pragma unroll
        for (int t = 0; t < 8; ++t) A[t] = A[t] + __int_as_float(__builtin_amdgcn_update_dpp(0, __float_as_int(P[t]), 0x102, 0xf, 0xf, true));
#pragma unroll
        for (int t = 0; t < 8; ++t) A[t] = A[t] + __int_as_float(__builtin_amdgcn_update_dpp(0, __float_as_int(P[t]), 0x103, 0xf, 0xf, true));
        float zz = 0.0f;
#pragma unroll
        for (int t = 0; t < 8; ++t) zz = zz + A[t];
        float m = 0.0f;
#pragma unroll
        for (int sidx = 0; sidx < 8; ++sidx) {
            const float im = __int_as_float(__builtin_amdgcn_update_dpp(0, __float_as_int(m), 0x111, 0xf, 0xf, true));
            m = __builtin_fmaf(z1.w, e1.w, __builtin_fmaf(z1.z, e1.z, __builtin_fmaf(z1.y, e1.y, __builtin_fmaf(z1.x, e1.x,
                __builtin_fmaf(z0.w, e0.w, __builtin_fmaf(z0.z, e0.z, __builtin_fmaf(z0.y, e0.y, __builtin_fmaf(z0.x, e0.x, im))))))));
        }
        const float zz7 = __int_as_float(__builtin_amdgcn_update_dpp(0, __float_as_int(zz), 0x117, 0xf, 0xf, true));
        const float d = (zz7 + eek) - 2.0f * m;
        if (j8 == 7 && jj < ntasks) {
            atomicMin(&tb.best_s[rr], trk::dist_key(d, kc));
            tb.zz_s[rr] = zz7;
        }
    }
    lds_order_wave();
    int o_best = 0;
    if ((F.o_open || F.o_hard) && !o_wide) {
        const unsigned long long bk = tb.best_s[lane];
        if (bk != ~0ull) o_best = (int)(unsigned)bk; else o_wide = true;
    }
    unsigned long long wm = __builtin_amdgcn_ballot_w64(o_wide);
    if (wm) {
        float *zrow_s = reinterpret_cast<float *>(tb.task_s);
        do {
            const int r = __builtin_amdgcn_readfirstlane((int)__builtin_ctzll(wm));
            wm &= wm - 1ull;
            __builtin_amdgcn_wave_barrier();
            zrow_s[lane] = zscalar(r, lane);
            if (lane == 0) tb.best_s[r] = ~0ull;
            lds_order_wave();
            const float zz = tb.zz_s[r];
            int best = 0;
            if (zz == zz) {
                unsigned long long key = ~0ull;
                for (int kb = lane; kb < K; kb += 256) {
                    float m[4] = {0.0f, 0.0f, 0.0f, 0.0f};
#pragma unroll 2
                    for (int c4 = 0; c4 < D / 4; ++c4) {
                        const f32x4 zv = *reinterpret_cast<const f32x4 *>(zrow_s + 4 * c4);
                        f32x4 e[4];
#pragma unroll
                        for (int i = 0; i < 4; ++i)
                            e[i] = __builtin_bit_cast(f32x4, __builtin_amdgcn_raw_buffer_load_b128(cb_rs, (unsigned)(kb + 64 * i) * (D * 4) + (unsigned)c4 * 16u, 0, 0));
#pragma unroll
                        for (int i = 0; i < 4; ++i)
                            m[i] = __builtin_fmaf(zv.w, e[i].w, __builtin_fmaf(zv.z, e[i].z, __builtin_fmaf(zv.y, e[i].y, __builtin_fmaf(zv.x, e[i].x, m[i]))));
                    }
#pragma unroll
                    for (int i = 0; i < 4; ++i) {
                        const int k = kb + 64 * i;
                        if (k < K) {
                            const float d = (zz + ee_g[k]) - 2.0f * m[i];
                            const unsigned long long kk = d != d ? (unsigned long long)(unsigned)k : trk::dist_key(d, k);
                            key = kk < key ? kk : key;
                        }
                    }
                }
                atomicMin(&tb.best_s[r], key);
                lds_order_wave();
                best = (int)(unsigned)tb.best_s[r];
            }
            if (lane == r) o_best = best;
        } while (wm);
    }
    if (R.open || R.hard || R.bad) R.kbest = o_best;
    __builtin_amdgcn_wave_barrier();
}

template <bool NCHW = false, int T = 2, bool HALF = false, class FRow>
__device__ __forceinline__ float epilogue_sp(const RowsSp<T> &R, int lane, const float *__restrict__ cb, int K, FRow &&frow,
                                             float *__restrict__ zq_unit, int nleft, long long *__restrict__ idx_unit,
                                             int *__restrict__ hist_s, float *tile_f = nullptr, int HW = 0, unsigned zq_bytes = 0u) {
    constexpr int D = 64, RU = 32 * T;
    const int j16 = lane & 15, g4 = lane >> 4;
    const auto cb_rs = __builtin_amdgcn_make_buffer_rsrc(const_cast<float *>(cb), 0, (unsigned)K * (D * 4), 0x00020000);
    f32x4 ev[T][8];
#pragma unroll
    for (int t = 0; t < T; ++t)
#pragma unroll
        for (int i = 0; i < 8; ++i) {
            const int kr = __builtin_amdgcn_ds_bpermute((32 * t + 4 * i + g4) << 2, R.kbest);
            ev[t][i] = __builtin_bit_cast(f32x4, __builtin_amdgcn_raw_buffer_load_b128(cb_rs, (unsigned)kr * (D * 4) + (unsigned)j16 * 16u, 0, 0));
        }
    if (R.valid) {
        idx_unit[lane] = R.kbest;
        atomicAdd(&hist_s[R.kbest], 1);
    }
    const auto zq_rs = __builtin_amdgcn_make_buffer_rsrc(zq_unit ? zq_unit : const_cast<float *>(cb), 0,
                                                         zq_unit ? (NCHW ? zq_bytes : (unsigned)nleft * (D * 4)) : 0u, 0x00020000);
    unsigned vo[4];
#pragma unroll
    for (int k = 0; k < 4; ++k) {
        vo[k] = (unsigned)lane * 16u + 4096u * k;
        asm volatile("" : "+v"(vo[k]));
    }
    float sqv[T][8];
    f32x4 oh[8];
    (void)oh;
#pragma unroll
    for (int t = 0; t < T; ++t)
#pragma unroll
        for (int i = 0; i < 8; ++i) {
            const f32x4 zv = frow(t, i), e = ev[t][i];
            const float d0 = e.x - zv.x, d1 = e.y - zv.y, d2 = e.z - zv.z, d3 = e.w - zv.w;
            f32x4 o;
            o.x = zv.x + d0; o.y = zv.y + d1; o.z = zv.z + d2; o.w = zv.w + d3;
            sqv[t][i] = ((d0 * d0 + d1 * d1) + d2 * d2) + d3 * d3;
            if constexpr (!NCHW) {
                __builtin_amdgcn_raw_buffer_store_b128(__builtin_bit_cast(u32x4v, o), zq_rs, vo[(t * 8 + i) >> 2] + (unsigned)((t * 8 + i) & 3) * 1024u, 0, VQ_ZQ_STORE_AUX);
            } else if constexpr (HALF) {
                oh[i] = o;
            } else {
                if (i == 0) lds_order_wave();
                *reinterpret_cast<f32x4 *>(tile_f + (4 * i + g4) * 64 + (((j16 ^ i) & 15) << 2)) = o;
                if (i == 7) {
                    lds_order_wave();
                    const int cl = lane >> 3, j8 = lane & 7;
                    unsigned so = (unsigned)(cl * HW + 4 * j8 + 32 * t) * 4u;
#pragma unroll
                    for (int c8 = 0; c8 < 8; ++c8) {
                        f32x4 wv;
#pragma unroll
                        for (int e2 = 0; e2 < 4; ++e2) wv[e2] = tile_f[(4 * j8 + e2) * 64 + ((((2 * c8 + (cl >> 2)) ^ j8) & 15) << 2) + (cl & 3)];
                        __builtin_amdgcn_raw_buffer_store_b128(__builtin_bit_cast(u32x4v, wv), zq_rs, so, 0, VQ_ZQ_STORE_AUX);
                        so += (unsigned)(8 * HW) * 4u;
                    }
                }
            }
        }
    if constexpr (NCHW && HALF) {
        static_assert(T == 1, "the half-tile form has one row tile per unit");
        const int cl = lane >> 3, j8 = lane & 7;
#pragma unroll
        for (int hh = 0; hh < 2; ++hh) {
            lds_order_wave();
            if ((j16 >> 3) == hh) {
#pragma unroll
                for (int i = 0; i < 8; ++i) *reinterpret_cast<f32x4 *>(tile_f + (4 * i + g4) * 32 + ((((j16 & 7) ^ i) & 7) << 2)) = oh[i];
            }
            lds_order_wave();
            unsigned so = (unsigned)((32 * hh + cl) * HW + 4 * j8) * 4u;
#pragma unroll
            for (int c8 = 0; c8 < 4; ++c8) {
                f32x4 wv;
#pragma unroll
                for (int e2 = 0; e2 < 4; ++e2) wv[e2] = tile_f[(4 * j8 + e2) * 32 + ((((2 * c8 + (cl >> 2)) ^ j8) & 7) << 2) + (cl & 3)];
                __builtin_amdgcn_raw_buffer_store_b128(__builtin_bit_cast(u32x4v, wv), zq_rs, so, 0, VQ_ZQ_STORE_AUX);
                so += (unsigned)(8 * HW) * 4u;
            }
        }
    }
    float sacc = 0.0f;
    if (nleft == RU) {
#pragma unroll
        for (int t = 0; t < T; ++t)
#pragma unroll
            for (int i = 0; i < 8; ++i) sacc += sqv[t][i];
    } else {
#pragma unroll
        for (int t = 0; t < T; ++t)
#pragma unroll
            for (int i = 0; i < 8; ++i) sacc += 32 * t + 4 * i + g4 < nleft ? sqv[t][i] : 0.0f;
    }
    return sacc;
}

}
}
```

Before: 4.521 million images/s.

## Fuse decoder head into quantizing encoder kernel and finalize into decoder tail

The encoder kernel that quantizes z_e now continues in the same workgroup with the decoder's front transposed conv and residual pair. It feeds z_q from registers and LDS, so z_q is no longer written to global memory and read back. The VQ loss/perplexity finalize kernel is folded into block 0 of the decoder tail kernel, which removes one launch. This adds register and LDS pressure and a longer kernel in the fused instance, and block 0 of the tail kernel now does serial reduction work.

```diff
diff --git a/vqvae_amd/csrc/common.h b/vqvae_amd/csrc/common.h
--- a/vqvae_amd/csrc/common.h
+++ b/vqvae_amd/csrc/common.h
@@ -142,8 +142,12 @@
     int K, K32;
     float *zq; long long *idx; int *hist; double *partials;
 };
+struct ResPairDecHead { const float *packed_front; const float *bias_front; const float *packed_w1; const float *packed_w2; int flags;
+                        float *y; int *out_amax; };
 struct ResPairPost { const float *packed; const float *bias; int Cout; float *out; int *zero = nullptr; int zero_n = 0;
-                     const VqFuse *vq = nullptr; bool debug_ze = false; };
+                     const VqFuse *vq = nullptr; bool debug_ze = false;
+                     const ResPairDecHead *dec_head = nullptr; };
+struct VqFinalizeArgs { const double *partials; int nparts; const int *hist; int K; long long N; int D; float beta; float *loss; float *perplexity; };
 bool res_pair_post_supported(int C, int Cout);
 int res_pair_forward_impl(const float *x, const float *packed_w1, const float *packed_w2, int64_t B, int H, int W, int C,
                           int Rh, int flags, float *y, hipStream_t stream, const int *in_amax, int *out_amax,
@@ -179,7 +183,8 @@
                            int *out_amax, int *zero_buf = nullptr, int zero_n = 0);
 bool dec_tail_supported(int h4, int w4, int C, int C1, int Cout);
 int dec_tail_forward_impl(const float *x, const float *packed2, const float *bias2, const float *packed4, const float *bias4,
-                          int64_t B, int h4, int w4, int C, int C1, int Cout, float *y_nchw, hipStream_t st, const int *in_amax);
+                          int64_t B, int h4, int w4, int C, int C1, int Cout, float *y_nchw, hipStream_t st, const int *in_amax,
+                          const VqFinalizeArgs *finalize = nullptr);
 int conv_in_forward_impl(const float *x_nchw, const float *packed, const float *bias, int64_t B, int H, int W, int Cin,
                          int Cout, int flags, float *y, hipStream_t stream, int *out_amax, const float *ep_mask = nullptr);
 
diff --git a/vqvae_amd/csrc/conv_fused.hip b/vqvae_amd/csrc/conv_fused.hip
--- a/vqvae_amd/csrc/conv_fused.hip
+++ b/vqvae_amd/csrc/conv_fused.hip
@@ -7,7 +7,15 @@
 #ifndef CRP_MINW
 #define CRP_MINW 2
 #endif
-template <int NT3, bool VQ = false, bool GATHER = false, bool ZEOUT = false>
+struct DecHeadArgs {
+    FrontConv fc;
+    const u32x4 *w1img, *w2img;
+    const int *hdr1, *hdr2;
+    int flags;
+    float *out;
+    int *out_amax;
+};
+template <int NT3, bool VQ = false, bool GATHER = false, bool ZEOUT = false, bool DECHEAD = false>
 __global__ __launch_bounds__(CRP_NW * 64, CRP_MINW) void conv_res_pair8_h2_kernel(const float *__restrict__ in, FrontConv fc,
                                                                    const u32x4 *__restrict__ w1img, const u32x4 *__restrict__ w2img,
                                                                    float *__restrict__ out, int B, int flags,
@@ -15,7 +23,8 @@
                                                                    const int *__restrict__ in_amax, int *__restrict__ out_amax,
                                                                    const u32x4 *__restrict__ w3img, const int *__restrict__ hdr3,
                                                                    const float *__restrict__ bias3, float *__restrict__ out3,
-                                                                   int *__restrict__ zero_buf, int zero_n, VqFuse vq) {
+                                                                   int *__restrict__ zero_buf, int zero_n, VqFuse vq, DecHeadArgs dh) {
+    static_assert(!DECHEAD || (VQ && !GATHER && !ZEOUT), "the decoder's head continues the quantizing instance");
     static_assert(NT3 == 0 || NT3 == 1 || NT3 == 2 || NT3 == 4, "the 1x1 post conv streams through NT3 weight stages of 16 KiB");
     static_assert(!VQ || (NT3 == 2 && CRP_NW == 4), "the fused quantizer takes the 64-channel z_e of four images per workgroup");
     constexpr int NT2 = 4, C = 128, MT = 2, PX = 64, HP = PX + 1, PLANE = HP * 2;
@@ -24,7 +33,9 @@
     __shared__ u32x4 As_all[CRP_NW * TILE4];
     constexpr int WBUF = 18 * 64;
     const int nvq = VQ ? (vq.K32 >> 7) : 0;
-    const int NSTAGE = 18 + NT3 + nvq;
+    int NSTAGE = 18 + NT3 + nvq;
+    FrontConv fcc = fc;
+    const u32x4 *w1c = w1img, *w2c = w2img;
     __shared__ u32x4 Wb_all[2 * WBUF];
     __shared__ __attribute__((aligned(16))) unsigned char vq_tab_all[VQ ? CRP_NW * 1040 : 16];
     __shared__ int vq_hist_s[VQ ? 1024 : 1];
@@ -35,10 +46,13 @@
     if constexpr (VQ) {
         for (int i = threadIdx.x; i < vq.K; i += CRP_NW * 64) vq_hist_s[i] = 0;
     }
-    const int tid = threadIdx.x, lane = tid & 63, wave = tid >> 6;
-    const int l31 = lane & 31, h = lane >> 5;
-    u32x4 *As = As_all + wave * TILE4;
-    float *Hs = reinterpret_cast<float *>(As);
+    const int tid = threadIdx.x, wave = tid >> 6;
+    int lane, l31, h;
+    u32x4 *As;
+    float *Hs;
+    unsigned dma_lane;
+    int spx[MT];
+    unsigned tapok[MT], tapok0[MT];
     const bool relu_out = flags & kFlagReluOut;
     constexpr int cpt = C >> 5;
 
@@ -47,33 +61,50 @@
     if (zero_buf && blockIdx.x == 0)
         for (int i = tid; i < zero_n; i += CRP_NW * 64) zero_buf[i] = 0;
 
-    int spx[MT];
-    unsigned tapok[MT], tapok0[MT];
-#pragma unroll
-    for (int mt = 0; mt < MT; ++mt) {
-        spx[mt] = 32 * mt + l31;
-        const int y = spx[mt] >> 3, x = spx[mt] & 7;
-        unsigned m = 0, m0 = 0;
-#pragma unroll
-        for (int t = 0; t < 9; ++t) {
-            const int yy = y + t / 3 - 1, xx = x + t % 3 - 1;
-            if (yy >= 0 && yy < 8 && xx >= 0 && xx < 8) m |= 1u << t;
-            const int y0 = y + (int)((fc.dym >> (4 * t)) & 15) - 8, x0 = x + (int)((fc.dxm >> (4 * t)) & 15) - 8;
-            if (y0 >= 0 && y0 < 8 && x0 >= 0 && x0 < 8) m0 |= 1u << t;
-        }
-        tapok[mt] = m;
-        tapok0[mt] = m0;
-    }
+    auto lane_setup = [&](int t_id) {
+        lane = t_id & 63;
+        l31 = lane & 31;
+        h = lane >> 5;
+        As = As_all + (t_id >> 6) * TILE4;
+        Hs = reinterpret_cast<float *>(As);
+        dma_lane = (unsigned)lane * 16u;
+#pragma unroll
+        for (int mt = 0; mt < MT; ++mt) {
+            spx[mt] = 32 * mt + l31;
+            const int y = spx[mt] >> 3, x = spx[mt] & 7;
+            unsigned m = 0;
+#pragma unroll
+            for (int t = 0; t < 9; ++t) {
+                const int yy = y + t / 3 - 1, xx = x + t % 3 - 1;
+                if (yy >= 0 && yy < 8 && xx >= 0 && xx < 8) m |= 1u << t;
+            }
+            tapok[mt] = m;
+        }
+    };
+    lane_setup(tid);
+    auto front_masks = [&]() {
+#pragma unroll
+        for (int mt = 0; mt < MT; ++mt) {
+            const int y = spx[mt] >> 3, x = spx[mt] & 7;
+            unsigned m0 = 0;
+#pragma unroll
+            for (int t = 0; t < 9; ++t) {
+                const int y0 = y + (int)((fcc.dym >> (4 * t)) & 15) - 8, x0 = x + (int)((fcc.dxm >> (4 * t)) & 15) - 8;
+                if (y0 >= 0 && y0 < 8 && x0 >= 0 && x0 < 8) m0 |= 1u << t;
+            }
+            tapok0[mt] = m0;
+        }
+    };
+    front_masks();
 
     f32x16 Y[MT][NT2];
     const int wave_u = __builtin_amdgcn_readfirstlane(wave);
-    const unsigned dma_lane = (unsigned)lane * 16u;
     auto dma = [&](const u32x4 *src_uniform, u32x4 *dst_piece) {
         const unsigned lds = __builtin_amdgcn_readfirstlane((unsigned)(unsigned long long)(__attribute__((address_space(3))) char *)(char *)dst_piece);
         asm volatile("s_mov_b32 m0, %2\n\ts_nop 0\n\tglobal_load_lds_dwordx4 %0, %1" ::"v"(dma_lane), "s"(src_uniform), "s"(lds) : "memory");
     };
     auto dma_slice = [&](int sl, int buf) {
-        const u32x4 *base = w1img + (size_t)(sl >> 1) * 256 + (sl & 1) * 64;
+        const u32x4 *base = w1c + (size_t)(sl >> 1) * 256 + (sl & 1) * 64;
         for (int p = wave_u; p < 18; p += CRP_NW)
             dma(base + (size_t)(p >> 1) * cpt * 256 + (p & 1) * 128, Wb_all + buf * WBUF + p * 64);
     };
@@ -88,7 +119,7 @@
             if (wave_u == 0) dma(reinterpret_cast<const u32x4 *>(vq.seeds) + (size_t)j * 32, Wb_all + buf * WBUF + 16 * 64);
         }
         else if (k >= 18) dma_linear(w3img + (size_t)(k - 18) * 1024, buf);
-        else if (k % 9 == 8) dma_linear(w2img, buf);
+        else if (k % 9 == 8) dma_linear(w2c, buf);
         else dma_slice(k % 9, buf);
     };
     auto dma_wait_sync = [&]() {
@@ -97,8 +128,17 @@
     };
     float ymax = 0.0f;
     int wstage = 0;
-    {
-        const int cpt0 = fc.Cin >> 5;
+    f32x4 zr[2][8];
+    f32x16(&Yo)[MT][NT2] = Y;
+    float &ymax_o = ymax;
+    int &wstage_o = wstage;
+    auto front = [&](auto FZ) __attribute__((always_inline)) {
+        constexpr bool FROMZ = decltype(FZ)::value;
+        const FrontConv &fc = fcc;
+        f32x16 Y[MT][NT2];
+        float ymax = 0.0f;
+        int wstage = 0;
+        const int cpt0 = FROMZ ? 2 : fc.Cin >> 5;
         const float *src = in + ((size_t)(img_ok ? img : 0) * PX + lane) * fc.Cin;
         bool gbad = false;
         if constexpr (GATHER) {
@@ -109,6 +149,11 @@
         const bool gany = GATHER && __builtin_amdgcn_ballot_w64(gbad) != 0;
         f32x4 raw[8];
         auto load_raw0 = [&](int cc) {
+            if constexpr (FROMZ) {
+#pragma unroll
+                for (int j = 0; j < 8; ++j) raw[j] = cc == 0 ? zr[0][j] : zr[1][j];
+                return;
+            }
 #pragma unroll
             for (int j = 0; j < 8; ++j) raw[j] = *reinterpret_cast<const f32x4 *>(src + 32 * cc + 4 * j);
             if (gany) {
@@ -118,13 +163,19 @@
             }
         };
         float m = 0.0f;
-        const int given = (in_amax && img_ok) ? in_amax[img] : -1;
-        if (given >= 0) m = __int_as_float(given);
+        const int given = (!FROMZ && in_amax && img_ok) ? in_amax[img] : -1;
+        auto fold_raw = [&]() {
+#pragma unroll
+            for (int j = 0; j < 8; ++j)
+                m = fmaxf(m, fmaxf(fmaxf(__builtin_fabsf(raw[j].x), __builtin_fabsf(raw[j].y)), fmaxf(__builtin_fabsf(raw[j].z), __builtin_fabsf(raw[j].w))));
+        };
+        if constexpr (FROMZ) {
+            load_raw0(0); fold_raw();
+            load_raw0(1); fold_raw();
+        } else if (given >= 0) m = __int_as_float(given);
         else for (int cc = 0; cc < cpt0; ++cc) {
             load_raw0(cc);
-#pragma unroll
-            for (int j = 0; j < 8; ++j)
-                m = fmaxf(m, fmaxf(fmaxf(__builtin_fabsf(raw[j].x), __builtin_fabsf(raw[j].y)), fmaxf(__builtin_fabsf(raw[j].z), __builtin_fabsf(raw[j].w))));
+            fold_raw();
         }
         const int kx = wave_scale_exp(img_ok ? m : 0.0f);
         const float xs = __builtin_ldexpf(1.0f, kx), d0 = __builtin_ldexpf(1.0f, -kx);
@@ -171,14 +222,14 @@
                         X[t][mt][0] = ap[0];
                         X[t][mt][1] = ap[PLANE];
                     }
-                if (tap == 1 && cc + 1 < cpt0) {
+                if (!FROMZ && tap == 1 && cc + 1 < cpt0) {
                     asm volatile("s_waitcnt vmcnt(8)" ::: "memory");
                     __syncthreads();
                 } else dma_wait_sync();
                 if (tap + 1 < 9) dma_front(cc, tap + 1, (wstage + 1) & 1);
                 else if (cc + 1 < cpt0) dma_front(cc + 1, 0, (wstage + 1) & 1);
                 else dma_stage(0, (wstage + 1) & 1);
-                if (tap == 0 && cc + 1 < cpt0) load_raw0(cc + 1);
+                if (tap == 0 && cc + 1 < cpt0) load_raw0(FROMZ ? 1 : cc + 1);
                 const u32x4 *wt = Wb_all + (wstage & 1) * WBUF + lane;
                 u32x4 Wc0 = wt[0], Wc1 = wt[64];
 #pragma unroll
@@ -211,8 +262,15 @@
                     for (int q = 0; q < 4; q += 2)
                         SCALE2_BIAS_RELU2(Y[mt][nt][4 * g + q], Y[mt][nt][4 * g + q + 1], dv[q], dv[q + 1], bv[q], bv[q + 1], ymax);
             }
-    }
-    lds_order_wave();
+        lds_order_wave();
+#pragma unroll
+        for (int mt = 0; mt < MT; ++mt)
+#pragma unroll
+            for (int nt = 0; nt < NT2; ++nt) Yo[mt][nt] = Y[mt][nt];
+        ymax_o = ymax;
+        wstage_o = wstage;
+    };
+    front(std::false_type{});
 
     auto stage_sync = [&](int k) -> const u32x4 * {
         dma_wait_sync();
@@ -533,7 +591,16 @@
                            [&](int rr, int jc) { return *zchunk(rr, jc); },
                            [&](int rr, int c) { return reinterpret_cast<const float *>(zchunk(rr, c >> 2))[c & 3]; });
             const int j16 = lane & 15, g4 = lane >> 4;
-            const float sacc = vqu::epilogue_sp<false, MT>(R, lane, vq.cb, vq.K, [&](int t, int i) { return *zchunk(32 * t + 4 * i + g4, j16); },
+            float sacc;
+            if constexpr (DECHEAD) {
+                sacc = vqu::epilogue_sp<false, MT>(R, lane, vq.cb, vq.K, [&](int t, int i) { return *zchunk(32 * t + 4 * i + g4, j16); },
+                                                   nullptr, img_ok ? PX : 0, vq.idx + (size_t)(img_ok ? img : 0) * PX, vq_hist_s, nullptr, 0, 0u,
+                                                   [&](int t, int i, const f32x4 &o) { *zchunk(32 * t + 4 * i + g4, j16) = o; });
+                lds_order_wave();
+#pragma unroll
+                for (int c16 = 0; c16 < 16; ++c16) zr[c16 >> 3][c16 & 7] = *zchunk(lane, c16);
+            } else
+            sacc = vqu::epilogue_sp<false, MT>(R, lane, vq.cb, vq.K, [&](int t, int i) { return *zchunk(32 * t + 4 * i + g4, j16); },
                                              (img_ok && vq.zq) ? vq.zq + (size_t)img * PX * 64 : nullptr, img_ok ? PX : 0,
                                              vq.idx + (size_t)(img_ok ? img : 0) * PX, vq_hist_s);
             double dacc = img_ok ? (double)sacc : 0.0;
@@ -549,6 +616,33 @@
             for (int k = tid; k < vq.K; k += CRP_NW * 64) {
                 const int c = vq_hist_s[k];
                 if (c) atomicAdd(&vq.hist[k], c);
+            }
+            if constexpr (DECHEAD) {
+                int tid2 = tid;
+                asm volatile("" : "+v"(tid2));
+                lane_setup(tid2);
+                fcc = dh.fc;
+                w1c = dh.w1img;
+                w2c = dh.w2img;
+                NSTAGE = 18;
+                for (int i = tid; i < 288; i += CRP_NW * 64)
+                    dw_s[i] = i < 128 ? h2_dw(dh.fc.hdr)[i] : (i < 160 ? h2_dw(dh.hdr1)[i - 128] : h2_dw(dh.hdr2)[i - 160]);
+                front_masks();
+                front(std::true_type{});
+                layer(std::integral_constant<int, 0>{}, true);
+                layer(std::integral_constant<int, 1>{}, (dh.flags & kFlagReluOut) != 0);
+                if (dh.out_amax && img_ok) publish_amax_exclusive(dh.out_amax, img, ymax, lane);
+                if (img_ok) {
+#pragma unroll
+                    for (int mt = 0; mt < MT; ++mt)
+#pragma unroll
+                        for (int nt = 0; nt < NT2; ++nt) {
+                            float v[16];
+#pragma unroll
+                            for (int r = 0; r < 16; ++r) v[r] = Y[mt][nt][r];
+                            store_tile(v, dh.out + (wbase + mt * 32) * C + nt * 32, C);
+                        }
+                }
             }
         } else
         if (img_ok) {
@@ -833,8 +927,12 @@
                                                               const int *__restrict__ hdr2, const float *__restrict__ bias2,
                                                               TailGeom tg, const u32x4 *__restrict__ w4img,
                                                               const int *__restrict__ hdr4, const float *__restrict__ bias4,
-                                                              float *__restrict__ out, int B, const int *__restrict__ in_amax) {
+                                                              float *__restrict__ out, int B, const int *__restrict__ in_amax,
+                                                              VqFinalizeArgs fin) {
     constexpr int NT = 2, MT = 2, PX = 64, HP = PX + 1, PLANE = HP * 2, CIN = 128, CPT = CIN / 32, CO = 3;
+    __shared__ double fin_red[256];
+    if (fin.loss && blockIdx.x == 0)
+        vqu::finalize_block(fin_red, fin.partials, fin.nparts, fin.hist, fin.K, fin.N, fin.D, fin.beta, fin.loss, fin.perplexity);
     constexpr int TILE4 = 2 * 2 * PLANE;
     constexpr int WBUF = 16 * 64, NSTAGE = 34;
     __shared__ u32x4 As_all[4 * TILE4];
@@ -1124,6 +1222,30 @@
                  make_geom(VQVAE_CONV_1x1, 1, 8, 8, C, post->Cout, 0, g3) != VQVAE_OK)) return VQVAE_ERR_UNSUPPORTED;
     if (post && post->vq && (post->Cout != 64 || CRP_NW != 4 || post->vq->K32 % 128 || post->vq->K32 > 1024 || !post->vq->partials))
         return VQVAE_ERR_UNSUPPORTED;
+    const ResPairDecHead *hd = post ? post->dec_head : nullptr;
+    DecHeadArgs dha{};
+    if (hd) {
+        ConvGeom gd;
+        if (!post->vq || post->debug_ze || post->vq->zq || !hd->packed_front || !hd->packed_w1 || !hd->packed_w2 || !hd->y ||
+            (reinterpret_cast<uintptr_t>(hd->y) & 15) || make_geom(VQVAE_CONVT_3x3_S1, B, H, W, 64, C, 0, gd) != VQVAE_OK)
+            return VQVAE_ERR_UNSUPPORTED;
+        const char *hfd = reinterpret_cast<const char *>(hd->packed_front) + packed_h2_offset(gd, VQVAE_CONVT_3x3_S1);
+        dha.fc.wimg = reinterpret_cast<const u32x4 *>(hfd + h2_header_bytes(gd.ntile));
+        dha.fc.hdr = reinterpret_cast<const int *>(hfd);
+        dha.fc.bias = hd->bias_front;
+        dha.fc.dym = gd.dymask[0];
+        dha.fc.dxm = gd.dxmask[0];
+        dha.fc.Cin = 64;
+        const char *d1 = reinterpret_cast<const char *>(hd->packed_w1) + (size_t)9 * cpt * (1024 * sizeof(float) + 3072 * sizeof(unsigned short));
+        const char *d2 = reinterpret_cast<const char *>(hd->packed_w2) + (size_t)cpt * (1024 * sizeof(float) + 3072 * sizeof(unsigned short));
+        dha.w1img = reinterpret_cast<const u32x4 *>(d1 + h2_header_bytes(1));
+        dha.w2img = reinterpret_cast<const u32x4 *>(d2 + h2_header_bytes((C + 31) / 32));
+        dha.hdr1 = reinterpret_cast<const int *>(d1);
+        dha.hdr2 = reinterpret_cast<const int *>(d2);
+        dha.flags = hd->flags;
+        dha.out = hd->y;
+        dha.out_amax = hd->out_amax;
+    }
     prof_begin(VQVAE_PROF_RES_LAYER, st);
     if (post) {
         const char *h3 = reinterpret_cast<const char *>(post->packed) + packed_h2_offset(g3, VQVAE_CONV_1x1);
@@ -1131,13 +1253,16 @@
         const int *hd3 = reinterpret_cast<const int *>(h3);
 #define CRP_POST(NT3_)                                                                                                          \
     hipLaunchKernelGGL((conv_res_pair8_h2_kernel<NT3_>), dim3(gtc), dim3(CRP_NW * 64), 0, st, x, fc, w1h, w2h, y, (int)B, flags, hd1, hd2, \
-                       in_amax, out_amax, w3h, hd3, post->bias, post->out, post->zero, post->zero_n, VqFuse{})
+                       in_amax, out_amax, w3h, hd3, post->bias, post->out, post->zero, post->zero_n, VqFuse{}, DecHeadArgs{})
         if (post->vq && post->debug_ze) {
             hipLaunchKernelGGL((conv_res_pair8_h2_kernel<2, true, false, true>), dim3(gtc), dim3(CRP_NW * 64), 0, st, x, fc, w1h, w2h, y, (int)B, flags,
-                               hd1, hd2, in_amax, out_amax, w3h, hd3, post->bias, post->out, post->zero, post->zero_n, *post->vq);
+                               hd1, hd2, in_amax, out_amax, w3h, hd3, post->bias, post->out, post->zero, post->zero_n, *post->vq, DecHeadArgs{});
+        } else if (post->vq && hd) {
+            hipLaunchKernelGGL((conv_res_pair8_h2_kernel<2, true, false, false, true>), dim3(gtc), dim3(CRP_NW * 64), 0, st, x, fc, w1h, w2h, y, (int)B,
+                               flags, hd1, hd2, in_amax, out_amax, w3h, hd3, post->bias, post->out, post->zero, post->zero_n, *post->vq, dha);
         } else if (post->vq) {
             hipLaunchKernelGGL((conv_res_pair8_h2_kernel<2, true>), dim3(gtc), dim3(CRP_NW * 64), 0, st, x, fc, w1h, w2h, y, (int)B, flags,
-                               hd1, hd2, in_amax, out_amax, w3h, hd3, post->bias, post->out, post->zero, post->zero_n, *post->vq);
+                               hd1, hd2, in_amax, out_amax, w3h, hd3, post->bias, post->out, post->zero, post->zero_n, *post->vq, DecHeadArgs{});
         } else
         switch (post->Cout / 32) {
             case 1: CRP_POST(1); break;
@@ -1151,10 +1276,10 @@
             gf.idx = reinterpret_cast<long long *>(const_cast<int64_t *>(gather_idx));
             gf.K = gather_K;
             hipLaunchKernelGGL((conv_res_pair8_h2_kernel<0, false, true>), dim3(gtc), dim3(CRP_NW * 64), 0, st, x, fc, w1h, w2h, y, (int)B, flags,
-                               hd1, hd2, in_amax, out_amax, nullptr, nullptr, nullptr, nullptr, nullptr, 0, gf);
+                               hd1, hd2, in_amax, out_amax, nullptr, nullptr, nullptr, nullptr, nullptr, 0, gf, DecHeadArgs{});
         } else
         hipLaunchKernelGGL((conv_res_pair8_h2_kernel<0>), dim3(gtc), dim3(CRP_NW * 64), 0, st, x, fc, w1h, w2h, y, (int)B, flags, hd1, hd2,
-                           in_amax, out_amax, nullptr, nullptr, nullptr, nullptr, nullptr, 0, VqFuse{});
+                           in_amax, out_amax, nullptr, nullptr, nullptr, nullptr, nullptr, 0, VqFuse{}, DecHeadArgs{});
     }
     prof_end(VQVAE_PROF_RES_LAYER, st);
     return (int)hipGetLastError();
@@ -1186,7 +1311,8 @@
 bool vqvae::dec_tail_supported(int h4, int w4, int C, int C1, int Cout) { return h4 == 8 && w4 == 8 && C == 128 && C1 == 64 && Cout == 3; }
 
 int vqvae::dec_tail_forward_impl(const float *x, const float *packed2, const float *bias2, const float *packed4, const float *bias4,
-                                 int64_t B, int h4, int w4, int C, int C1, int Cout, float *y_nchw, hipStream_t st, const int *in_amax) {
+                                 int64_t B, int h4, int w4, int C, int C1, int Cout, float *y_nchw, hipStream_t st, const int *in_amax,
+                                 const VqFinalizeArgs *finalize) {
     if (!x || !packed2 || !packed4 || !y_nchw) return VQVAE_ERR_NULL;
     if (B < 1 || !dec_tail_supported(h4, w4, C, C1, Cout)) return VQVAE_ERR_UNSUPPORTED;
     if ((reinterpret_cast<uintptr_t>(x) | reinterpret_cast<uintptr_t>(y_nchw)) & 15) return VQVAE_ERR_UNSUPPORTED;
@@ -1202,7 +1328,7 @@
     hipLaunchKernelGGL(dec_tail8_h2_kernel, dim3((unsigned)((B + 3) / 4)), dim3(256), 0, st, x,
                        reinterpret_cast<const u32x4 *>(h2 + h2_header_bytes(g.ntile)), reinterpret_cast<const int *>(h2), bias2, tg,
                        reinterpret_cast<const u32x4 *>(h4p + h2_header_bytes(1) + cells * 2048 * sizeof(unsigned short)),
-                       reinterpret_cast<const int *>(h4p), bias4, y_nchw, (int)B, in_amax);
+                       reinterpret_cast<const int *>(h4p), bias4, y_nchw, (int)B, in_amax, finalize ? *finalize : VqFinalizeArgs{});
     prof_end(VQVAE_PROF_CONV_OUT, st);
     return (int)hipGetLastError();
 }
diff --git a/vqvae_amd/csrc/model.hip b/vqvae_amd/csrc/model.hip
--- a/vqvae_amd/csrc/model.hip
+++ b/vqvae_amd/csrc/model.hip
@@ -101,6 +101,8 @@
     bool fused;
     bool vq_fuse;
     bool zq_amax;
+    bool mid_fuse;
+    bool tail_finalize;
 };
 FwdPlan fwd_plan(const VqvaeDims *d, int H, int W, int flags) {
     FwdPlan p{};
@@ -122,6 +124,13 @@
 #endif
     p.fused = p.enc_front && p.enc_pair_post && p.dec_front && p.dec_tail;
     p.vq_fuse = p.fused && vq_fuse_ok(d->n_embeddings, d->embedding_dim, flags);
+    const bool plain = p.vq_fuse && !(flags & kVqFormFlags) && !(flags & VQVAE_FWD_DEBUG_ZE);
+#ifndef VQVAE_NO_MID_FUSION
+    p.mid_fuse = plain && p.dec_front;
+#endif
+#ifndef VQVAE_NO_TAIL_FINALIZE
+    p.tail_finalize = plain && p.dec_tail;
+#endif
     return p;
 }
 
@@ -269,7 +278,8 @@
 
 static int encoder_run(const VqvaeWeights *w, const float *x, int64_t B, int H, int W, float *z_e, void *workspace,
                        size_t workspace_bytes, hipStream_t st, const FwdPlan &p, int *am_given, int *zero_buf = nullptr, int zero_n = 0,
-                       bool *zeroed = nullptr, const VqFuse *vq = nullptr, float *hid_given = nullptr, bool debug_ze = false) {
+                       bool *zeroed = nullptr, const VqFuse *vq = nullptr, float *hid_given = nullptr, bool debug_ze = false,
+                       const ResPairDecHead *dec_head = nullptr) {
     if (!w || !x || !z_e || !workspace) return VQVAE_ERR_NULL;
     const VqvaeDims *d = &w->dims;
     if (!dims_ok(d) || B < 1 || H < 4 || W < 4 || H % 4 || W % 4) return VQVAE_ERR_SHAPE;
@@ -298,7 +308,7 @@
         if ((rc = conv_forward_impl(VQVAE_CONV_4x4_S2, a, w->enc2, w->enc2_b, B, H / 2, W / 2, h / 2, h, VQVAE_CONV_RELU_OUT | cf, b, st, am0, am1)) != 0) return rc;
     }
     if (p.enc_pair_post) {
-        const ResPairPost post{w->pre, w->pre_b, d->embedding_dim, z_e, vq ? nullptr : zero_buf, vq ? 0 : zero_n, vq, vq && debug_ze};
+        const ResPairPost post{w->pre, w->pre_b, d->embedding_dim, z_e, vq ? nullptr : zero_buf, vq ? 0 : zero_n, vq, vq && debug_ze, dec_head};
         if (zeroed) *zeroed = zero_buf != nullptr;
         return conv_res_pair_forward_impl(VQVAE_CONV_3x3_S1, b, w->enc4, w->enc4_b, h, w->enc_res_w1, w->enc_res_w2, B, H / 4, W / 4, h,
                                           d->res_h_dim, VQVAE_CONV_RELU_OUT, nullptr, st, am1, nullptr, &post);
@@ -335,8 +345,9 @@
 static int *zq_amax_slot(const VqvaeDims *d, int64_t B, int *am) { return am + (size_t)(2 + d->n_res_layers) * B; }
 static int decoder_run(const VqvaeWeights *w, const float *z_q, int64_t B, int h4, int w4, float *x_hat, void *workspace,
                        size_t workspace_bytes, hipStream_t st, const FwdPlan &p, int *am_given, bool zq_amax_given = false,
-                       float *hid_given = nullptr, const int64_t *gather_idx = nullptr) {
-    if (!w || !z_q || !x_hat || !workspace) return VQVAE_ERR_NULL;
+                       float *hid_given = nullptr, const int64_t *gather_idx = nullptr, ResPairDecHead *head_out = nullptr,
+                       bool head_done = false, const VqFinalizeArgs *finalize = nullptr) {
+    if (!w || (!z_q && !head_out && !head_done) || !x_hat || !workspace) return VQVAE_ERR_NULL;
     const VqvaeDims *d = &w->dims;
     if (!dims_ok(d) || B < 1 || h4 < 1 || w4 < 1) return VQVAE_ERR_SHAPE;
     Carve c{static_cast<char *>(workspace), workspace_bytes};
@@ -357,7 +368,7 @@
     int rc;
     if (gather_idx && !p.dec_front) return VQVAE_ERR_UNSUPPORTED;
     int *amz = nullptr;
-    if (am && !gather_idx && p.zq_amax) {
+    if (am && !gather_idx && p.zq_amax && !head_out && !head_done) {
         amz = zq_amax_slot(d, B, am);
         if (!zq_amax_given) act_absmax_impl(z_q, B, (long long)h4 * w4 * d->embedding_dim, amz, st);
     }
@@ -365,6 +376,11 @@
     const int *amt = am;
     if (p.dec_front) {
         int *aout = am ? am + (size_t)2 * B : nullptr;
+        if (head_out) {
+            *head_out = ResPairDecHead{w->dec0, w->dec0_b, w->dec_res_w1, w->dec_res_w2, VQVAE_CONV_RELU_OUT, a, aout};
+            return VQVAE_OK;
+        }
+        if (!head_done)
         if ((rc = conv_res_pair_forward_impl(VQVAE_CONVT_3x3_S1, z_q, w->dec0, w->dec0_b, d->embedding_dim, w->dec_res_w1, w->dec_res_w2, B, h4,
                                              w4, h, d->res_h_dim, VQVAE_CONV_RELU_OUT, a, st, amz, aout, nullptr, gather_idx,
                                              d->n_embeddings)) != 0) return rc;
@@ -378,7 +394,8 @@
         if (!res_layer_fused_ok(h, d->res_h_dim)) amt = nullptr;
     }
     if (p.dec_tail)
-        return dec_tail_forward_impl(t, w->dec2, w->dec2_b, w->dec4, w->dec4_b, B, h4, w4, h, h / 2, d->in_ch, x_hat, st, amt);
+        return dec_tail_forward_impl(t, w->dec2, w->dec2_b, w->dec4, w->dec4_b, B, h4, w4, h, h / 2, d->in_ch, x_hat, st, amt, finalize);
+    if (finalize) return VQVAE_ERR_UNSUPPORTED;
     float *u = (t == a) ? b : a;
     int *am_u = am ? am + (size_t)(3 + d->n_res_layers) * B : nullptr;
     if ((rc = conv_forward_impl(VQVAE_CONVT_4x4_S2, t, w->dec2, w->dec2_b, B, h4, w4, h, h / 2, VQVAE_CONV_RELU_OUT | cf, u, st, amt, am_u)) != 0) return rc;
@@ -466,11 +483,19 @@
         const bool debug_ze = vq_flags & VQVAE_FWD_DEBUG_ZE;
         if (debug_ze && !idx) return VQVAE_ERR_NULL;
         if (debug_ze) vf.partials = reinterpret_cast<double *>(idx_ws);
+        const VqFinalizeArgs fin{vf.partials, (int)((B + 3) / 4), hist, d->n_embeddings, (long long)rows, d->embedding_dim, d->beta, loss, perplexity};
+        ResPairDecHead head{};
+        if (p.mid_fuse) {
+            if ((rc = decoder_run(w, nullptr, B, H / 4, W / 4, x_hat, acts, acts_bytes, st, p, am_dec, false, nullptr, nullptr, &head)) != 0) return rc;
+            vf.zq = nullptr;
+        }
         if ((rc = encoder_run(w, x, B, H, W, z_e, acts, acts_bytes, st, p, am2, hist, d->n_embeddings, &hist_zeroed, &vf, nullptr,
-                              debug_ze)) != 0) return rc;
-        if ((rc = vq_finalize_impl(vf.partials, (int)((B + 3) / 4), hist, d->n_embeddings, (int64_t)rows, d->embedding_dim, d->beta, loss,
+                              debug_ze, p.mid_fuse ? &head : nullptr)) != 0) return rc;
+        if (!p.tail_finalize &&
+            (rc = vq_finalize_impl(vf.partials, (int)((B + 3) / 4), hist, d->n_embeddings, (int64_t)rows, d->embedding_dim, d->beta, loss,
                                    perplexity, st)) != 0) return rc;
-        return decoder_run(w, z_q, B, H / 4, W / 4, x_hat, acts, acts_bytes, st, p, am_dec);
+        return decoder_run(w, z_q, B, H / 4, W / 4, x_hat, acts, acts_bytes, st, p, am_dec, false, nullptr, nullptr, nullptr, p.mid_fuse,
+                           p.tail_finalize ? &fin : nullptr);
     }
     bool zq_amax_done = false;
     if ((rc = encoder_run(w, x, B, H, W, z_e, acts, acts_bytes, st, p, am2, p.fused ? hist : nullptr, d->n_embeddings, &hist_zeroed,
diff --git a/vqvae_amd/csrc/vq_exact.hip b/vqvae_amd/csrc/vq_exact.hip
--- a/vqvae_amd/csrc/vq_exact.hip
+++ b/vqvae_amd/csrc/vq_exact.hip
@@ -1,5 +1,6 @@
 #include "common.h"
 #include "vq_device.h"
+#include "vq_unit.h"
 
 namespace vqvae {
 
@@ -325,36 +326,7 @@
                                                           float *__restrict__ loss,
                                                           float *__restrict__ perplexity) {
     __shared__ double red[256];
-    const int tid = threadIdx.x;
-    double s = 0.0;
-    const float fn = (float)N;
-    for (int k = tid; k < K; k += 256) {
-        const float p = (float)hist[k] / fn;
-        const float lg = (float)log((double)(p + 1e-10f));
-        s += (double)(p * lg);
-    }
-    red[tid] = s;
-    __syncthreads();
-    for (int o = 128; o > 0; o >>= 1) {
-        if (tid < o) red[tid] += red[tid + o];
-        __syncthreads();
-    }
-    const double ent = red[0];
-    __syncthreads();
-    double q = 0.0;
-    for (int i = tid; i < nparts; i += 256) q += partials[i];
-    red[tid] = q;
-    __syncthreads();
-    for (int o = 128; o > 0; o >>= 1) {
-        if (tid < o) red[tid] += red[tid + o];
-        __syncthreads();
-    }
-    if (tid == 0) {
-        *perplexity = (float)exp(-(double)(float)ent);
-        const float m = (float)(red[0] / ((double)N * (double)D));
-        const float bm = beta * m;
-        *loss = m + bm;
-    }
+    vqu::finalize_block(red, partials, nparts, hist, K, N, D, beta, loss, perplexity);
 }
 
 __global__ __launch_bounds__(256) void vq_onehot_kernel(const long long *__restrict__ idx, long long N,
diff --git a/vqvae_amd/csrc/vq_unit.h b/vqvae_amd/csrc/vq_unit.h
--- a/vqvae_amd/csrc/vq_unit.h
+++ b/vqvae_amd/csrc/vq_unit.h
@@ -1,6 +1,7 @@
 #pragma once
 #include "common.h"
 #include "vq_track.h"
+#include <type_traits>
 
 #ifndef VQ_ZQ_STORE_AUX
 #define VQ_ZQ_STORE_AUX 0
@@ -316,11 +317,15 @@
     __builtin_amdgcn_wave_barrier();
 }
 
-template <bool NCHW = false, int T = 2, bool HALF = false, class FRow>
+struct NoSink {};
+template <bool NCHW = false, int T = 2, bool HALF = false, class FRow, class Sink = NoSink>
 __device__ __forceinline__ float epilogue_sp(const RowsSp<T> &R, int lane, const float *__restrict__ cb, int K, FRow &&frow,
                                              float *__restrict__ zq_unit, int nleft, long long *__restrict__ idx_unit,
-                                             int *__restrict__ hist_s, float *tile_f = nullptr, int HW = 0, unsigned zq_bytes = 0u) {
+                                             int *__restrict__ hist_s, float *tile_f = nullptr, int HW = 0, unsigned zq_bytes = 0u,
+                                             Sink &&sink = Sink{}) {
     constexpr int D = 64, RU = 32 * T;
+    constexpr bool kSink = !std::is_same<typename std::remove_reference<Sink>::type, NoSink>::value;
+    static_assert(!kSink || !NCHW, "the sink takes row-major chunks");
     const int j16 = lane & 15, g4 = lane >> 4;
     const auto cb_rs = __builtin_amdgcn_make_buffer_rsrc(const_cast<float *>(cb), 0, (unsigned)K * (D * 4), 0x00020000);
     f32x4 ev[T][8];
@@ -355,7 +360,9 @@
             f32x4 o;
             o.x = zv.x + d0; o.y = zv.y + d1; o.z = zv.z + d2; o.w = zv.w + d3;
             sqv[t][i] = ((d0 * d0 + d1 * d1) + d2 * d2) + d3 * d3;
-            if constexpr (!NCHW) {
+            if constexpr (kSink) {
+                sink(t, i, o);
+            } else if constexpr (!NCHW) {
                 __builtin_amdgcn_raw_buffer_store_b128(__builtin_bit_cast(u32x4v, o), zq_rs, vo[(t * 8 + i) >> 2] + (unsigned)((t * 8 + i) & 3) * 1024u, 0, VQ_ZQ_STORE_AUX);
             } else if constexpr (HALF) {
                 oh[i] = o;
@@ -414,5 +421,41 @@
     return sacc;
 }
 
-}
-}
+__device__ __forceinline__ void finalize_block(double *red, const double *__restrict__ partials, int nparts, const int *__restrict__ hist,
+                                               int K, long long N, int D, float beta, float *__restrict__ loss,
+                                               float *__restrict__ perplexity) {
+    const int tid = threadIdx.x;
+    double s = 0.0;
+    const float fn = (float)N;
+    for (int k = tid; k < K; k += 256) {
+        const float p = (float)hist[k] / fn;
+        const float lg = (float)log((double)(p + 1e-10f));
+        s += (double)(p * lg);
+    }
+    red[tid] = s;
+    __syncthreads();
+    for (int o = 128; o > 0; o >>= 1) {
+        if (tid < o) red[tid] += red[tid + o];
+        __syncthreads();
+    }
+    const double ent = red[0];
+    __syncthreads();
+    double q = 0.0;
+    for (int i = tid; i < nparts; i += 256) q += partials[i];
+    red[tid] = q;
+    __syncthreads();
+    for (int o = 128; o > 0; o >>= 1) {
+        if (tid < o) red[tid] += red[tid + o];
+        __syncthreads();
+    }
+    if (tid == 0) {
+        *perplexity = (float)exp(-(double)(float)ent);
+        const float m = (float)(red[0] / ((double)N * (double)D));
+        const float bm = beta * m;
+        *loss = m + bm;
+    }
+    __syncthreads();
+}
+
+}
+}
```

Result: faster. 4.627 million images/s, median of 6 (+2.3%).
